# open-speech/HTK

Measured on AMD Instinct MI355X. Metric: herest_gmm_frame_state_loglik_per_sec, higher is better.
Workload: dtype f32 (scores: bf16x3 split operands, fp32 accumulate) + f64 (alpha / beta with fp32-transcendental log-add, accumulators); 1 GPU; HERest EM iteration (pass + accumulator all-reduce + model update), 5000 tied states x 16 mix, D=39, 1250 x 500-frame utterances per GPU (BASELINE config[2]: 10k utterances sharded 8-way); states=5000, mix=16, utts_per_gpu=1250, frames=500, chunks=1, update=HERest -m 3 -v 0.01, on the device

## Files before the change

### htk_amd/build.py

```python
from __future__ import annotations

import os
import subprocess
import sys

HERE = os.path.dirname(os.path.abspath(__file__))
OBJ = os.path.join(HERE, "_obj")
LIB = os.path.join(HERE, "libhtk_amd.so")
HIP_SRCS = ["csrc/model.hip", "csrc/gmm_exact.hip", "csrc/gmm_full.hip", "csrc/gmm_mfma.hip", "csrc/gmm_bf16.hip", "csrc/gmm_f16.hip", "csrc/fb_kernels.hip", "csrc/fb_wave.hip", "csrc/fb_state.hip", "csrc/fb_lr.hip", "csrc/fb.hip", "csrc/viterbi.hip", "csrc/decode.hip", "csrc/decode_n.hip", "csrc/decode_ord.hip", "csrc/decode_set.hip", "csrc/mfcc.hip", "csrc/cepsnorm.hip", "csrc/inputxform.hip", "csrc/update.hip", "csrc/comm.hip", "csrc/treeclust.hip", "csrc/datacluster.hip", "csrc/treesynth.hip", "csrc/hinit.hip", "csrc/hrest.hip", "csrc/results.hip", "csrc/latrescore.hip"]
C_SRCS = ["host/prep.c", "host/update.c", "host/fbank.c", "host/accio.c", "host/parmfile.c", "host/cepsnorm.c", "host/mmf.c", "host/labio.c", "host/net.c", "host/lattice.c", "host/slfout.c", "host/treeclust.c", "host/treesynth.c", "host/hinit.c", "host/hrest.c", "host/unit_train.c", "host/results.c", "host/latrescore.c", "host/htktext.c"]
HEADERS = ["csrc/fb_lr_lean.inc", "csrc/internal.h", "csrc/kernels.h", "csrc/hipcheck.h", "csrc/devbuf.h", "csrc/ladd.h", "csrc/wavegrp.h", "csrc/fb_state.h", "csrc/decode.h", "csrc/decode_dev.h", "csrc/decode_ord.h", "csrc/hinit_seg.h", "csrc/gauss_derive.h", "csrc/unit_train.h", "csrc/results.h", "csrc/latrescore.h", "host/mmf_priv.h", "host/htktext.h", "../include/htk_amd.h"]
ARCH = "gfx950"
EXTRA_FLAGS = {"csrc/gmm_mfma.hip": ["-fno-honor-nans"], "csrc/gmm_bf16.hip": ["-fno-honor-nans"], "csrc/gmm_f16.hip": ["-fno-honor-nans"],
               "csrc/fb_kernels.hip": ["-Wno-pass-failed"]}


def _newer(target, deps):
    if not os.path.exists(target):
        return True
    t = os.path.getmtime(target)
    return any(os.path.getmtime(d) > t for d in deps if os.path.exists(d))


def build(force: bool = False, verbose: bool = False) -> str:
    os.makedirs(OBJ, exist_ok=True)
    hdrs = [os.path.join(HERE, h) for h in HEADERS]
    objs = []
    procs = []
    for src in HIP_SRCS + C_SRCS:
        p = os.path.join(HERE, src)
        if not os.path.exists(p):
            continue
        o = os.path.join(OBJ, os.path.basename(src) + ".o")
        objs.append(o)
        if force or _newer(o, [p] + hdrs):
            if src.endswith(".hip"):
                cmd = ["hipcc", "--offload-arch=" + ARCH, "-O3", "-ffp-contract=off", "-fPIC", "-std=c++17",
                       "-Wall", "-Wno-unused-function"] + EXTRA_FLAGS.get(src, []) + ["-c", p, "-o", o]
            else:
                cmd = ["gcc", "-O2", "-std=gnu11", "-ffp-contract=off", "-fPIC", "-Wall", "-c", p, "-o", o]
            if verbose:
                print(" ".join(cmd))
            procs.append((cmd, subprocess.Popen(cmd)))
    for cmd, pr in procs:
        if pr.wait() != 0:
            raise RuntimeError("build failed: " + " ".join(cmd))
    if force or procs or _newer(LIB, objs):
        cmd = ["hipcc", "--offload-arch=" + ARCH, "-shared", "-fPIC", "-o", LIB] + objs + ["-lm", "-ldl"]
        if verbose:
            print(" ".join(cmd))
        subprocess.check_call(cmd)
    build_tools(verbose)
    return LIB


TOOLS = ["herest", "hvite"]


def build_tools(verbose: bool = False) -> None:
    root = os.path.dirname(HERE)
    bindir = os.path.join(root, "tools", "bin")
    os.makedirs(bindir, exist_ok=True)
    for t in TOOLS:
        src = os.path.join(root, "tools", t + ".c")
        if not os.path.exists(src):
            continue
        exe = os.path.join(bindir, t)
        if not _newer(exe, [src, os.path.join(root, "tools", "cli_common.h"), os.path.join(root, "include", "htk_amd.h"), LIB]):
            continue
        cmd = ["gcc", "-O2", "-std=gnu11", "-Wall", "-I" + os.path.join(root, "include"), "-I" + os.path.join(root, "tools"), src, "-o", exe,
               "-L" + HERE, "-lhtk_amd", "-Wl,-rpath,$ORIGIN/../../htk_amd", "-lm"]
        if verbose:
            print(" ".join(cmd))
        subprocess.check_call(cmd)


if __name__ == "__main__":
    print(build(force="--force" in sys.argv, verbose=True))
```

### htk_amd/csrc/fb.hip

```cpp
#include <hip/hip_runtime.h>
#include <cstdio>
#include <cstdlib>
#include <cstring>
#include <cmath>
#include <algorithm>
#include <vector>
#include <thread>
#include <mutex>
#include <condition_variable>
#include <functional>
#include "internal.h"
#include "hipcheck.h"
#include "kernels.h"
#include "devbuf.h"

static constexpr char fbOwner[] = "fb";
typedef DevBufT<fbOwner> DevBuf;

struct PrepPool {
   std::vector<std::thread> th;
   std::mutex mu;
   std::condition_variable cvGo, cvDone;
   std::function<void(int)> job;
   int generation = 0, pending = 0, nJobs = 0;
   bool quit = false;
   void start(int n)
   {
      for (int k = 0; k < n; k++)
         th.emplace_back([this, k]() {
            int seen = 0;
            for (;;) {
               std::function<void(int)> f;
               {
                  std::unique_lock<std::mutex> lk(mu);
                  cvGo.wait(lk, [&] { return quit || generation != seen; });
                  if (quit) return;
                  seen = generation;
                  if (k + 1 >= nJobs) { if (--pending == 0) cvDone.notify_one(); continue; }
                  f = job;
               }
               f(k + 1);
               std::unique_lock<std::mutex> lk(mu);
               if (--pending == 0) cvDone.notify_one();
            }
         });
   }
   void run(int n, const std::function<void(int)> &f)
   {
      if (n <= 1 || th.empty()) { for (int k = 0; k < n; k++) f(k); return; }
      {
         std::unique_lock<std::mutex> lk(mu);
         job = f; nJobs = n; pending = (int)th.size(); generation++;
      }
      cvGo.notify_all();
      f(0);
      std::unique_lock<std::mutex> lk(mu);
      cvDone.wait(lk, [&] { return pending == 0; });
   }
   ~PrepPool()
   {
      { std::unique_lock<std::mutex> lk(mu); quit = true; }
      cvGo.notify_all();
      for (auto &t : th) t.join();
   }
};


template <typename T> struct Tab : std::vector<T> { const T *dev = nullptr; };

enum TabGroup { TG_MODEL, TG_CELL, TG_SLOT, TG_SLOT_PAIR, TG_SLOT_STREAM, TG_THREAD, TG_TASK, TG_TASK_WIDE, TG_BATCH, TG_COUNT };

#define FB_BATCH_TABLES(X) \
   X(UttDesc, utt, TG_BATCH) \
   X(int, mN, TG_MODEL) X(int, mTp, TG_MODEL) X(int, mCell0, TG_MODEL) X(int, mSlot0, TG_MODEL) X(int, mDms, TG_MODEL) X(int, mHmm, TG_MODEL) X(int, mTrans, TG_MODEL) \
   X(int, slotState, TG_SLOT) \
   X(short, cQ, TG_CELL) X(short, thrCell, TG_THREAD) X(short, cI, TG_CELL) \
   X(short, taperLo, TG_BATCH) X(short, taperHi, TG_BATCH)       \
   X(ScoreTask, tasks, TG_TASK) X(ScoreTask, tasksW, TG_TASK_WIDE)       \
   X(size_t, gamOff, TG_BATCH) X(int, gamChunkUtt, TG_BATCH) \
   X(int, uttList, TG_BATCH)            \
   X(short, sQ, TG_SLOT) \
   X(int, slotStateU, TG_SLOT_STREAM)   \
   X(int, nextSame, TG_BATCH)           \
   X(int, qBeamNP, TG_BATCH)            \
   X(int, slotRange, TG_SLOT_PAIR)      \
   X(int, wqStart, TG_BATCH)

struct BatchTables {
#define X(T, name, group) Tab<T> name;
   FB_BATCH_TABLES(X)
#undef X
   template <class O, class F> void for_each(O &o, F &&f)
   {
#define X(T, name, group) f(name, o.name, group);
      FB_BATCH_TABLES(X)
#undef X
   }
   template <class F> void for_each(F &&f) { for_each(*this, [&](auto &v, auto &, int g) { f(v, g); }); }
};

struct PrepChunk : BatchTables {
   std::vector<int> evLo, evHi;
   size_t outp = 0, beta = 0, gam = 0;
   long long frameStates = 0;
   int nCellsMax = 1, QMax = 1, TMax = 1, nThrMax = 64, rc = HTKAMD_OK;
   char err[256] = "";
   void reset()
   {
      for_each([](auto &v, int) { v.clear(); });
      outp = beta = gam = 0; frameStates = 0; nCellsMax = QMax = TMax = 1; nThrMax = 64; rc = HTKAMD_OK; err[0] = 0;
   }
};

struct UttClasses {
   static constexpr int N = 13;
   struct Range { int first, n; };
   static int index(int family, int W) { return W == 0 ? 4 : (family ? 4 * family + 1 : 0) + (W == 1 ? 0 : W == 2 ? 1 : W == 4 ? 2 : 3); }
   void set(const std::vector<int> (&cls)[N], std::vector<int> &list)
   {
      list.clear();
      for (int c = 0; c < N; c++) { list.insert(list.end(), cls[c].begin(), cls[c].end()); off[c + 1] = (int)list.size(); }
   }
   Range of(int family, int W) const { const int c = index(family, W); return {off[c], off[c + 1] - off[c]}; }
   Range general() const { return of(FB_LANE_PER_MODEL, 0); } int nGeneral() const { return general().n; }
   int nLr() const { return off[N] - of(FB_LEFT_TO_RIGHT, 1).first; }
   bool anyOffLr() const { return of(FB_LEFT_TO_RIGHT, 1).first > 0; }
private:
   int off[N + 1] = {};
};

struct ResLayout {
   size_t nUtt;
   size_t status() const { return sizeof(double) * nUtt; }
   size_t counter() const { return (sizeof(double) + sizeof(int)) * nUtt; }
   size_t flag() const { return counter() + sizeof(int); } size_t bytes() const { return counter() + 2 * sizeof(int); }
};

enum { UTT_NO_TEE = 1, UTT_ALL_LR = 2 };

struct htkamd_fb : BatchTables {
   htkamd_model *m = nullptr;
   int nUtt = 0;
   int debug = 0;
   int forceGeneral = 0;
   int noStatePath = 0;
   int noLrPath = 0;
   int topoVersion = 0;
   std::vector<unsigned char> uttFlags;
   UttClasses cls;
   size_t gamTotal = 0, betaWTotal = 0, alphaWTotal = 0;
   int totalFrames = 0, nCellsMax = 1, QMax = 1, TMax = 1, blockDim = 64;
   long long frameStates = 0;
   const float *dX = nullptr;
   DevBuf d_arena;
   DevBuf d_qLo, d_qHi, d_aLo, d_aHi, d_outp, d_beta, d_gam, d_alpha, d_pr;
   DevBuf d_betaW;
   DevBuf d_tmE, d_tmMaxP;
   DevBuf d_outpU;
   DevBuf d_alphaW, d_qBeam, d_aBeam, d_trPart, d_hits, d_hitCtl;
   DevBuf d_sink;
   DevBuf d_stCnt, d_stBucket;
   DevBuf d_laneRec;
   bool mixStateLast = false;
   bool mixDeferred = false;
   FbArgs *faMix = nullptr;
   const int *qBeamLast = nullptr;
   DevBuf d_transOff, d_trOccOff, d_counter;
   DevBuf d_rec, d_recSorted, d_recCtl;
   int recCapForce = 0;
   PrepPool *pool = nullptr; std::vector<PrepChunk> *chunks = nullptr;
   void *h_arena = nullptr; size_t h_arenaCap = 0;
   void *h_res = nullptr; size_t h_resCap = 0;
   hipEvent_t evRes = nullptr; bool resPending = false;
   bool f16Pass = false;
   hipEvent_t ev[6] = {}, evK[2] = {}, evCopy = nullptr;
   hipStream_t resStream = nullptr;
   bool timed = false, copyPending = false, scored = false;
   int evMode = 0, evModeLast = 0;
   ResLayout res() const { return {(size_t)nUtt}; }
};

static bool compat_revisit(const htkamd_model *m) { return (m->compat & HTKAMD_COMPAT_STREAM_REVISIT) && m->NSt > 1 && m->NSt != 3 && !m->tiedMix; }

extern "C" int htkamd_fb_create(htkamd_model *m, htkamd_fb **out)
{
   if (!m || !out) { htkamd_set_error("fb_create: NULL argument"); return HTKAMD_EINVAL; }
   if (m->fullc) { htkamd_set_error("fb_create: forward-backward on FULLC models is not supported yet (its mixture statistics are diagonal)"); return HTKAMD_EMODEL; }
   if (m->maxM > 4096) { htkamd_set_error("fb_create: %d mixture components per state not supported", m->maxM); return HTKAMD_EMODEL; }
   htkamd_fb *fb = new htkamd_fb();
   fb->m = m;
   auto fail = [&](const char *what, hipError_t e) { htkamd_set_error("fb_create: %s: %s", what, hipGetErrorString(e)); htkamd_fb_destroy(fb); return HTKAMD_EHIP; };
   hipError_t e;
   for (hipEvent_t *v : {&fb->ev[0], &fb->ev[1], &fb->ev[2], &fb->ev[3], &fb->ev[4], &fb->ev[5], &fb->evK[0], &fb->evK[1]})
      if ((e = hipEventCreate(v)) != hipSuccess) return fail("hipEventCreate", e);
   if ((e = hipEventCreateWithFlags(&fb->evCopy, hipEventDisableTiming)) != hipSuccess) return fail("hipEventCreate", e);
   if ((e = hipStreamCreateWithFlags(&fb->resStream, hipStreamNonBlocking)) != hipSuccess) return fail("hipStreamCreate", e);
   int rc;
   if ((rc = fb->d_counter.reserve(64)) || (rc = fb->d_transOff.reserve(sizeof(int) * (m->nT + 1))) || (rc = fb->d_trOccOff.reserve(sizeof(int) * (m->nT + 1)))) { htkamd_fb_destroy(fb); return rc; }
   if ((e = hipMemcpy(fb->d_transOff.p, m->h_transOff, sizeof(int) * (m->nT + 1), hipMemcpyHostToDevice)) != hipSuccess ||
       (e = hipMemcpy(fb->d_trOccOff.p, m->h_trOccOff, sizeof(int) * (m->nT + 1), hipMemcpyHostToDevice)) != hipSuccess) return fail("hipMemcpy", e);
   *out = fb;
   return HTKAMD_OK;
}

extern "C" void htkamd_fb_destroy(htkamd_fb *fb)
{
   if (!fb) return;
   if (fb->h_arena) (void)hipHostFree(fb->h_arena);
   if (fb->h_res) (void)hipHostFree(fb->h_res);
   delete fb->pool; delete fb->chunks; delete fb->faMix;
   for (hipEvent_t v : fb->ev) if (v) (void)hipEventDestroy(v);
   for (hipEvent_t v : {fb->evCopy, fb->evRes, fb->evK[0], fb->evK[1]}) if (v) (void)hipEventDestroy(v);
   if (fb->resStream) (void)hipStreamDestroy(fb->resStream);
   delete fb;
}

extern "C" int htkamd_fb_set_debug(htkamd_fb *fb, int on)
{
   if (!fb) { htkamd_set_error("fb_set_debug: NULL"); return HTKAMD_EINVAL; }
   fb->debug = on & 1;
   fb->forceGeneral = (on & 2) ? 1 : 0;
   fb->noStatePath = (on & 4) ? 1 : 0;
   fb->recCapForce = (on & 8) ? 128 : ((on & 16) ? -1 : 0);
   fb->noLrPath = (on & 32) ? 1 : 0;
   return HTKAMD_OK;
}

static int prep_utterance(htkamd_fb *fb, const htkamd_batch_desc *b, int u, PrepChunk &C)
{
   const htkamd_model *m = fb->m;
   std::vector<int> &evLo = C.evLo, &evHi = C.evHi;
      UttDesc &d = fb->utt[u];
      const int T = b->frameOff[u + 1] - b->frameOff[u], Q = b->labOff[u + 1] - b->labOff[u];
      const int *labs = b->labs + b->labOff[u];
      d.T = T; d.Q = Q; d.frame0 = b->frameOff[u];
      d.q0 = (int)C.mN.size(); d.cell0 = (int)C.cQ.size(); d.slot0 = (int)C.slotState.size();
      d.status = HTKAMD_UTT_OK; d.nEval = 0;
      d.outp0 = C.outp; d.beta0 = C.beta; d.gam0 = C.gam;
      unsigned char &flags = fb->uttFlags[u];
      flags = UTT_NO_TEE | UTT_ALL_LR;
      if (T <= 0 || Q <= 0) {
         for (int t = 0; t < T; t++) { fb->taperLo[d.frame0 + t] = 0; fb->taperHi[d.frame0 + t] = 0; fb->qBeamNP[d.frame0 + t] = 1; }
         d.status = HTKAMD_UTT_SKIPPED; d.nCells = d.nSlots = 0; d.thr0 = (int)C.thrCell.size(); d.nThr = 0; return HTKAMD_OK;
      }
      int nCells = 0, nSlots = 0, qt = 0, prevDm = 1;
      for (int q = 1; q <= Q; q++) {
         const int h = labs[q - 1];
         if (h < 0 || h >= m->H) { snprintf(C.err, sizeof(C.err), "fb_prepare: utterance %d label %d: HMM index %d out of range", u, q, h); return HTKAMD_EINVAL; }
         const int ti = m->h_hmmTrans[h], N = m->h_transN[ti], dm = m->h_minDur[ti];
         C.mN.push_back(N); C.mTp.push_back(m->h_transOff[ti]); C.mCell0.push_back(nCells); C.mSlot0.push_back(nSlots);
         C.mDms.push_back(dm); C.mHmm.push_back(h); C.mTrans.push_back(ti);
         for (int i = 1; i <= N; i++) { C.cQ.push_back((short)q); C.cI.push_back((short)i); }
         for (int j = 2; j < N; j++) { C.slotState.push_back(m->h_hmmState[m->h_hmmStateOff[h] + (j - 2) * m->NSt]); C.sQ.push_back((short)q); C.slotRange.push_back(0); C.slotRange.push_back(-1); }
         nCells += N; nSlots += N - 2; qt += dm;
         if (dm == 0) flags &= ~UTT_NO_TEE;
         if (m->h_transLR[ti] != 1) flags &= ~UTT_ALL_LR;
         if (q > 1 && dm == 0 && prevDm == 0) d.status = HTKAMD_UTT_ETEE;
         prevDm = dm;
      }
      if (C.mDms[d.q0] == 0 || C.mDms[d.q0 + Q - 1] == 0) d.status = HTKAMD_UTT_ETEE;
      if (d.status == HTKAMD_UTT_OK && qt > T) d.status = HTKAMD_UTT_SKIPPED;
      d.nCells = nCells; d.nSlots = nSlots;
      if (m->NSt > 1) for (int ks = 0; ks < m->NSt; ks++) for (int k = 0; k < nSlots; k++) C.slotStateU.push_back(C.slotState[d.slot0 + k] + ks);
      {
         d.thr0 = (int)C.thrCell.size();
         for (int role = 0; role < 3; role++) {
            for (int q = 1; q <= Q; q++) {
               const int c0 = C.mCell0[d.q0 + q - 1], N = C.mN[d.q0 + q - 1];
               if (role == 0) C.thrCell.push_back((short)c0);
               else if (role == 2) C.thrCell.push_back((short)(c0 + N - 1));
               else for (int i = 2; i < N; i++) C.thrCell.push_back((short)(c0 + i - 1));
            }
            while ((C.thrCell.size() - d.thr0) % 64) C.thrCell.push_back((short)-1);
         }
         d.nThr = (int)C.thrCell.size() - d.thr0;
      }
      const bool waveOk = fb->m->maxN <= 5 && !fb->forceGeneral && !compat_revisit(fb->m) && Q <= 512;
      if (!waveOk) {
         if (Q > 32000 || d.nThr > 1024) {
            snprintf(C.err, sizeof(C.err), "fb_prepare: utterance %d has %d models / %d model states; the device path handles chains of up to 512 models of "
                     "up to 5 states, or up to 1024 model states per utterance", u, Q, nCells);
            return HTKAMD_EINVAL;
         }
         if (d.nThr > C.nThrMax) C.nThrMax = d.nThr;
         if (nCells > C.nCellsMax) C.nCellsMax = nCells;
         if (Q > C.QMax) C.QMax = Q;
      }
      if (T > C.TMax) C.TMax = T;
      C.outp += (size_t)T * nSlots; C.beta += (size_t)T * nCells; C.gam += (size_t)T * nSlots;
      if (d.status != HTKAMD_UTT_OK) {
         for (int t = 0; t < T; t++) { fb->taperLo[d.frame0 + t] = 0; fb->taperHi[d.frame0 + t] = 0; fb->qBeamNP[d.frame0 + t] = 1; }
         return HTKAMD_OK;
      }
      short *lo = fb->taperLo.data() + d.frame0 - 1, *hi = fb->taperHi.data() + d.frame0 - 1;
      const int *dms = C.mDms.data() + d.q0 - 1;
      {
         int q = 1, dq = dms[q], i = 0;
         for (int t = 1; t <= T; t++) {
            while (i == dq) { i = 0; if (q < Q) { q++; dq = dms[q]; } else dq = -1; }
            hi[t] = (short)q; i++;
         }
         q = Q; dq = dms[q]; i = 0;
         for (int t = T; t >= 1; t--) {
            while (i == dq) { i = 0; if (q > 1) { q--; dq = dms[q]; } else dq = -1; }
            lo[t] = (short)q; i++;
         }
      }
      evLo.assign(T + 2, 0); evHi.assign(T + 2, 0);
      {
         const long long before = C.frameStates;
         int qHiN = Q, qLoN = lo[T];
         int *npw = fb->qBeamNP.data() + d.frame0 - 1;
         npw[T] = qLoN | (qHiN << 16);
         const int *msl = C.mSlot0.data() + d.q0 - 1;
         auto slotsIn = [&](int a, int z) { return (z < Q ? msl[z + 1] : nSlots) - msl[a]; };
         evLo[T] = qLoN > 1 ? qLoN - 1 : 1; evHi[T] = Q;
// ... 213 lines not shown
         fb->h_arena = nullptr; fb->h_arenaCap = 0;
         const size_t want = total + total / 4;
         HIPCHECK(hipHostMalloc(&fb->h_arena, want, hipHostMallocDefault));
         fb->h_arenaCap = want;
      }
      if (fb->copyPending) { HIPCHECK(hipEventSynchronize(fb->evCopy)); fb->copyPending = false; }
      if ((rc = fb->d_arena.reserve(total))) return rc;
      {
         struct Piece { char *dst; const char *src; size_t n; };
         std::vector<Piece> pieces;
         const size_t cut = (size_t)256 << 10;
         const size_t *at = off.data();
         fb->for_each([&](auto &v, int) {
            const size_t bytes = sizeof(v[0]) * v.size();
            for (size_t o = 0; o < bytes; o += cut)
               pieces.push_back({(char *)fb->h_arena + *at + o, (const char *)v.data() + o, bytes - o < cut ? bytes - o : cut});
            v.dev = (decltype(v.dev))((char *)fb->d_arena.p + *at++);
         });
         const int nP = (int)pieces.size(), nT = nW < 8 ? nW : 8;
         fb->pool->run(nT, [&](int k) { for (int i = k; i < nP; i += nT) memcpy(pieces[i].dst, pieces[i].src, pieces[i].n); });
      }
      HIPCHECK(hipMemcpyAsync(fb->d_arena.p, fb->h_arena, total, hipMemcpyHostToDevice, s));
      HIPCHECK(hipEventRecord(fb->evCopy, s));
      fb->copyPending = true;
   }
   const bool wavePathPrep = fb->cls.nGeneral() == 0;
   const size_t nf = fb->totalFrames ? fb->totalFrames : 1;
   if ((rc = fb->d_qLo.reserve(sizeof(short) * nf)) || (rc = fb->d_qHi.reserve(sizeof(short) * nf)) ||
       (rc = fb->d_aLo.reserve(sizeof(short) * nf)) || (rc = fb->d_aHi.reserve(sizeof(short) * nf)) ||
       (rc = fb->d_outp.reserve(sizeof(float) * (outp + 16))) || (rc = fb->d_beta.reserve(sizeof(double) * ((beta && !wavePathPrep) ? beta : 1))) ||
       (rc = fb->d_gam.reserve(sizeof(double) * ((gam && fb->cls.anyOffLr()) ? gam : 1))) || (rc = fb->d_pr.reserve(ResLayout{(size_t)(U ? U : 1)}.bytes())) ||
       (fb->m->NSt > 1 && (rc = fb->d_outpU.reserve(sizeof(float) * (outp * fb->m->NSt + 16)))) ||
       (fb->m->tiedMix && ((rc = fb->d_tmE.reserve(sizeof(float) * (nf * fb->m->tmPool + 16))) || (rc = fb->d_tmMaxP.reserve(sizeof(float) * (nf * fb->m->NSt + 16))))))
      return rc;
   if (fb->debug && (rc = fb->d_alpha.reserve(sizeof(double) * (beta ? beta : 1)))) return rc;
   guard.ok = true;
   return HTKAMD_OK;
}

extern "C" long long htkamd_fb_frame_states(const htkamd_fb *fb) { return fb ? fb->frameStates : 0; }

extern "C" int htkamd_fb_score_work(const htkamd_fb *fb, long long out[3])
{
   if (!fb || !out) { htkamd_set_error("fb_score_work: NULL argument"); return HTKAMD_EINVAL; }
   long long skip = 0, all = 0;
   const bool ranges = fb->m->NSt == 1 && fb->slotRange.size() == 2 * fb->slotState.size();
   for (const ScoreTask &tk : fb->tasksW) {
      const int nPairs = (tk.nSlots + 1) >> 1;
      for (int w = 0; w < B16_TASK_FRAMES / 32; w++) {
         if (32 * w >= tk.nFrames) break;
         all += nPairs;
         if (!ranges) { skip += nPairs; continue; }
         const int r0 = tk.frame0 + 32 * w, r1 = r0 + 31;
         for (int j = 0; j < nPairs; j++) {
            const int k0 = tk.slot0 + 2 * j, k1 = (2 * j + 1 < tk.nSlots) ? k0 + 1 : k0;
            const int lo = std::min(fb->slotRange[2 * k0], fb->slotRange[2 * k1]), hi = std::max(fb->slotRange[2 * k0 + 1], fb->slotRange[2 * k1 + 1]);
            if (lo <= r1 && hi >= r0) skip++;
         }
      }
   }
   out[0] = skip; out[1] = all; out[2] = (fb->frameStates + 63) / 64;
   return HTKAMD_OK;
}

extern "C" int htkamd_fb_prepared_current(const htkamd_fb *fb) { return fb && fb->topoVersion == fb->m->topoVersion; }

static ScoreArgs fb_score_args(htkamd_fb *fb, const htkamd_fb_config *cfg)
{
   const htkamd_model *m = fb->m;
   ScoreArgs sa = htkamd_score_args(m);
   sa.NSt = 1; sa.streamWt = nullptr;
   const bool wideTasks = (cfg->scoreMode & (HTKAMD_SCORE_F16 | HTKAMD_SCORE_BF16 | HTKAMD_SCORE_MFMA)) != 0;
   const Tab<ScoreTask> &tasks = wideTasks ? fb->tasksW : fb->tasks;
   sa.tasks = tasks.dev; sa.nTasks = (int)tasks.size(); sa.X = fb->dX;
   sa.slotState = fb->slotState.dev; sa.out = (float *)fb->d_outp.p;
   if (m->NSt > 1) { sa.slotState = fb->slotStateU.dev; sa.out = (float *)fb->d_outpU.p; }
   sa.taskCounter = (int *)fb->d_counter.p;
   if (wideTasks && m->NSt == 1 && fb->wqStart.size() == 9) { sa.qStart = fb->wqStart.dev; sa.qCounters = (int *)fb->d_counter.p + 8; }
   if ((cfg->scoreMode & HTKAMD_SCORE_BF16) && !(cfg->scoreMode & HTKAMD_SCORE_F16) && m->NSt == 1 && !getenv("HTKAMD_NO_TAPER_SKIP")) sa.slotRange = fb->slotRange.dev;
   fb->f16Pass = (cfg->scoreMode & HTKAMD_SCORE_F16) != 0 && !m->tiedMix && sa.nTasks > 0;
   if (fb->f16Pass) {
      sa.taskCounter = (int *)((char *)fb->d_pr.p + fb->res().counter());
      sa.rangeFlag = (int *)((char *)fb->d_pr.p + fb->res().flag());
   }
   return sa;
}

static FbArgs fb_args(const htkamd_fb *fb, const htkamd_fb_config *cfg, const htkamd_accs *accs)
{
   const htkamd_model *m = fb->m;
   FbArgs fa;
   memset(&fa, 0, sizeof(fa));
   fa.utt = fb->utt.dev; fa.nUtt = fb->nUtt;
   fa.mN = fb->mN.dev; fa.mTp = fb->mTp.dev; fa.mCell0 = fb->mCell0.dev; fa.mSlot0 = fb->mSlot0.dev; fa.mDms = fb->mDms.dev; fa.mHmm = fb->mHmm.dev; fa.mTrans = fb->mTrans.dev;
   fa.sQ = fb->sQ.dev; fa.thrCell = fb->thrCell.dev; fa.cQ = fb->cQ.dev; fa.cI = fb->cI.dev; fa.slotState = fb->slotState.dev;
   fa.taperLo = fb->taperLo.dev; fa.taperHi = fb->taperHi.dev;
   fa.qLo = (short *)fb->d_qLo.p; fa.qHi = (short *)fb->d_qHi.p; fa.aLo = (short *)fb->d_aLo.p; fa.aHi = (short *)fb->d_aHi.p;
   fa.X = fb->dX; fa.transP = m->d_transP; fa.outp = (float *)fb->d_outp.p;
   fa.beta = (double *)fb->d_beta.p; fa.gam = (double *)fb->d_gam.p; fa.alphaDbg = fb->debug ? (double *)fb->d_alpha.p : nullptr;
   fa.pr = (double *)fb->d_pr.p; fa.status = (int *)((char *)fb->d_pr.p + fb->res().status());
   fa.stateCompOff = m->d_stateCompOff; fa.compGauss = m->d_compGauss;
   fa.NSt = m->NSt; fa.outpU = (const float *)fb->d_outpU.p; fa.dimStream = m->d_dimStream;
   fa.compatRevisit = compat_revisit(m) && !fb->nextSame.empty(); fa.nextSame = fb->nextSame.dev;
   fa.transOff = (const int *)fb->d_transOff.p; fa.trOccOff = (const int *)fb->d_trOccOff.p;
   fa.compLogWt = m->d_compLogWt; fa.gparam = m->d_gparam; fa.mean = m->d_mean; fa.laddTab = m->d_laddTab;
   fa.PS = m->PS; fa.D = m->D; fa.maxN = m->maxN; fa.maxM = m->maxM;
   fa.nCellsMax = fb->nCellsMax; fa.QMax = fb->QMax; fa.TMax = fb->TMax;
   fa.acc = accs->d_vec; fa.lay = accs->lay;
   fa.pruneInit = cfg->pruneInit; fa.pruneInc = cfg->pruneInc; fa.pruneLim = cfg->pruneLim;
   fa.minLogExp = m->minLogExp; fa.minFrwdP = cfg->minFrwdP; fa.uFlags = cfg->uFlags;
   fa.gamTotal = fb->gamTotal; fa.gamOffByUtt = fb->gamOff.dev; fa.gamChunkUtt = fb->gamChunkUtt.dev;
   return fa;
}

struct LdsSizes { size_t beta, alpha; };
static LdsSizes fb_lds_sizes(const FbArgs &fa)
{
   const size_t nc = fa.nCellsMax, qm = fa.QMax + 3, mn = fa.maxN, tm = (size_t)fa.TMax + 3;
   auto r8 = [](size_t x) { return (x + 7) & ~(size_t)7; };
   const size_t ldsTab = r8((size_t)LADD_NK * (LADD_DEG + 1) * 8);
   return {2 * r8(nc * 8) + r8(qm * 8) + r8(nc * mn * 4) + 4 * r8(qm * 4) + r8(32) + ldsTab,
           2 * r8(nc * 8) + r8(3 * nc * 8) + r8(qm * 8) + r8(nc * (mn + 1) * 8) + ldsTab + r8(3 * nc * 4) + 2 * r8(nc * mn * 4) + 4 * r8(qm * 4) + 2 * r8(tm * 2)};
}

static const int clsW[4] = {1, 2, 4, 8};

static int fb_reserve_lr(htkamd_fb *fb, const htkamd_fb_config *cfg, FbArgs &fa, bool fastLadd, hipStream_t s)
{
   const htkamd_model *m = fb->m;
   int rc;
   size_t rows = 0;
   for (int W : clsW) rows += (size_t)fb->cls.of(FB_LEFT_TO_RIGHT, W).n * htkamd_stats_lr_chunks(fb->TMax) * W;
   const size_t nfr = fb->totalFrames ? fb->totalFrames : 1;
   if ((rc = fb->d_laneRec.reserve(sizeof(LaneRec) * (fb->slotState.size() + 1))) || (rc = fb->d_sink.reserve(256))) return rc;
   fa.laneRec = (LaneRec *)fb->d_laneRec.p; fa.sink = (double *)fb->d_sink.p;
   if ((rc = fb->d_alphaW.reserve(sizeof(double) * (fb->alphaWTotal + 64))) || (rc = fb->d_qBeam.reserve(sizeof(int) * (nfr + 2))) ||
       (rc = fb->d_aBeam.reserve(sizeof(int) * (nfr + 2))) || (rc = fb->d_trPart.reserve(sizeof(double) * htkamd_stats_lr_row_doubles() * (rows + 256))) ||
       (rc = fb->d_hits.reserve(sizeof(MixHit) * (rows * htkamd_stats_lr_region_cap() + 64))) || (rc = fb->d_hitCtl.reserve(sizeof(int) * (rows + 1))))
      return rc;
   fa.alphaW = (double *)fb->d_alphaW.p; fa.qBeam = (int *)fb->d_qBeam.p; fa.aBeam = (int *)fb->d_aBeam.p; fa.trPart = (double *)fb->d_trPart.p;
   fa.hits = (MixHit *)fb->d_hits.p; fa.hitCtl = (int *)fb->d_hitCtl.p; fa.nHitRegions = (int)rows; fa.hitRegionCap = htkamd_stats_lr_region_cap();
   fa.hitSlots = (m->NSt > 1 || m->tiedMix) ? 1 : 0;
   fa.qBeamNP = fb->qBeamNP.dev;
   if (htkamd_beta_lr_is_lean(fa, fastLadd)) fa.qBeam = const_cast<int *>(fb->qBeamNP.dev);
   fb->qBeamLast = fa.qBeam;
   fb->mixStateLast = false;
   fa.fastMath = fastLadd ? 1 : 0;
   if (fb->recCapForce == 0 && !fa.hitSlots && m->maxM <= 16 && (m->D == 39 || m->D == 26 || m->D == 13) &&
       (cfg->uFlags & (HTKAMD_UPMEANS | HTKAMD_UPVARS | HTKAMD_UPMIXES))) {
      size_t cap = 64;
      while (cap < 65536 && cap * (size_t)m->S < (size_t)16 * fb->totalFrames) cap <<= 1;
      while (cap > 64 && cap * (size_t)m->S * sizeof(HitS) > ((size_t)1 << 30)) cap >>= 1;
      { const char *e = getenv("HTKAMD_ST_CAP"); if (e && atoi(e) > 0) cap = (size_t)atoi(e); }
      if ((rc = fb->d_stCnt.reserve(sizeof(int) * (3 * (size_t)m->S + 4))) || (rc = fb->d_stBucket.reserve(sizeof(HitS) * cap * (size_t)m->S))) return rc;
      fb->mixStateLast = true;
      fa.stCnt = (int *)fb->d_stCnt.p; fa.nTiedStates = m->S; fa.stBucket = (HitS *)fb->d_stBucket.p; fa.stCap = (int)cap;
      HIPCHECK(hipMemsetAsync(fa.stCnt, 0, sizeof(int) * (3 * (size_t)m->S + 4), s));
   }
   return HTKAMD_OK;
}

struct FamilyKernels { int family; int (*beta)(const FbArgs &, int, bool, hipStream_t); int (*alpha)(const FbArgs &, int, bool, hipStream_t); };
static const FamilyKernels familyKernels[] = {{FB_LANE_PER_MODEL, htkamd_launch_beta_w, htkamd_launch_alpha_w},
                                              {FB_LANE_PER_STATE, htkamd_launch_beta_s, htkamd_launch_alpha_s},
                                              {FB_LEFT_TO_RIGHT, htkamd_launch_beta_lr, htkamd_launch_alpha_lr}};

static int fb_recursions(htkamd_fb *fb, const FbArgs &fa, const LdsSizes &lds, bool fastLadd, bool noEv, hipStream_t s)
{
   int rc;
   for (int pass = 0; pass < 2; pass++) {
      FbArgs fc = fa;
      const UttClasses::Range g = fb->cls.general();
      fc.uttList = fb->uttList.dev + g.first; fc.nList = g.n;
      if (g.n > 0 && (rc = pass == 0 ? htkamd_launch_beta(fc, fb->blockDim, lds.beta, s) : htkamd_launch_alpha(fc, fb->blockDim, lds.alpha, s))) return rc;
      for (const FamilyKernels &k : familyKernels)
         for (int c = 3; c >= 0; c--) {
            const UttClasses::Range r = fb->cls.of(k.family, clsW[c]);
            fc.uttList = fb->uttList.dev + r.first; fc.nList = r.n;
            if ((rc = (pass == 0 ? k.beta : k.alpha)(fc, clsW[c], fastLadd, s))) return rc;
         }
      if (!noEv) HIPCHECK(hipEventRecord(fb->ev[2 + pass], s));
   }
   return HTKAMD_OK;
}

static int fb_stats_lr(htkamd_fb *fb, const FbArgs &fa, bool fastLadd, bool noEv, hipStream_t s)
{
   int rc;
   FbArgs fc = fa;
   size_t rowOff = 0;
   for (int c = 3; c >= 0; c--) {
      const UttClasses::Range r = fb->cls.of(FB_LEFT_TO_RIGHT, clsW[c]);
      fc.uttList = fb->uttList.dev + r.first; fc.nList = r.n;
      fc.trPart = fa.trPart ? fa.trPart + rowOff * htkamd_stats_lr_row_doubles() : nullptr;
      fc.hits = fa.hits ? fa.hits + rowOff * htkamd_stats_lr_region_cap() : nullptr; fc.hitCtl = fa.hitCtl ? fa.hitCtl + rowOff : nullptr;
      rowOff += (size_t)fc.nList * htkamd_stats_lr_chunks(fb->TMax) * clsW[c];
      if ((rc = htkamd_launch_stats_lr(fc, clsW[c], fastLadd, s))) return rc;
   }
   if (!noEv) HIPCHECK(hipEventRecord(fb->ev[4], s));
   return HTKAMD_OK;
}

static int fb_mix_stats(htkamd_fb *fb, const htkamd_fb_config *cfg, FbArgs &fa, bool defer, hipStream_t s)
{
   const htkamd_model *m = fb->m;
   const int nLr = fb->cls.nLr();
   int rc;
   if (!(cfg->uFlags & (HTKAMD_UPMEANS | HTKAMD_UPVARS | HTKAMD_UPMIXES))) return HTKAMD_OK;
   if ((cfg->uFlags & (HTKAMD_UPMEANS | HTKAMD_UPVARS)) && fb->recCapForce >= 0) {
      const size_t cap = fb->recCapForce > 0 ? (size_t)fb->recCapForce : std::min<size_t>((size_t)16 * fb->totalFrames + 4096, (size_t)1 << 30);
      if ((rc = fb->d_rec.reserve(sizeof(MixRec) * cap)) || (rc = fb->d_recSorted.reserve(sizeof(MixRec) * cap)) ||
          (rc = fb->d_recCtl.reserve(sizeof(int) * (3 * ((size_t)m->G + 1) + 1 + (size_t)m->G / 2048 + 2))))
         return rc;
      fa.rec = (MixRec *)fb->d_rec.p; fa.recSorted = (MixRec *)fb->d_recSorted.p; fa.recCap = (int)cap; fa.G = m->G; fa.recCtl = (int *)fb->d_recCtl.p;
   }
   if (m->tiedMix || m->NSt > 1) {
      fa.stateCompOff = m->d_stateCompOff; fa.rec = nullptr;
      if (fb->nUtt > nLr && (rc = m->tiedMix ? htkamd_launch_mixstats_tm(fa, s) : htkamd_launch_mixstats_ms(fa, s))) return rc;
      if (nLr > 0 && (rc = htkamd_launch_mixhits_streams(fa, m->tiedMix != 0, s))) return rc;
      return HTKAMD_OK;
   }
   const bool dense = fb->nUtt > nLr && fa.gamTotal > 0, listed = nLr > 0;
   if ((rc = htkamd_launch_mixstats(fa, s, dense, listed, defer))) return rc;
   if (defer && listed && !dense && htkamd_mixstate_applies(fa)) {
      if (!fb->faMix) fb->faMix = new FbArgs();
      *fb->faMix = fa;
      fb->mixDeferred = true;
   }
   return HTKAMD_OK;
}

static int fb_execute_impl(htkamd_fb *fb, const htkamd_fb_config *cfg, htkamd_accs *accs, void *stream, bool defer)
{
   if (!fb || !cfg || !accs) { htkamd_set_error("fb_execute: NULL argument"); return HTKAMD_EINVAL; }
   fb->mixDeferred = false;
   if (accs->m != fb->m) { htkamd_set_error("fb_execute: accumulators belong to a different model"); return HTKAMD_EINVAL; }
   if (fb->nUtt == 0) return HTKAMD_OK;
   const htkamd_model *m = fb->m;
   hipStream_t s = (hipStream_t)stream;
   if (fb->topoVersion != m->topoVersion) {
      htkamd_set_error("fb_execute: the model's minimum durations changed since htkamd_fb_prepare (a re-estimated transition reached or left zero): prepare the batch again");
      return HTKAMD_EINVAL;
   }
   const ScoreArgs sa = fb_score_args(fb, cfg);
   if (cfg->scoreMode & ~(HTKAMD_SCORE_MFMA | HTKAMD_SCORE_FASTLADD | HTKAMD_SCORE_BF16 | HTKAMD_SCORE_F16 | HTKAMD_SCORE_SOUTP | HTKAMD_SCORE_DIAGC)) { htkamd_set_error("fb_execute: unknown score mode %d", cfg->scoreMode); return HTKAMD_EINVAL; }
   const bool fastLadd = (cfg->scoreMode & HTKAMD_SCORE_FASTLADD) != 0;
   FbArgs fa = fb_args(fb, cfg, accs);
   const LdsSizes lds = fb_lds_sizes(fa);

   int rc;
   if (fb->copyPending) HIPCHECK(hipStreamWaitEvent(s, fb->evCopy, 0));
   const bool noEv = fb->evMode == 1;
   HIPCHECK(hipEventRecord(fb->ev[0], s));
   if (m->tiedMix) {
      fa.tmE = (float *)fb->d_tmE.p; fa.tmMaxP = (float *)fb->d_tmMaxP.p; fa.tmPoolOff = m->d_tmPoolOff; fa.tmPool = m->tmPool; fa.totalFrames = fb->totalFrames;
      fa.tmTasks = fb->tasks.dev; fa.tmNTasks = (int)fb->tasks.size(); fa.tmSlotState = sa.slotState; fa.tmOut = sa.out;
      fa.compWeight = m->d_compWeight; fa.var = m->d_var;
      if ((rc = htkamd_launch_tm_score(fa, s))) return rc;
      fb->scored = false;
   } else {
      if ((rc = htkamd_launch_score(cfg->scoreMode, m, sa, s, fb->evK[0], fb->evK[1]))) return rc;
      fb->scored = sa.nTasks > 0;
   }
   if (m->NSt > 1) {
      if ((rc = htkamd_launch_combine_streams(fa, s))) return rc;
      if (m->maxM > 1) fa.stateCompOff = m->d_msCompOff;
   } else if (m->tiedMix) fa.stateCompOff = m->d_msCompOff;
   if (!noEv) HIPCHECK(hipEventRecord(fb->ev[1], s));
   if (fb->cls.nGeneral() > 0 && lds.alpha > 160 * 1024) { htkamd_set_error("fb_execute: %zu bytes of LDS needed (max model size %zu states)", lds.alpha, (size_t)m->maxN); return HTKAMD_EMODEL; }
   if ((rc = fb->d_betaW.reserve(sizeof(double) * (fb->betaWTotal + 8 * 512)))) return rc;
   fa.betaW = (double *)fb->d_betaW.p;
   if (fb->cls.nLr() > 0 && (rc = fb_reserve_lr(fb, cfg, fa, fastLadd, s))) return rc;
   if ((rc = fb_recursions(fb, fa, lds, fastLadd, noEv, s)) || (rc = fb_stats_lr(fb, fa, fastLadd, noEv, s)) || (rc = fb_mix_stats(fb, cfg, fa, defer, s))) return rc;
   HIPCHECK(hipEventRecord(fb->ev[5], s));
   fb->timed = true; fb->evModeLast = noEv ? 1 : 0;
   return HTKAMD_OK;
}

extern "C" int htkamd_fb_execute(htkamd_fb *fb, const htkamd_fb_config *cfg, htkamd_accs *accs, void *stream)
{
   return fb_execute_impl(fb, cfg, accs, stream, false);
}

extern "C" int htkamd_fb_execute_begin(htkamd_fb *fb, const htkamd_fb_config *cfg, htkamd_accs *accs, void *stream, int *deferred)
{
   if (deferred) *deferred = 0;
   const int rc = fb_execute_impl(fb, cfg, accs, stream, true);
   if (rc == HTKAMD_OK && deferred && fb && fb->nUtt > 0) *deferred = fb->mixDeferred ? 1 : 0;
   return rc;
}

extern "C" int htkamd_fb_execute_mix(htkamd_fb *fb, int state0, int state1, void *stream)
{
   if (!fb) { htkamd_set_error("fb_execute_mix: NULL"); return HTKAMD_EINVAL; }
   if (fb->nUtt == 0 || !fb->mixDeferred) return HTKAMD_OK;
   const int rc = htkamd_launch_mixstate_range(*fb->faMix, state0, state1, (hipStream_t)stream);
   if (rc) return rc;
   HIPCHECK(hipEventRecord(fb->ev[5], (hipStream_t)stream));
   return HTKAMD_OK;
}


static int res_staging(htkamd_fb *fb, size_t bytes)
{
   if (bytes > fb->h_resCap) {
      if (fb->h_res) (void)hipHostFree(fb->h_res);
      fb->h_res = nullptr; fb->h_resCap = 0;
      HIPCHECK(hipHostMalloc(&fb->h_res, bytes + bytes / 4, hipHostMallocDefault));
      fb->h_resCap = bytes + bytes / 4;
   }
   return HTKAMD_OK;
}

extern "C" int htkamd_fb_results_begin(htkamd_fb *fb, void *stream)
{
   if (!fb) { htkamd_set_error("fb_results_begin: NULL"); return HTKAMD_EINVAL; }
   if (fb->nUtt == 0) return HTKAMD_OK;
   hipStream_t s = (hipStream_t)stream;
   const size_t bytes = fb->res().bytes();
   int rc = res_staging(fb, bytes);
   if (rc) return rc;
   if (!fb->evRes) HIPCHECK(hipEventCreateWithFlags(&fb->evRes, hipEventDisableTiming));
   HIPCHECK(hipMemcpyAsync(fb->h_res, fb->d_pr.p, bytes, hipMemcpyDeviceToHost, s));
   HIPCHECK(hipEventRecord(fb->evRes, s));
   fb->resPending = true;
   return HTKAMD_OK;
}

extern "C" int htkamd_fb_results(htkamd_fb *fb, double *pr, int *status, void *stream)
{
   if (!fb) { htkamd_set_error("fb_results: NULL"); return HTKAMD_EINVAL; }
   hipStream_t s = (hipStream_t)stream;
   if (fb->nUtt == 0) return HTKAMD_OK;
   const size_t bytes = fb->res().bytes();
   if (fb->resPending) {
      fb->resPending = false;
      HIPCHECK(hipEventSynchronize(fb->evRes));
   } else {
      int rc = res_staging(fb, bytes);
      if (rc) return rc;
      hipStream_t cs = fb->timed ? fb->resStream : s;
      if (fb->timed) HIPCHECK(hipEventSynchronize(fb->ev[5]));
      HIPCHECK(hipMemcpyAsync(fb->h_res, fb->d_pr.p, bytes, hipMemcpyDeviceToHost, cs));
      HIPCHECK(hipStreamSynchronize(cs));
   }
   if (pr) memcpy(pr, fb->h_res, sizeof(double) * (size_t)fb->nUtt);
   if (status) memcpy(status, (const char *)fb->h_res + fb->res().status(), sizeof(int) * (size_t)fb->nUtt);
   if (fb->f16Pass) {
      int flag;
      memcpy(&flag, (const char *)fb->h_res + fb->res().flag(), sizeof(int));
      if (flag) {
         htkamd_set_error("fb_results: the fp16 scoring path met %s%s%s outside its range: nothing of this pass can be used (accumulators included) -- repeat it with HTKAMD_SCORE_BF16",
                          (flag & HTKAMD_F16_EMODEL) ? "a model coefficient" : "", (flag & HTKAMD_F16_EMODEL) && (flag & HTKAMD_F16_EFEAT) ? " and " : "", (flag & HTKAMD_F16_EFEAT) ? "a feature value" : "");
         return HTKAMD_ERANGE;
      }
   }
   return HTKAMD_OK;
}

extern "C" int htkamd_fb_set_event_mode(htkamd_fb *fb, int mode)
{
   if (!fb || mode < 0 || mode > 1) { htkamd_set_error("fb_set_event_mode: bad argument"); return HTKAMD_EINVAL; }
   fb->evMode = mode;
   return HTKAMD_OK;
}

extern "C" int htkamd_fb_kernel_times5(htkamd_fb *fb, double out[5])
{
   if (!fb || !out) { htkamd_set_error("fb_kernel_times: NULL"); return HTKAMD_EINVAL; }
   if (!fb->timed) { htkamd_set_error("fb_kernel_times: nothing executed yet"); return HTKAMD_EINVAL; }
   HIPCHECK(hipEventSynchronize(fb->ev[5]));
   for (int i = 0; i < 5; i++) {
      float ms = 0.f;
      if (i == 0 && fb->scored) HIPCHECK(hipEventElapsedTime(&ms, fb->evK[0], fb->evK[1]));
      else if (fb->evModeLast == 1) { out[i] = -1.0; continue; }
      else HIPCHECK(hipEventElapsedTime(&ms, fb->ev[i], fb->ev[i + 1]));
      out[i] = (double)ms * 1e-3;
   }
   return HTKAMD_OK;
}

extern "C" int htkamd_fb_mix_counts(htkamd_fb *fb, long long out[2])
{
   if (!fb || !out) { htkamd_set_error("fb_mix_counts: NULL"); return HTKAMD_EINVAL; }
   out[0] = out[1] = -1;
   if (!fb->timed || !fb->mixStateLast || !fb->d_stCnt.p) return HTKAMD_OK;
   HIPCHECK(hipEventSynchronize(fb->ev[5]));
   const size_t S = (size_t)fb->m->S;
   std::vector<int> c(2 * S);
   HIPCHECK(hipMemcpy(c.data(), (int *)fb->d_stCnt.p + S + 4, sizeof(int) * 2 * S, hipMemcpyDeviceToHost));
   out[0] = out[1] = 0;
   for (size_t i = 0; i < S; i++) { out[0] += c[2 * i]; out[1] += c[2 * i + 1]; }
   return HTKAMD_OK;
}

extern "C" int htkamd_fb_kernel_times(htkamd_fb *fb, double out[4])
{
   double t[5];
   const int rc = htkamd_fb_kernel_times5(fb, t);
   if (rc) return rc;
   out[0] = t[0]; out[1] = t[1]; out[2] = (t[2] < 0.0 || t[3] < 0.0) ? -1.0 : t[2] + t[3]; out[3] = t[4];
   return HTKAMD_OK;
}

extern "C" int htkamd_fb_get_trellis(htkamd_fb *fb, int u, double *beta, double *alpha, float *outp,
                                     int *qLo, int *qHi, int *aLo, int *aHi, int *pT, int *pQ, int *pMaxN, void *stream)
{
   if (!fb || u < 0 || u >= fb->nUtt) { htkamd_set_error("fb_get_trellis: bad utterance index"); return HTKAMD_EINVAL; }
   hipStream_t s = (hipStream_t)stream;
   HIPCHECK(hipStreamSynchronize(s));
   const UttDesc &d = fb->utt[u];
   const int T = d.T, Q = d.Q, nC = d.nCells, nS = d.nSlots, maxN = fb->m->maxN;
   if (pT) *pT = T; if (pQ) *pQ = Q; if (pMaxN) *pMaxN = maxN;
   if (T <= 0 || Q <= 0) return HTKAMD_OK;
   std::vector<short> lo(T), hi(T), alo(T), ahi(T);
   const std::pair<std::vector<short> *, const DevBuf *> beams[] = {{&lo, &fb->d_qLo}, {&hi, &fb->d_qHi}, {&alo, &fb->d_aLo}, {&ahi, &fb->d_aHi}};
   for (auto &bm : beams) HIPCHECK(hipMemcpy(bm.first->data(), (short *)bm.second->p + d.frame0, sizeof(short) * T, hipMemcpyDeviceToHost));
   if (d.W > 0 && d.family == FB_LEFT_TO_RIGHT && fb->qBeamLast) {
      std::vector<int> qb(T);
      HIPCHECK(hipMemcpy(qb.data(), fb->qBeamLast + d.frame0, sizeof(int) * T, hipMemcpyDeviceToHost));
      for (int t = 0; t < T; t++) { lo[t] = (short)(qb[t] & 0xffff); hi[t] = (short)((qb[t] >> 16) & 0xffff); }
   }
   if (d.W > 0 && d.family == FB_LEFT_TO_RIGHT) {
      std::vector<int> ab(T);
      HIPCHECK(hipMemcpy(ab.data(), (int *)fb->d_aBeam.p + d.frame0, sizeof(int) * T, hipMemcpyDeviceToHost));
      for (int t = 0; t < T; t++) { alo[t] = fb->sQ[d.slot0 + (ab[t] & 0xffff)]; ahi[t] = fb->sQ[d.slot0 + ((ab[t] >> 16) & 0xffff)]; }
   }
   for (int t = 0; t < T; t++) {
      if (qLo) qLo[t] = lo[t]; if (qHi) qHi[t] = hi[t]; if (aLo) aLo[t] = alo[t]; if (aHi) aHi[t] = ahi[t];
   }
   const int *mN = fb->mN.data() + d.q0, *mC = fb->mCell0.data() + d.q0, *mS = fb->mSlot0.data() + d.q0;
   const size_t n = (size_t)T * Q * maxN;
   if (beta) {
      std::vector<double> b((size_t)T * nC);
      if (d.W > 0 && d.family != FB_LANE_PER_MODEL) {
         const bool lr = d.family == FB_LEFT_TO_RIGHT;
         const size_t Lw = (size_t)64 * d.W;
         std::vector<double> bs((size_t)T * (lr ? 1 : 2) * Lw);
         HIPCHECK(hipMemcpy(bs.data(), (double *)fb->d_betaW.p + d.betaW0, sizeof(double) * bs.size(), hipMemcpyDeviceToHost));
         std::vector<float> o(lr ? (size_t)T * nS : 0);
         if (lr) HIPCHECK(hipMemcpy(o.data(), (float *)fb->d_outp.p + d.outp0, sizeof(float) * o.size(), hipMemcpyDeviceToHost));
         const int *mTp = fb->mTp.data() + d.q0;
         auto entry = [&](int t, int q) {
            const int l0 = mS[q - 1];
            if (!lr) return bs[(size_t)T * Lw + (size_t)t * Lw + l0];
            if (q < lo[t] || q > hi[t]) return (double)LZERO;
            const double aa = fb->m->h_transP[mTp[q - 1] + 1], y = bs[(size_t)t * Lw + l0];
            if (!(aa > LSMALL && y > LSMALL)) return (double)LZERO;
            const double v = aa + (double)o[(size_t)l0 * T + t] + y;
            return v < LSMALL ? (double)LZERO : v;
         };
         for (int t = 0; t < T; t++)
            for (int q = 1; q <= Q; q++) {
               const int Nq = mN[q - 1], l0 = mS[q - 1];
               double *cell = &b[(size_t)t * nC + mC[q - 1]];
               cell[0] = entry(t, q);
               for (int i = 2; i < Nq; i++) cell[i - 1] = bs[(size_t)t * Lw + l0 + i - 2];
               double bN = LZERO;
               if (t == T - 1) bN = (q == Q) ? 0.0 : LZERO;
               else if (q < Q && q + 1 >= lo[t + 1] && q + 1 <= hi[t + 1]) bN = entry(t + 1, q + 1);
               cell[Nq - 1] = bN;
            }
      } else if (d.W > 0) {
         const size_t run = (size_t)64 * d.W;
         std::vector<double> bs((size_t)T * 5 * run);
         HIPCHECK(hipMemcpy(bs.data(), (double *)fb->d_betaW.p + d.betaW0, sizeof(double) * bs.size(), hipMemcpyDeviceToHost));
         for (int t = 0; t < T; t++)
            for (int q = 1; q <= Q; q++)
               for (int i = 0; i < mN[q - 1]; i++)
                  b[(size_t)t * nC + mC[q - 1] + i] = bs[((size_t)t * 5 + i) * run + (q - 1)];
      } else
      HIPCHECK(hipMemcpy(b.data(), (double *)fb->d_beta.p + d.beta0, sizeof(double) * b.size(), hipMemcpyDeviceToHost));
      for (size_t k = 0; k < n; k++) beta[k] = NAN;
      for (int t = 0; t < T; t++)
         for (int q = lo[t]; q <= hi[t]; q++)
            for (int i = 0; i < mN[q - 1]; i++)
               beta[((size_t)t * Q + (q - 1)) * maxN + i] = b[(size_t)t * nC + mC[q - 1] + i];
   }
   if (alpha) {
      if (!fb->debug) { htkamd_set_error("fb_get_trellis: alpha is only kept in debug mode (htkamd_fb_set_debug before prepare)"); return HTKAMD_EINVAL; }
      std::vector<double> al((size_t)T * nC);
      HIPCHECK(hipMemcpy(al.data(), (double *)fb->d_alpha.p + d.beta0, sizeof(double) * al.size(), hipMemcpyDeviceToHost));
      for (size_t k = 0; k < n; k++) alpha[k] = NAN;
      for (int t = 0; t < T; t++)
         for (int q = 1; q <= Q; q++)
            for (int i = 0; i < mN[q - 1]; i++)
               alpha[((size_t)t * Q + (q - 1)) * maxN + i] = al[(size_t)t * nC + mC[q - 1] + i];
   }
   if (outp) {
      std::vector<float> o((size_t)T * nS);
      HIPCHECK(hipMemcpy(o.data(), (float *)fb->d_outp.p + d.outp0, sizeof(float) * o.size(), hipMemcpyDeviceToHost));
      for (size_t k = 0; k < n; k++) outp[k] = NAN;
      for (int t = 0; t < T; t++)
         for (int q = 1; q <= Q; q++)
            for (int j = 2; j < mN[q - 1]; j++)
               outp[((size_t)t * Q + (q - 1)) * maxN + (j - 1)] = o[(size_t)(mS[q - 1] + j - 2) * T + t];
   }
   return HTKAMD_OK;
}

int htkamd_fb_device_results(htkamd_fb *fb, htkamd_fb_dev *out)
{
   if (!fb || !out || fb->nUtt <= 0 || !fb->d_pr.p) { htkamd_set_error("fb_device_results: no pass to read"); return HTKAMD_EINVAL; }
   out->pr = (const double *)fb->d_pr.p; out->status = (const int *)((const char *)fb->d_pr.p + fb->res().status());
   return HTKAMD_OK;
}
```

### htk_amd/csrc/fb_kernels.hip

```cpp
#include <hip/hip_runtime.h>
#include <cstring>
#include <cstdlib>
#include "internal.h"
#include "hipcheck.h"
#include "kernels.h"
#include "ladd.h"

#define ladd(x, y, mle) ladd_tab((x), (y), (mle), ltab)

#define EXPFLOOR (-100.0)

struct CellMeta {
   int q, i, N, mc0, ms0;
};

struct LdsCarve {
   char *p;
   __device__ explicit LdsCarve(void *base) : p((char *)base) {}
   template <typename T> __device__ T *take(size_t n)
   {
      T *r = (T *)p;
      p += ((n * sizeof(T) + 7) & ~(size_t)7);
      return r;
   }
// ... 533 lines not shown
            }
            recUsed += np;
         }
      }
   }
   if (pass) {
      if (upMu && !stored) atomicAdd(a.acc + a.lay.muOcc + g, Lr);
      if (upVa && !stored) atomicAdd(a.acc + a.lay.vaOcc + g, Lr);
      if (upWt) atomicAdd(a.acc + a.lay.wt + c0 + m, Lr);
   }
   unsigned long long pm = __ballot(pass && !stored);
   while (pm) {
      const int ml = __ffsll((long long)pm) - 1;
      pm &= pm - 1;
      const double L = __shfl(Lr, ml);
      const int gg = __shfl(g, ml);
      const unsigned long long xp = (unsigned long long)xrow;
      const float *xr = (const float *)(((unsigned long long)__shfl((int)(xp >> 32), ml) << 32) | (unsigned int)__shfl((int)(xp & 0xffffffffu), ml));
      const float *mean = a.mean + (size_t)gg * D;
      for (int k = lane; k < D; k += 64) {
         const float z = xr[k] - mean[k];
         if (upMu && upVa) {
            const float zl = (float)((double)z * L);
            atomicAdd(a.acc + a.lay.mu + (size_t)gg * D + k, (double)zl);
            atomicAdd(a.acc + a.lay.va + (size_t)gg * D + k, (double)(z * zl));
         } else if (upMu) {
            atomicAdd(a.acc + a.lay.mu + (size_t)gg * D + k, (double)z * L);
         } else if (upVa) {
            atomicAdd(a.acc + a.lay.va + (size_t)gg * D + k, (double)(z * z) * L);
         }
      }
   }
}

template <int DT, int GS>
__device__ __forceinline__ void mix_hit(const FbArgs &a, const bool ok, const int st, const int frameRow, const double seed, int &recBase, int &recUsed)
{
   const int lane = threadIdx.x & 63, sub = lane % GS;
   const int D = DT > 0 ? DT : a.D;
   const double minF = (double)a.minFrwdP;
   const int s = ok ? st : 0;
   const int c0 = a.stateCompOff[s], M = ok ? a.stateCompOff[s + 1] - c0 : 0;
   const float *xrow = a.X + (size_t)(ok ? frameRow : 0) * D;
   int Mmax = M;
#pragma unroll
   for (int o = 32; o > 0; o >>= 1) { const int w = __shfl_xor(Mmax, o); Mmax = w > Mmax ? w : Mmax; }
   for (int mb = 0; mb < Mmax; mb += GS) {
      const int m = mb + sub;
      bool pass = false;
      double Lr = 0.0;
      int g = 0;
      if (m < M) {
         g = a.compGauss[c0 + m];
         if (M == 1 || a.maxM == 1) { pass = true; Lr = exp(seed); }
         else {
            const float wt = a.compLogWt[c0 + m];
            if (wt > (float)LMINMIX) {
               const float *P = a.gparam + (size_t)g * a.PS;
               float sum = P[2 * D];
               if (DT > 0) {
                  const float4 *P4 = (const float4 *)P;
                  constexpr int NQ = (DT + 1) / 2;
#pragma unroll 1
                  for (int q0 = 0; q0 < NQ; q0 += 4) {
                     float4 pv[4]; float xv[8];
#pragma unroll
                     for (int i = 0; i < 4; i++) if (q0 + i < NQ) pv[i] = P4[q0 + i];
#pragma unroll
                     for (int i = 0; i < 8; i++) if (2 * q0 + i < DT) xv[i] = xrow[2 * q0 + i];
#pragma unroll
                     for (int i = 0; i < 8; i++)
                        if (2 * q0 + i < DT) {
                           const float mu = (i & 1) ? pv[i >> 1].z : pv[i >> 1].x, iv = (i & 1) ? pv[i >> 1].w : pv[i >> 1].y;
                           const float xmm = xv[i] - mu;
                           sum += xmm * xmm * iv;
                        }
                  }
               } else {
                  for (int i = 0; i < D; i++) {
                     const float xmm = xrow[i] - P[2 * i];
                     sum += xmm * xmm * P[2 * i + 1];
                  }
               }
               const float prob = -0.5f * sum;
               const double x = (seed + (double)wt) + (double)prob;
               if (-x < minF) { pass = true; Lr = exp(x); }
            }
         }
      }
      mix_post<GS>(a, s, c0, m, g, pass, Lr, frameRow, xrow, recBase, recUsed);
   }
}

template <int DT, int GS>
__global__ __launch_bounds__(256, 4) void k_mixstats(FbArgs a)
{
   constexpr int HPS = 64 / GS;
   __shared__ unsigned short hitIdx[4][512];
   __shared__ double hitSeed[4][512];
   const int lane = threadIdx.x & 63;
   const int grp = lane / GS;
   const size_t nWaves = ((size_t)gridDim.x * blockDim.x) >> 6;
   const size_t waveId = ((size_t)blockIdx.x * blockDim.x + threadIdx.x) >> 6;
   int recBase = -1, recUsed = 0;
   for (size_t base0 = waveId * 512; base0 < a.gamTotal; base0 += nWaves * 512) {
    double vv[8];
#pragma unroll
    for (int r = 0; r < 8; r++) {
       const size_t idx = base0 + (size_t)r * 64 + lane;
       vv[r] = (idx < a.gamTotal) ? a.gam[idx] : LZERO;
    }
    const int cu = a.gamChunkUtt[base0 >> 9];
    volatile unsigned short *hIdx = hitIdx[threadIdx.x >> 6];
    volatile double *hSeed = hitSeed[threadIdx.x >> 6];
    int count = 0;
#pragma unroll
    for (int r = 0; r < 8; r++) {
       const double v = vv[r];
       const unsigned long long hm = __ballot(v > LSMALL);
       if (v > LSMALL) {
          const int pos = count + __popcll(hm & ((1ull << lane) - 1));
          hIdx[pos] = (unsigned short)(r * 64 + lane); hSeed[pos] = v;
       }
       count += __popcll(hm);
    }
    for (int i0 = 0; i0 < count; i0 += HPS) {
       const int src = (i0 + grp < count) ? i0 + grp : -1;
       const bool have = src >= 0;
       const size_t hidx = base0 + (have ? hIdx[src] : 0);
       const double seed = have ? hSeed[src] : LZERO;
       int u = cu;
       while (u + 1 < a.nUtt && a.gamOffByUtt[u + 1] <= hidx) u++;
       const UttDesc *up = a.utt + u;
       const size_t udGam0 = up->gam0;
       const int udSlots = up->nSlots, udSlot0 = up->slot0, udFrame0 = up->frame0;
       const bool ok = have && a.status[u] == HTKAMD_UTT_OK && up->family != FB_LEFT_TO_RIGHT;
       const size_t rel = hidx - udGam0;
       const int nSl = udSlots > 0 ? udSlots : 1;
       const int t0 = (int)(rel / nSl), slot = (int)(rel % nSl);
       mix_hit<DT, GS>(a, ok, ok ? a.slotState[udSlot0 + slot] : 0, udFrame0 + (ok ? t0 : 0), seed, recBase, recUsed);
    }
   }
   if (recBase >= 0 && recUsed + lane < 64) a.rec[recBase + recUsed + lane].g = -1;
}

__device__ __forceinline__ double uniform_f64(double v)
{
   const unsigned long long b = __builtin_bit_cast(unsigned long long, v);
   const unsigned int lo = __builtin_amdgcn_readfirstlane((unsigned int)b), hi = __builtin_amdgcn_readfirstlane((unsigned int)(b >> 32));
   return __builtin_bit_cast(double, ((unsigned long long)hi << 32) | lo);
}

template <int DT, int GS>
__global__ __launch_bounds__(256, 3) void k_mixhits(FbArgs a)
{
   constexpr int HPS = 64 / GS;
   __shared__ int hitSt[4][64], hitFrame[4][64];
   __shared__ double hitSeed[4][64];
   __shared__ unsigned long long hitKey[4][64];
   const int lane = threadIdx.x & 63, wv = threadIdx.x >> 6;
   const int grp = lane / GS, sub = lane % GS;
   const int nWaves = (int)(((size_t)gridDim.x * blockDim.x) >> 6);
   const int waveId = (int)(((size_t)blockIdx.x * blockDim.x + threadIdx.x) >> 6);
   if (a.stCnt && a.stBucket && !a.hitSlots && a.stCnt[a.nTiedStates] == 0) return;
   int recBase = -1, recUsed = 0;
   volatile int *hSt = hitSt[wv], *hFr = hitFrame[wv];
   volatile double *hSeed = hitSeed[wv];
   volatile unsigned long long *hKey = hitKey[wv];
   for (int b = waveId; b < a.nHitRegions; b += nWaves) {
      const int cnt = a.hitCtl[b];
      const MixHit *reg = a.hits + (size_t)b * a.hitRegionCap;
      for (int c0r = 0; c0r < cnt; c0r += 64) {
         const int n = (cnt - c0r < 64) ? cnt - c0r : 64;
         if constexpr (DT > 0) {
            MixHit h; h.st = 0; h.frame = 0; h.seed = LZERO;
            if (lane < n) h = reg[c0r + lane];
            const unsigned long long key = ((unsigned long long)(unsigned int)h.st << 32) | (unsigned int)h.frame;
            hKey[lane] = (lane < n) ? key : ~0ull;
            int rank = 0;
            for (int jx = 0; jx < n; jx++) { const unsigned long long kj = hKey[jx]; rank += (kj < key || (kj == key && jx < lane)) ? 1 : 0; }
            if (lane < n) { hSt[rank] = h.st; hFr[rank] = h.frame; hSeed[rank] = h.seed; }
            const int per = (n + HPS - 1) / HPS;
            const int i0g = grp * per, i1g = (i0g + per < n) ? i0g + per : n;
            constexpr int NQ = (DT + 1) / 2;
            float4 pm[NQ];
            float gcst = 0.0f, wt = 0.0f;
            int stPrev = -1, c0 = 0, M = 0, g = 0;
            const double minF = uniform_f64((double)a.minFrwdP);
            for (int it = 0; it < per; it++) {
               const int idx = i0g + it;
               const bool have = idx < i1g;
               const int st = have ? hSt[idx] : 0, frameRow = have ? hFr[idx] : 0;
               const double seed = have ? hSeed[idx] : LZERO;
               if (have && st != stPrev) {
                  stPrev = st;
                  c0 = a.stateCompOff[st]; M = a.stateCompOff[st + 1] - c0;
                  if (sub < M) {
                     g = a.compGauss[c0 + sub];
                     wt = a.compLogWt[c0 + sub];
                     const float4 *P4 = (const float4 *)(a.gparam + (size_t)g * a.PS);
#pragma unroll
                     for (int q = 0; q < NQ; q++) pm[q] = P4[q];
                     gcst = a.gparam[(size_t)g * a.PS + 2 * DT];
                  }
               }
               const float *xrow = a.X + (size_t)frameRow * DT;
               bool pass = false;
               double Lr = 0.0;
               if (have && sub < M) {
                  if (M == 1 || a.maxM == 1) { pass = true; Lr = exp(seed); }
                  else if (wt > (float)LMINMIX) {
                     float sum = gcst;
#pragma unroll
                     for (int q0 = 0; q0 < NQ; q0 += 4) {
                        float xv[8];
#pragma unroll
                        for (int i = 0; i < 8; i++) if (2 * q0 + i < DT) xv[i] = xrow[2 * q0 + i];
#pragma unroll
                        for (int i = 0; i < 8; i++)
                           if (2 * q0 + i < DT) {
                              const float4 pv = pm[q0 + (i >> 1)];
                              const float mu = (i & 1) ? pv.z : pv.x, iv = (i & 1) ? pv.w : pv.y;
                              const float xmm = xv[i] - mu;
                              sum += xmm * xmm * iv;
                           }
                     }
                     const float prob = -0.5f * sum;
                     const double x = (seed + (double)wt) + (double)prob;
                     if (-x < minF) { pass = true; Lr = exp(x); }
                  }
               }
               mix_post<GS>(a, st, c0, sub, g, pass, Lr, frameRow, xrow, recBase, recUsed);
            }
         } else {
            if (lane < n) { const MixHit h = reg[c0r + lane]; hSt[lane] = h.st; hFr[lane] = h.frame; hSeed[lane] = h.seed; }
            for (int i0 = 0; i0 < n; i0 += HPS) {
               const int src = (i0 + grp < n) ? i0 + grp : -1;
               const bool have = src >= 0;
               mix_hit<DT, GS>(a, have, have ? hSt[src] : 0, have ? hFr[src] : 0, have ? hSeed[src] : LZERO, recBase, recUsed);
            }
         }
      }
   }
   if (recBase >= 0 && recUsed + lane < 64) a.rec[recBase + recUsed + lane].g = -1;
}

#define REC_TILE 2048
__global__ __launch_bounds__(256) void k_rec_tilesum(int *ctl, int G, int *tileSum)
{
   __shared__ int part[4];
   if (ctl[0] == 0) return;
   const int *cnt = ctl + 1;
   int sum = 0;
   for (int i = blockIdx.x * REC_TILE + threadIdx.x; i < (blockIdx.x + 1) * REC_TILE && i < G; i += 256) sum += cnt[i];
#pragma unroll
   for (int o = 32; o > 0; o >>= 1) sum += __shfl_xor(sum, o);
   if ((threadIdx.x & 63) == 0) part[threadIdx.x >> 6] = sum;
   __syncthreads();
   if (threadIdx.x == 0) tileSum[blockIdx.x] = part[0] + part[1] + part[2] + part[3];
}
__global__ __launch_bounds__(256) void k_rec_tilescan(int *ctl, int G, const int *tileSum)
{
   __shared__ int wsum[4];
   __shared__ int offSh;
   if (ctl[0] == 0) return;
   const int *cnt = ctl + 1;
   int *start = ctl + 1 + (G + 1);
   const int tid = threadIdx.x, lane = tid & 63, wv = tid >> 6;
   int off = 0;
   for (int b = tid; b < (int)blockIdx.x; b += 256) off += tileSum[b];
#pragma unroll
   for (int o = 32; o > 0; o >>= 1) off += __shfl_xor(off, o);
   if (lane == 0) wsum[wv] = off;
   __syncthreads();
   if (tid == 0) offSh = wsum[0] + wsum[1] + wsum[2] + wsum[3];
   __syncthreads();
   off = offSh;
   __syncthreads();
   const int i0 = blockIdx.x * REC_TILE + tid * 8;
   int v[8], mine = 0;
#pragma unroll
   for (int k = 0; k < 8; k++) { v[k] = (i0 + k < G) ? cnt[i0 + k] : 0; mine += v[k]; }
   int inc = mine;
#pragma unroll
   for (int o = 1; o < 64; o <<= 1) { const int w = __shfl_up(inc, o); if (lane >= o) inc += w; }
   if (lane == 63) wsum[wv] = inc;
   __syncthreads();
   int run = off + inc - mine;
   for (int w = 0; w < wv; w++) run += wsum[w];
#pragma unroll
   for (int k = 0; k < 8; k++) { if (i0 + k < G) start[i0 + k] = run; run += v[k]; }
   if (i0 <= G - 1 && G - 1 < i0 + 8) start[G] = run;
}

__global__ __launch_bounds__(256) void k_rec_scatter(FbArgs a)
{
   const int G = a.G;
   if (a.recCtl[0] == 0) return;
   const int *start = a.recCtl + 1 + (G + 1);
   int *cur = a.recCtl + 1 + 2 * (G + 1);
   const int n = (a.recCtl[0] >= 0 && a.recCtl[0] < a.recCap) ? a.recCtl[0] : (a.recCap & ~63);
   for (int i = blockIdx.x * blockDim.x + threadIdx.x; i < n; i += gridDim.x * blockDim.x) {
      const MixRec r = a.rec[i];
      if (r.g < 0) continue;
      a.recSorted[start[r.g] + atomicAdd(cur + r.g, 1)] = r;
   }
}

__global__ __launch_bounds__(256) void k_rec_reduce(FbArgs a)
{
   const int G = a.G, D = a.D, lane = threadIdx.x & 63;
   if (a.recCtl[0] == 0) return;
   const int *start = a.recCtl + 1 + (G + 1);
   const bool upMu = a.uFlags & HTKAMD_UPMEANS, upVa = a.uFlags & HTKAMD_UPVARS;
   const int nWaves = (gridDim.x * blockDim.x) >> 6;
   for (int g = (blockIdx.x * blockDim.x + threadIdx.x) >> 6; g < G; g += nWaves) {
      const int r0 = start[g], r1 = start[g + 1];
      if (r0 == r1) continue;
      for (int k0 = 0; k0 < D; k0 += 64) {
         const int k = k0 + lane;
         const float mean = (k < D) ? a.mean[(size_t)g * D + k] : 0.0f;
         double sMu = 0.0, sVa = 0.0, sL = 0.0;
         for (int rb = r0; rb < r1; rb += 64) {
            const int nb = (r1 - rb < 64) ? r1 - rb : 64;
            MixRec mine; mine.frame = 0; mine.L = 0.0;
            if (lane < nb) mine = a.recSorted[rb + lane];
            sL += mine.L;
            for (int i = 0; i < nb; i += 4) {
               float xv[4]; double Lv[4];
#pragma unroll
               for (int e = 0; e < 4; e++) {
                  const int ii = (i + e < nb) ? i + e : nb - 1;
                  const int fr = __shfl(mine.frame, ii);
                  Lv[e] = (i + e < nb) ? __shfl(mine.L, ii) : 0.0;
                  xv[e] = (k < D) ? a.X[(size_t)fr * D + k] : 0.0f;
               }
#pragma unroll
               for (int e = 0; e < 4; e++) {
                  if (i + e >= nb) break;
                  const float z = xv[e] - mean;
                  const double L = Lv[e];
                  if (upMu && upVa) {
                     const float zl = (float)((double)z * L);
                     sMu += (double)zl; sVa += (double)(z * zl);
                  } else if (upMu) sMu += (double)z * L;
                  else if (upVa) sVa += (double)(z * z) * L;
               }
            }
         }
         if (k < D) {
            if (upMu && sMu != 0.0) atomicAdd(a.acc + a.lay.mu + (size_t)g * D + k, sMu);
            if (upVa && sVa != 0.0) atomicAdd(a.acc + a.lay.va + (size_t)g * D + k, sVa);
         }
         if (k0 == 0) {
#pragma unroll
            for (int o = 32; o > 0; o >>= 1) sL += __shfl_xor(sL, o);
            if (lane == 0) {
               if (upMu) atomicAdd(a.acc + a.lay.muOcc + g, sL);
               if (upVa) atomicAdd(a.acc + a.lay.vaOcc + g, sL);
            }
         }
      }
   }
}

#define MS_EU 8
template <int DT, int MODE>
__global__ __launch_bounds__(64, MS_EU) void k_mixstate(FbArgs a)
{
#define MS_CHUNK 32
#define MS_CAP 128
#define MS_PARTS 4
   constexpr int GS = 16, HPS = 64 / GS, NQ = (DT + 1) / 2, XS = (DT + 3) & ~3;
   constexpr int CH = MS_CHUNK;
   __shared__ float xs[CH * XS];
   __shared__ double Lt[CH][GS];
   __shared__ double hSeed[CH];
   const int st = a.stBase + blockIdx.x, lane = threadIdx.x, grp = lane / GS, sub = lane % GS;
   const int nst = a.stCnt[st] < a.stCap ? a.stCnt[st] : a.stCap;
   const int part = blockIdx.y;
   const int r0 = part * MS_CAP, r1 = (part == (int)gridDim.y - 1 || r0 + MS_CAP > nst) ? nst : r0 + MS_CAP;
   if (r0 >= nst) return;
   const HitS *bucket = a.stBucket + (size_t)st * a.stCap;
   const int c0 = a.stateCompOff[st], M = a.stateCompOff[st + 1] - c0;
   const bool single = (M == 1 || a.maxM == 1);
   constexpr bool upMu = (MODE & 1) != 0, upVa = (MODE & 2) != 0;
   const bool upWt = a.uFlags & HTKAMD_UPMIXES;
   __shared__ float4 pl[NQ][GS];
   int g = 0;
   float wt = 0.0f, gcst = 0.0f;
   if (sub < M) {
      g = a.compGauss[c0 + sub];
      wt = a.compLogWt[c0 + sub];
      gcst = a.gparam[(size_t)g * a.PS + 2 * DT];
      if (grp == 0) {
         const float4 *P4 = (const float4 *)(a.gparam + (size_t)g * a.PS);
#pragma unroll
         for (int q = 0; q < NQ; q++) { const float4 pv = P4[q]; pl[q][sub] = make_float4(pv.x, pv.z, pv.y, pv.w); }
// ... 17 lines not shown
      if (lane < n) { const HitS h = bucket[base + lane]; hfr = h.frame; hSeed[lane] = h.seed; }
      for (int r = 0; r < n; r++) {
         const int fr = __builtin_amdgcn_readlane(hfr, r);
         if (lane < DT)
            __builtin_amdgcn_global_load_lds((const __attribute__((address_space(1))) void *)(a.X + (size_t)fr * DT + lane),
                                             (__attribute__((address_space(3))) void *)(xs + r * XS), 4, 0, 0);
      }
      asm volatile("s_waitcnt vmcnt(0)" ::: "memory");
      __syncthreads();
      for (int it = 0; it * HPS < n; it++) {
         const int h = it * HPS + grp;
         const bool have = h < n;
         bool pass = false;
         double Lr = 0.0;
         if (have && sub < M) {
            const double seed = hSeed[h];
            if (single) { pass = true; Lr = exp(seed); }
            else if (wt > (float)LMINMIX) {
               typedef float v2f __attribute__((ext_vector_type(2)));
               const v2f *xr = (const v2f *)(xs + h * XS);
               float sum = gcst;
#pragma unroll
               for (int q = 0; q < NQ; q++) {
                  const float4 pv = pl[q][sub];
                  const v2f xv = xr[q];
                  v2f mu; mu[0] = pv.x; mu[1] = pv.y;
                  v2f iv; iv[0] = pv.z; iv[1] = pv.w;
                  const v2f xmm = xv - mu;
                  const v2f tt = xmm * xmm * iv;
                  sum += tt[0];
                  if (2 * q + 1 < DT) sum += tt[1];
               }
               const float prob = -0.5f * sum;
               const double x = (seed + (double)wt) + (double)prob;
               if (-x < minF) { pass = true; Lr = a.fastMath ? (double)__builtin_amdgcn_exp2f((float)x * 1.44269504088896341f) : exp(x); }
            }
         }
         if (have) Lt[h][sub] = pass ? Lr : 0.0;
         wtAcc += pass ? Lr : 0.0;
         nTriples += pass ? 1 : 0;
      }
      __syncthreads();
      if (upMu || upVa) {
         unsigned long long bmAll[GS];
#pragma unroll
         for (int m4 = 0; m4 < GS; m4 += 4) {
            double Lq[4];
#pragma unroll
            for (int i = 0; i < 4; i++) Lq[i] = (lane < n) ? Lt[lane][m4 + i] : 0.0;
#pragma unroll
            for (int i = 0; i < 4; i++) bmAll[m4 + i] = __ballot(Lq[i] != 0.0);
         }
#pragma unroll
         for (int m = 0; m < GS; m++) {
            if (m < M) {
               unsigned long long bm = bmAll[m];
               double mu = sMu[m], va = sVa[m];
               const float mean = meanR[m];
               while (bm) {
                  double Lv[4]; float xv[4];
#pragma unroll
                  for (int i = 0; i < 4; i++) {
                     const bool live = bm != 0;
                     const int h = live ? (int)__builtin_ctzll(bm) : 0;
                     bm &= bm - 1;
                     Lv[i] = live ? Lt[h][m] : 0.0;
                     xv[i] = xs[h * XS + (lane < DT ? lane : 0)];
                  }
#pragma unroll
                  for (int i = 0; i < 4; i++) {
                     const double L = Lv[i];
                     const float z = xv[i] - mean;
                     if constexpr (upMu && upVa) { const float zl = (float)((double)z * L); mu += (double)zl; va += (double)(z * zl); }
                     else if constexpr (upMu) mu += (double)z * L;
                     else va += (double)(z * z) * L;
                  }
               }
               sMu[m] = mu; sVa[m] = va;
            }
         }
      }
   }
#pragma unroll
   for (int m = 0; m < GS; m++) {
      if (m < M && lane < DT) {
         const int gm = a.compGauss[c0 + m];
         if (upMu && sMu[m] != 0.0) atomicAdd(a.acc + a.lay.mu + (size_t)gm * DT + lane, sMu[m]);
         if (upVa && sVa[m] != 0.0) atomicAdd(a.acc + a.lay.va + (size_t)gm * DT + lane, sVa[m]);
      }
   }
   double w = wtAcc;
   w += __shfl_xor(w, 16); w += __shfl_xor(w, 32);
   if (grp == 0 && sub < M && w != 0.0) {
      if (upWt) atomicAdd(a.acc + a.lay.wt + c0 + sub, w);
      if (upMu) atomicAdd(a.acc + a.lay.muOcc + g, w);
      if (upVa) atomicAdd(a.acc + a.lay.vaOcc + g, w);
   }
#pragma unroll
   for (int o = 32; o > 0; o >>= 1) nTriples += __shfl_xor(nTriples, o);
   if (lane == 0) { if (part == 0) a.stCnt[a.nTiedStates + 4 + 2 * st] = nst; atomicAdd(a.stCnt + a.nTiedStates + 5 + 2 * st, nTriples); }
   double so = (sub < M) ? w : 0.0;
#pragma unroll
   for (int o = GS / 2; o > 0; o >>= 1) so += __shfl_xor(so, o);
   if (lane == 0 && so != 0.0) atomicAdd(a.acc + a.lay.wtOcc + st, so);
}

bool htkamd_mixstate_applies(const FbArgs &a) { return a.stCnt && a.stBucket && !a.hitSlots && a.maxM <= 16 && (a.D == 39 || a.D == 26 || a.D == 13); }
int htkamd_launch_mixstate_range(const FbArgs &a_in, int st0, int st1, hipStream_t s)
{
   if (st0 < 0 || st1 > a_in.nTiedStates || st0 > st1) { htkamd_set_error("mixture statistics: state range [%d, %d) outside the set's %d", st0, st1, a_in.nTiedStates); return HTKAMD_EINVAL; }
   if (st0 == st1) return HTKAMD_OK;
   FbArgs a = a_in;
   a.stBase = st0;
   const int S = st1 - st0;
   const int mode = ((a.uFlags & HTKAMD_UPMEANS) ? 1 : 0) | ((a.uFlags & HTKAMD_UPVARS) ? 2 : 0);
#define MS_LAUNCH(DT_) \
   do { \
      if (mode == 3) hipLaunchKernelGGL((k_mixstate<DT_, 3>), dim3(S, MS_PARTS), dim3(64), 0, s, a); \
      else if (mode == 1) hipLaunchKernelGGL((k_mixstate<DT_, 1>), dim3(S, MS_PARTS), dim3(64), 0, s, a); \
      else if (mode == 2) hipLaunchKernelGGL((k_mixstate<DT_, 2>), dim3(S, MS_PARTS), dim3(64), 0, s, a); \
      else hipLaunchKernelGGL((k_mixstate<DT_, 0>), dim3(S, MS_PARTS), dim3(64), 0, s, a); \
   } while (0)
   if (a.D == 39) MS_LAUNCH(39); else if (a.D == 26) MS_LAUNCH(26); else MS_LAUNCH(13);
#undef MS_LAUNCH
   HIPCHECK(hipGetLastError());
   return HTKAMD_OK;
}

static int set_lds_limit(const void *fn, size_t lds)
{
   if (lds > 64 * 1024)
      HIPCHECK(hipFuncSetAttribute(fn, hipFuncAttributeMaxDynamicSharedMemorySize, (int)lds));
   return HTKAMD_OK;
}

int htkamd_launch_beta(const FbArgs &a, int blockDim, size_t lds, hipStream_t s)
{
   int rc = set_lds_limit((const void *)k_beta, lds);
   if (rc) return rc;
   hipLaunchKernelGGL(k_beta, dim3(a.nList), dim3(blockDim), lds, s, a);
   HIPCHECK(hipGetLastError());
   return HTKAMD_OK;
}

int htkamd_launch_alpha(const FbArgs &a, int blockDim, size_t lds, hipStream_t s)
{
   int rc = set_lds_limit((const void *)k_alpha, lds);
   if (rc) return rc;
   hipLaunchKernelGGL(k_alpha, dim3(a.nList), dim3(blockDim), lds, s, a);
   HIPCHECK(hipGetLastError());
   return HTKAMD_OK;
}

int htkamd_launch_mixstats(const FbArgs &a_in, hipStream_t s, bool dense, bool listed, bool deferState)
{
   if (!dense && !listed) return HTKAMD_OK;
   FbArgs a = a_in;
   dense = dense && a.gamTotal > 0;
   const bool stateOnly = listed && !dense && htkamd_mixstate_applies(a);
   if (stateOnly) a.rec = nullptr;
   if (a.rec) HIPCHECK(hipMemsetAsync(a.recCtl, 0, sizeof(int) * (3 * ((size_t)a.G + 1) + 1), s));
#define MIX_LAUNCH(K, GS) \
   switch (a.D) { \
   case 39: hipLaunchKernelGGL((K<39, GS>), grid, block, 0, s, a); break; \
   case 26: hipLaunchKernelGGL((K<26, GS>), grid, block, 0, s, a); break; \
   case 13: hipLaunchKernelGGL((K<13, GS>), grid, block, 0, s, a); break; \
   default: hipLaunchKernelGGL((K<0, GS>), grid, block, 0, s, a); break; \
   }
#define MIX_LAUNCH_GS(K) \
   if (a.maxM <= 16) { MIX_LAUNCH(K, 16) } else if (a.maxM <= 32) { MIX_LAUNCH(K, 32) } else { MIX_LAUNCH(K, 64) }
   if (dense) {
      size_t waves = (a.gamTotal + 511) / 512;
      size_t blocks = (waves + 3) / 4;
      if (blocks > 8192) blocks = 8192;
      const dim3 grid((unsigned)blocks), block(256);
      MIX_LAUNCH_GS(k_mixstats)
   }
   if (listed) {
      const dim3 grid(stateOnly ? 512 : 4096), block(256);
      if (stateOnly) {
         MIX_LAUNCH_GS(k_mixhits)
         HIPCHECK(hipGetLastError());
         if (!deferState) { const int rc = htkamd_launch_mixstate_range(a_in, 0, a_in.nTiedStates, s); if (rc) return rc; }
      } else {
         if (htkamd_mixstate_applies(a)) { const int rc = htkamd_launch_mixstate_range(a, 0, a.nTiedStates, s); if (rc) return rc; }
         MIX_LAUNCH_GS(k_mixhits)
      }
   }
#undef MIX_LAUNCH_GS
#undef MIX_LAUNCH
   HIPCHECK(hipGetLastError());
   if (a.rec) {
      const int nTile = (a.G + REC_TILE - 1) / REC_TILE;
      hipLaunchKernelGGL(k_rec_tilesum, dim3(nTile), dim3(256), 0, s, a.recCtl, a.G, a.recCtl + 1 + 3 * (a.G + 1));
      hipLaunchKernelGGL(k_rec_tilescan, dim3(nTile), dim3(256), 0, s, a.recCtl, a.G, a.recCtl + 1 + 3 * (a.G + 1));
      hipLaunchKernelGGL(k_rec_scatter, dim3(2048), dim3(256), 0, s, a);
      const int gb = (a.G + 3) / 4;
      hipLaunchKernelGGL(k_rec_reduce, dim3(gb < 16384 ? gb : 16384), dim3(256), 0, s, a);
      HIPCHECK(hipGetLastError());
   }
   return HTKAMD_OK;
}

__global__ __launch_bounds__(256) void k_combine_streams(FbArgs a)
{
   const UttDesc *up = a.utt + blockIdx.x;
   const size_t n = (size_t)up->T * up->nSlots;
   const float *src = a.outpU + up->outp0 * a.NSt;
   float *dst = a.outp + up->outp0;
   for (size_t i = (size_t)blockIdx.y * blockDim.x + threadIdx.x; i < n; i += (size_t)gridDim.y * blockDim.x) {
      float sum = 0.0f;
      for (int k = 0; k < a.NSt; k++) sum += src[(size_t)k * n + i];
      dst[i] = sum;
   }
}

int htkamd_launch_combine_streams(const FbArgs &a, hipStream_t s)
{
   if (a.nUtt <= 0) return HTKAMD_OK;
   hipLaunchKernelGGL(k_combine_streams, dim3((unsigned)a.nUtt, 16), dim3(256), 0, s, a);
   HIPCHECK(hipGetLastError());
   return HTKAMD_OK;
}

__device__ void ms_pair(const FbArgs &a, const UttDesc *up, const int t0, const int slot, const double seed, const int lane)
{
   const int D = a.D, NSt = a.NSt;
   const double minF = (double)a.minFrwdP;
   const bool upMu = a.uFlags & HTKAMD_UPMEANS, upVa = a.uFlags & HTKAMD_UPVARS, upWt = a.uFlags & HTKAMD_UPMIXES;
   const int nSl = up->nSlots, T = up->T;
   const int e0 = a.slotState[up->slot0 + slot];
   const float *xrow = a.X + (size_t)(up->frame0 + t0) * D;
   const float oS = a.outp[up->outp0 + (size_t)slot * T + t0];
   for (int ks = 0; ks < NSt; ks++) {
      const int e = e0 + ks, c0 = a.stateCompOff[e], M = a.stateCompOff[e + 1] - c0;
      const float oK = a.outpU[up->outp0 * NSt + ((size_t)ks * nSl + slot) * T + t0];
      float sumS = oS;
      if (a.compatRevisit) {
         sumS = 0.0f;
         for (int k2 = 0; k2 < NSt; k2++) sumS += a.outpU[up->outp0 * NSt + ((size_t)k2 * nSl + slot) * T + t0];
      }
      const float others = sumS - oK;
      for (int mb = 0; mb < M; mb += 64) {
         const int m = mb + lane;
         bool pass = false;
         double Lr = 0.0;
         int g = 0;
         if (m < M) {
            const float wt = a.compLogWt[c0 + m];
            g = a.compGauss[c0 + m];
            if (wt > (float)LMINMIX) {
               double x;
               if (M == 1) x = (a.maxM == 1) ? seed : seed + (double)oS;
               else {
                  const float *P = a.gparam + (size_t)g * a.PS;
                  float sum = P[2 * D];
                  for (int k = 0; k < D; k++) {
                     const float xmm = xrow[k] - P[2 * k];
                     sum += xmm * xmm * P[2 * k + 1];
                  }
                  const float prob = -0.5f * sum;
                  x = seed + (double)wt;
                  x += (double)prob;
                  x += (double)others;
               }
               if (-x < minF) { pass = true; Lr = exp(x); }
            }
         }
         double sumLr = pass ? Lr : 0.0;
#pragma unroll
         for (int o = 32; o > 0; o >>= 1) sumLr += __shfl_xor(sumLr, o);
         if (lane == 0 && sumLr != 0.0) atomicAdd(a.acc + a.lay.wtOcc + e, sumLr);
         if (pass) {
            if (upMu) atomicAdd(a.acc + a.lay.muOcc + g, Lr);
            if (upVa) atomicAdd(a.acc + a.lay.vaOcc + g, Lr);
            if (upWt) atomicAdd(a.acc + a.lay.wt + c0 + m, Lr);
         }
         unsigned long long pm = __ballot(pass);
         while (pm) {
            const int ml = __ffsll((long long)pm) - 1;
            pm &= pm - 1;
            const double L = __shfl(Lr, ml);
            const int gg = __shfl(g, ml);
            const float *mean = a.mean + (size_t)gg * D;
            for (int k = lane; k < D; k += 64) {
               if (a.dimStream[k] != ks) continue;
               const float z = xrow[k] - mean[k];
               if (upMu && upVa) {
                  const float zl = (float)((double)z * L);
                  atomicAdd(a.acc + a.lay.mu + (size_t)gg * D + k, (double)zl);
                  atomicAdd(a.acc + a.lay.va + (size_t)gg * D + k, (double)(z * zl));
               } else if (upMu) atomicAdd(a.acc + a.lay.mu + (size_t)gg * D + k, (double)z * L);
               else if (upVa) atomicAdd(a.acc + a.lay.va + (size_t)gg * D + k, (double)(z * z) * L);
            }
         }
      }
   }
}

__global__ __launch_bounds__(256) void k_mixstats_ms(FbArgs a)
{
   __shared__ unsigned short hitIdx[4][512];
   __shared__ double hitSeed[4][512];
   const int lane = threadIdx.x & 63;
   const size_t nWaves = ((size_t)gridDim.x * blockDim.x) >> 6;
   const size_t waveId = ((size_t)blockIdx.x * blockDim.x + threadIdx.x) >> 6;
   for (size_t base0 = waveId * 512; base0 < a.gamTotal; base0 += nWaves * 512) {
      volatile unsigned short *hIdx = hitIdx[threadIdx.x >> 6];
      volatile double *hSeed = hitSeed[threadIdx.x >> 6];
      int count = 0;
      for (int r = 0; r < 8; r++) {
         const size_t idx = base0 + (size_t)r * 64 + lane;
         const double v = (idx < a.gamTotal) ? a.gam[idx] : LZERO;
         const unsigned long long hm = __ballot(v > LSMALL);
         if (v > LSMALL) {
            const int pos = count + __popcll(hm & ((1ull << lane) - 1));
            hIdx[pos] = (unsigned short)(r * 64 + lane); hSeed[pos] = v;
         }
         count += __popcll(hm);
      }
      int u = a.gamChunkUtt[base0 >> 9];
      for (int i = 0; i < count; i++) {
         const size_t hidx = base0 + hIdx[i];
         const double seed = hSeed[i];
         while (u + 1 < a.nUtt && a.gamOffByUtt[u + 1] <= hidx) u++;
         const UttDesc *up = a.utt + u;
         if (a.status[u] != HTKAMD_UTT_OK || up->family == FB_LEFT_TO_RIGHT) continue;
         const int nSl_ = up->nSlots;
         const size_t rel = hidx - up->gam0;
         ms_pair(a, up, (int)(rel / nSl_), (int)(rel % nSl_), seed, lane);
      }
   }
}
// ... 248 lines not shown
```

### htk_amd/csrc/fb_lr.hip

```cpp
#include <hip/hip_runtime.h>
#include <type_traits>
#include "internal.h"
#include "hipcheck.h"
#include "kernels.h"
#include "ladd.h"
#include "wavegrp.h"
#include "fb_state.h"

typedef const __attribute__((address_space(4))) int cint_lr;

#define ALPHA_S(t) (a.alphaW[ud.alphaW0 + (size_t)((t) - 1) * L + gl])
#define ALPHA_E(t, q_) (a.alphaW[ud.alphaW0 + (size_t)T * L + (size_t)((t) - 1) * ud.QP + ((q_) - 1)])

struct LrRegs {
   int q, j, N, mi;
   bool first, last;
   float aSelf, aNext, aPrev;
   float aEntry, aExit;
   float aExitPrev, aEntryNext;
};

__device__ __forceinline__ void load_lr(LrRegs &s, const FbArgs &a, const UttDesc &ud, int gl, bool valid)
{
   s.q = 0; s.j = 2; s.N = 3; s.mi = 0; s.first = false; s.last = false;
// ... 258 lines not shown
   const int myFirst = gl - (j - 2);
   int prevFirst = myFirst;
   if (valid && s.first && q > 1) prevFirst = flOf[q - 1];
#define ladd(x, y) ladd_sel<false>((x), (y), mle, ltab)

   double aJ = LZERO, aE = LZERO, aEnext = LZERO;
   double yPrev = LZERO;
   double xpre = LZERO;
   double bT = LZERO, bT1 = LZERO, bT2 = LZERO;
   float oT = 0.f, oT1 = 0.f;
   int w1 = qBeam[1], w2 = (T >= 2) ? qBeam[2] : 1, w3 = 1;
   int wq1 = w1, wq2 = w2, wSame = -1;
   int hi0 = 0, lo1 = w1 & 0xffff, hi1 = w1 >> 16, lo2 = w2 & 0xffff, hi2 = (T >= 2) ? (w2 >> 16) : 0;
   double *pS = &ALPHA_S(1);
   double *pE = (valid && s.first) ? &ALPHA_E(1, q) : nullptr;
   {
      bT = BETA_S(1);
      if (T >= 2) bT1 = BETA_S(2);
   }
   st.load_all(0); st.park(0);
   if (T > 4) st.load_all(1);
   oT = st.get_all(0); if (T >= 2) oT1 = st.get_all(1);
   int err = 0;
   double mmpA = LZERO;
   int fLo0 = 0, fLo1 = flOf[lo1], fHi1 = flOf[hi1 > 0 ? hi1 : 1], fE0 = 0;
   MaskW<W> mLo = MaskW<W>::range(0, L - 1), mE = MaskW<W>::range(0, -1);
   int mLoOf = 0, mEOf = 0, lo1Of = lo1, hi1Of = hi1, e0Of = -1;
   double eT = LZERO, eT1 = LZERO;
   if (valid && s.first) { eT = entry_beta<false>(s.aEntry, (double)oT, bT); if (T >= 2) eT1 = entry_beta<false>(s.aEntry, (double)oT1, bT1); }

   auto step = [&](const int t, auto first_, auto inner_) -> bool {
      constexpr bool FIRST = decltype(first_)::value, INNER = decltype(inner_)::value;
      const bool has2 = INNER || t + 2 <= T, isLast = !INNER && t == T;
      if (has2) {
         w3 = qBeam[t + 2];
         bT2 = BETA_S(t + 2);
      }
      const int par = t & 1;
      const bool inB = valid && q >= lo1 && q <= hi1;
      bool in;
      int sl = 0, el = 0;
      if constexpr (FIRST) {
         const int eq = hi1;
         double a1 = 0.0;
         for (int k = 2; k <= q && k <= eq; k++) a1 += (double)(float)LZERO;
         in = valid && q <= eq;
         if (in) {
            aE = a1;
            const double aa = s.aEntry;
            xpre = aE + aa;
            aJ = (aa > LSMALL) ? xpre + (double)oT : LZERO;
         }
         sl = 0; el = fHi1;
         xalpha[par][SPAD + gl] = in ? aJ : LZERO;
         xsum[par][SPAD + gl] = inB ? aJ + bT : LZERO;
         xsync<W>();
         yPrev = xalpha[par][SPAD + gl - 1];
      } else {
         const unsigned long long bal = __ballot(valid && s.first && (pr - mmpA > minF));
         if constexpr (W > 1) { if (lane == 0) bslot[par][wv] = bal; }
         const double a1 = (q == 1) ? LZERO : aEnext;
         double x = s.first ? (((double)s.aEntry > LSMALL) ? (double)s.aEntry + a1 : LZERO) : LZERO;
         if (!s.first && (double)s.aPrev > LSMALL && yPrev > LSMALL) x = ladd(x, yPrev + (double)s.aPrev);
         if ((double)s.aSelf > LSMALL && aJ > LSMALL) x = ladd(x, aJ + (double)s.aSelf);
         const double aJn = x + (double)oT;
         xalpha[par][SPAD + gl] = aJn;
         xsum[par][SPAD + gl] = inB ? aJn + bT : LZERO;
         xsync<W>();
         MaskW<W> kept;
         if constexpr (W == 1) kept.w[0] = firsts.w[0] & ~bal;
         else {
#pragma unroll
            for (int k = 0; k < W; k++) kept.w[k] = firsts.w[k] & ~bslot[par][k];
         }
         const int slane = (kept & mLo).lowest();
         if (slane < 0 || slane > fHi1) { err = 1; return false; }
         sl = (slane < fLo1) ? fLo1 : slane;
         const int elane = (kept & mE).highest();
         if (elane < 0 || elane < sl) { err = 1; return false; }
         el = (elane > fHi1) ? fHi1 : elane;
         in = valid && myFirst >= sl && myFirst <= el;
         aJ = in ? aJn : LZERO; aE = in ? a1 : LZERO; xpre = x;
         const bool inPrev = prevFirst >= sl && prevFirst <= el;
         const double yp = xalpha[par][SPAD + gl - 1];
         yPrev = inPrev ? yp : LZERO;
      }
      if (gl == 0) gaBeam[t] = sl | (el << 16);
      *pS = xpre; pS += L;
      if (valid && s.first) { *pE = aE; pE += ud.QP; }
      const double aXp = ((double)s.aExitPrev > LSMALL && yPrev > LSMALL) ? from_zero(yPrev + (double)s.aExitPrev) : LZERO;
      if (a.alphaDbg && valid) {
         double *ad = a.alphaDbg + ud.beta0 + (size_t)(t - 1) * nC + mc0;
         ad[j - 1] = aJ;
         if (s.first) ad[0] = aE;
         if (s.last) {
            const double aa = s.aExit;
            ad[N - 1] = (aa > LSMALL && (t == 1 || aJ > LSMALL)) ? ladd(LZERO, aJ + aa) : LZERO;
         }
      }
      {
         double mm = aE + eT;
         const double *xs = xsum[par] + SPAD + gl;
#pragma unroll
         for (int k = 0; k < 3; k++) { const double v = xs[k]; mm = (2 + k <= N - 1 && v > mm) ? v : mm; }
         mm = (inB && in) ? mm : LZERO;
         const double bNp = (!isLast && q >= lo2 && q <= hi2) ? eT1 : LZERO;
         const double prevExit = (q > 1 && q - 1 >= lo1 && q - 1 <= hi1) ? aXp + bNp : LZERO;
         mmpA = (prevExit > mm) ? prevExit : mm;
      }
      aEnext = aXp;
      bT = bT1; bT1 = bT2;
      oT = oT1;
      if (has2) {
         const int f = t + 1;
         if ((f & 3) == 0) { st.park(f >> 2); if (4 * ((f >> 2) + 1) < T) st.load_all((f >> 2) + 1); }
         oT1 = st.get_all(f);
      }
      eT = eT1;
      if (has2) eT1 = entry_beta<false>(s.aEntry, (double)oT1, bT1);
      if (!INNER || w3 != wSame) {
         hi0 = hi1; lo1 = lo2; hi1 = hi2; lo2 = w3 & 0xffff; hi2 = has2 ? (w3 >> 16) : 0;
         fLo0 = fLo1;
         if (lo1 != lo1Of) { fLo1 = flOf[lo1]; lo1Of = lo1; }
         if (hi1 != hi1Of) { fHi1 = flOf[hi1 > 0 ? hi1 : 1]; hi1Of = hi1; }
         { const int e0 = ((hi0 < Q) ? hi0 + 1 : hi0) + 1; if (e0 != e0Of) { fE0 = flOf[e0]; e0Of = e0; } }
         if (fLo0 != mLoOf) { mLo = MaskW<W>::range(fLo0, L - 1); mLoOf = fLo0; }
         if (fE0 != mEOf) { mE = MaskW<W>::range(0, fE0 - 1); mEOf = fE0; }
         wSame = (has2 && wq1 == wq2 && wq2 == w3) ? w3 : -1;
         wq1 = wq2; wq2 = w3;
      }
      return true;
   };
   if (T >= 1 && step(1, std::true_type{}, std::false_type{})) {
      int t = 2;
      for (; t + 2 <= T; t++) if (!step(t, std::false_type{}, std::true_type{})) { t = T + 1; break; }
      for (; t <= T; t++) if (!step(t, std::false_type{}, std::false_type{})) break;
   }

   if (err) {
      if (gl == 0) { a.status[u] = HTKAMD_UTT_EALPHA; atomicAdd(a.acc + a.lay.nUttSkipped, 1.0); }
      return;
   }
   if (valid && s.first) atomicAdd(a.acc + a.lay.nEgs + cHmm, 1.0);
   if (gl == 0) {
      atomicAdd(a.acc + a.lay.totalPr, pr);
      atomicAdd(a.acc + a.lay.totalT, (double)T);
      atomicAdd(a.acc + a.lay.nUttDone, 1.0);
      atomicAdd(a.acc + a.lay.nEval, (double)ud.nEval);
   }
#undef ladd
}

#define STATS_FC 32
#define TR_ROW 16
#define EXP_TERM(acc, x) do { if constexpr (FAST) acc += exp_fast(x); else if ((x) > EXPFLOOR) acc += exp_tab((x), etab); } while (0)

__global__ __launch_bounds__(256) void k_trans_reduce(FbArgs a, int nRows)
{
   __shared__ double sh[256][TR_ROW + 1];
   __shared__ int mixed;
   const int tid = threadIdx.x, r = blockIdx.x * 256 + tid;
   if (tid == 0) mixed = 0;
   const double *row = a.trPart + (size_t)r * TR_ROW;
   int ti = -1;
   if (r < nRows) ti = (int)row[TR_ROW - 1];
#pragma unroll
   for (int k = 0; k < 11; k++) sh[tid][k] = (ti >= 0) ? row[k] : 0.0;
   __syncthreads();
   __shared__ int tiBlock;
   if (tid == 0) tiBlock = -1;
   __syncthreads();
   if (ti >= 0) atomicMax(&tiBlock, ti);
   __syncthreads();
   const int tb = tiBlock;
   if (ti >= 0 && ti != tb) mixed = 1;
   __syncthreads();
   auto add_row = [&](int t_, const double *v) {
      const int N0 = a.trOccOff[t_ + 1] - a.trOccOff[t_];
      double *tr = a.acc + a.lay.tr + a.transOff[t_];
      double *oc = a.acc + a.lay.trOcc + a.trOccOff[t_];
      for (int i = 2; i <= 4 && i <= N0 - 1; i++) {
         if (v[i - 2] != 0.0) atomicAdd(tr + (size_t)(i - 1) * N0 + (i - 1), v[i - 2]);
         if (v[3 + i - 2] != 0.0) atomicAdd(tr + (size_t)(i - 1) * N0 + i, v[3 + i - 2]);
         if (v[7 + i - 2] != 0.0) atomicAdd(oc + (i - 1), v[7 + i - 2]);
      }
      if (v[6] != 0.0) atomicAdd(tr + 1, v[6]);
      if (v[10] != 0.0) atomicAdd(oc, v[10]);
   };
   if (tb < 0) return;
   if (mixed) {
      if (ti >= 0) add_row(ti, sh[tid]);
      return;
   }
   const int k = tid & 15, part = tid >> 4;
   double v = 0.0;
   if (k < 11) for (int rr = part; rr < 256; rr += 16) v += sh[rr][k];
   __syncthreads();
   sh[part][k] = v;
   __syncthreads();
   if (tid < 11) {
      double tot = 0.0;
      for (int p = 0; p < 16; p++) tot += sh[p][tid];
      sh[16][tid] = tot;
   }
   __syncthreads();
   if (tid == 0) add_row(tb, sh[16]);
}

#include "fb_lr_lean.inc"

template <bool FAST> static void launch_beta_lr(const FbArgs &a, int W, hipStream_t s)
{
   if (W == 1) hipLaunchKernelGGL((k_beta_lr<1, FAST>), dim3(a.nList), dim3(64), 0, s, a);
   else if (W == 2) hipLaunchKernelGGL((k_beta_lr<2, FAST>), dim3(a.nList), dim3(128), 0, s, a);
   else if (W == 4) hipLaunchKernelGGL((k_beta_lr<4, FAST>), dim3(a.nList), dim3(256), 0, s, a);
   else hipLaunchKernelGGL((k_beta_lr<8, FAST>), dim3(a.nList), dim3(512), 0, s, a);
}
static void launch_alpha_lr(const FbArgs &a, int W, hipStream_t s)
{
   if (W == 1) hipLaunchKernelGGL((k_alpha_lr<1>), dim3(a.nList), dim3(64), 0, s, a);
   else if (W == 2) hipLaunchKernelGGL((k_alpha_lr<2>), dim3(a.nList), dim3(128), 0, s, a);
   else if (W == 4) hipLaunchKernelGGL((k_alpha_lr<4>), dim3(a.nList), dim3(256), 0, s, a);
   else hipLaunchKernelGGL((k_alpha_lr<8>), dim3(a.nList), dim3(512), 0, s, a);
}
template <bool DBG> static void launch_alpha_f(const FbArgs &a, int W, hipStream_t s)
{
   if (W == 1) hipLaunchKernelGGL((k_alpha_f<1, DBG>), dim3(a.nList), dim3(64), 0, s, a);
   else if (W == 2) hipLaunchKernelGGL(k_alpha_f2<DBG>, dim3(a.nList), dim3(64), 0, s, a);
   else if (W == 4) hipLaunchKernelGGL((k_alpha_f<4, DBG>), dim3(a.nList), dim3(256), 0, s, a);
   else hipLaunchKernelGGL((k_alpha_f<8, DBG>), dim3(a.nList), dim3(512), 0, s, a);
}
template <bool FAST> static void launch_stats_sp(const FbArgs &a, int W, int nChunks, hipStream_t s)
{
   if (W == 1) hipLaunchKernelGGL((k_stats_sp<1, FAST>), dim3(a.nList, nChunks), dim3(64), 0, s, a);
   else if (W == 2) hipLaunchKernelGGL((k_stats_sp<2, FAST>), dim3(a.nList, nChunks), dim3(128), 0, s, a);
   else if (W == 4) hipLaunchKernelGGL((k_stats_sp<4, FAST>), dim3(a.nList, nChunks), dim3(256), 0, s, a);
   else hipLaunchKernelGGL((k_stats_sp<8, FAST>), dim3(a.nList, nChunks), dim3(512), 0, s, a);
}

int htkamd_stats_lr_chunks(int TMax) { return (TMax + STATS_FC - 1) / STATS_FC; }
int htkamd_stats_lr_region_cap(void) { return STATS_FC * 64; }
size_t htkamd_stats_lr_row_doubles(void) { return TR_ROW; }

bool htkamd_beta_lr_is_lean(const FbArgs &a, bool fast) { return fast && a.qBeamNP && !(a.pruneInit < HTKAMD_NOPRUNE); }

int htkamd_launch_beta_lr(const FbArgs &a, int W, bool fast, hipStream_t s)
{
   if (a.nList <= 0) return HTKAMD_OK;
   if (htkamd_beta_lr_is_lean(a, fast)) {
      const dim3 grid(a.nList);
      if (W == 2) hipLaunchKernelGGL(k_beta_np2, grid, dim3(64), 0, s, a);
      else if (W == 1) hipLaunchKernelGGL((k_beta_np<1>), grid, dim3(64), 0, s, a);
      else if (W == 4) hipLaunchKernelGGL((k_beta_np<4>), grid, dim3(256), 0, s, a);
      else hipLaunchKernelGGL((k_beta_np<8>), grid, dim3(512), 0, s, a);
      HIPCHECK(hipGetLastError());
      return HTKAMD_OK;
   }
   if (fast) launch_beta_lr<true>(a, W, s); else launch_beta_lr<false>(a, W, s);
   HIPCHECK(hipGetLastError());
   return HTKAMD_OK;
}

int htkamd_launch_alpha_lr(const FbArgs &a, int W, bool fast, hipStream_t s)
{
   if (a.nList <= 0) return HTKAMD_OK;
   if (!fast) launch_alpha_lr(a, W, s);
   else if (a.alphaDbg) launch_alpha_f<true>(a, W, s);
   else launch_alpha_f<false>(a, W, s);
   HIPCHECK(hipGetLastError());
   return HTKAMD_OK;
}

int htkamd_launch_stats_lr(const FbArgs &a, int W, bool fast, hipStream_t s)
{
   if (a.nList <= 0) return HTKAMD_OK;
   const int nChunks = htkamd_stats_lr_chunks(a.TMax);
   if (fast) launch_stats_sp<true>(a, W, nChunks, s); else launch_stats_sp<false>(a, W, nChunks, s);
   const int nRows = a.nList * nChunks * W;
   hipLaunchKernelGGL(k_trans_reduce, dim3((nRows + 255) / 256), dim3(256), 0, s, a, nRows);
   HIPCHECK(hipGetLastError());
   return HTKAMD_OK;
}
```

### htk_amd/csrc/gmm_bf16.hip

```cpp
#include <hip/hip_runtime.h>
#include <hip/hip_ext.h>
#include "internal.h"
#include "hipcheck.h"
#include "kernels.h"

typedef float f4 __attribute__((ext_vector_type(4)));
typedef float f4u __attribute__((ext_vector_type(4), aligned(4)));
typedef __bf16 bf8 __attribute__((ext_vector_type(8)));
typedef unsigned int u4 __attribute__((ext_vector_type(4)));
typedef const __attribute__((address_space(4))) int cint;

#define EXP2(x) __builtin_amdgcn_exp2f(x)
#define LOG2(x) __builtin_amdgcn_logf(x)
#define B16_COL_TILES 2

__device__ __forceinline__ float rows_max_b(float v)
{
   auto a = __builtin_amdgcn_permlane16_swap(__float_as_uint(v), __float_as_uint(v), false, false);
   v = fmaxf(__uint_as_float(a[0]), __uint_as_float(a[1]));
   auto b = __builtin_amdgcn_permlane32_swap(__float_as_uint(v), __float_as_uint(v), false, false);
   return fmaxf(__uint_as_float(b[0]), __uint_as_float(b[1]));
}
__device__ __forceinline__ float rows_sum_b(float v)
{
// ... 311 lines not shown
            } else {
            const int c = ks >> 1, i0 = 8 * (ks & 1) + 4 * khL;
#pragma unroll
            for (int i = 0; i < 4; i++) {
               int dim = dpc * c + i0 + i;
               const bool pad = i0 + i >= dpc || dim >= D;
               if (pad) dim = D - 1;
               float v = row[dim];
               if (pad) v = 0.0f;
               float v2 = v * v;
               if ((ks & 1) && khL == 1 && i == 3) v2 = 1.0f;
               split3(v2, p[0][2 * i], p[1][2 * i], p[2][2 * i]);
               split3(v, p[0][2 * i + 1], p[1][2 * i + 1], p[2][2 * i + 1]);
            }
            }
#pragma unroll
            for (int s = 0; s < 3; s++) {
               u4 w;
               w[0] = p[s][0] | ((unsigned int)p[s][1] << 16); w[1] = p[s][2] | ((unsigned int)p[s][3] << 16);
               w[2] = p[s][4] | ((unsigned int)p[s][5] << 16); w[3] = p[s][6] | ((unsigned int)p[s][7] << 16);
               zb[ks][s] = __builtin_bit_cast(bf8, w);
            }
            __builtin_amdgcn_sched_barrier(0);
         }
      }

      int buf = 0;
      float *oPrev = a.out + tk.outBase + (size_t)(tk.outSlot0 + kh) * tk.ldo + fw + fcol;
      const size_t oStep = 2 * (size_t)tk.ldo;
      oPrev -= oStep;
      float *oQ = oPrev;
      float yP[16];
#pragma unroll
      for (int r = 0; r < 16; r++) yP[r] = 0.0f;
      float resQ = 0.0f;
      bool haveQ = false;
      bool prevAct = false;
      auto lse_full = [&]() {
         float m8[8], m4[4];
#pragma unroll
         for (int r = 0; r < 8; r++) m8[r] = fmaxf(yP[r], yP[r + 8]);
#pragma unroll
         for (int r = 0; r < 4; r++) m4[r] = fmaxf(m8[r], m8[r + 4]);
         const float mx = fmaxf(fmaxf(m4[0], m4[1]), fmaxf(m4[2], m4[3]));
         float e[16];
#pragma unroll
         for (int r = 0; r < 16; r++) e[r] = EXP2(yP[r] - mx);
#pragma unroll
         for (int r = 0; r < 8; r++) e[r] += e[r + 8];
#pragma unroll
         for (int r = 0; r < 4; r++) e[r] += e[r + 4];
         const float sm = (e[0] + e[1]) + (e[2] + e[3]);
         return (mx + LOG2(sm)) * 0.69314718055994531f;
      };
      int rLoV = 0x7fffffff, rHiV = -1;
      if (a.slotRange && lane < tk.nSlots) { const int2 rr = ((const int2 *)a.slotRange)[tk.slot0 + lane]; rLoV = rr.x; rHiV = rr.y; }
      const int wRow0 = tk.frame0 + fw, wRow1 = wRow0 + 31;
      for (int j = 0; j < nPairs; j++) {
         const bool more = j + 1 < nPairs;
         bool actJ = active;
         if (a.slotRange) {
            const int lo0 = __builtin_amdgcn_readlane(rLoV, (2 * j) & 63), lo1 = __builtin_amdgcn_readlane(rLoV, (2 * j + 1) & 63);
            const int hi0 = __builtin_amdgcn_readlane(rHiV, (2 * j) & 63), hi1 = __builtin_amdgcn_readlane(rHiV, (2 * j + 1) & 63);
            actJ = active && (lo0 < lo1 ? lo0 : lo1) <= wRow1 && (hi0 > hi1 ? hi0 : hi1) >= wRow0;
         }
         if (haveQ) { if (fw + fcol < tk.nFrames) *oQ = resQ; haveQ = false; }
         if (more) stage_pair(j + 1, buf ^ 1);
         if (!actJ) {
            if (prevAct) { resQ = lse_full(); oQ = oPrev; haveQ = true; }
         } else {
            typedef float v2f __attribute__((ext_vector_type(2)));
            float m6[6], m2[2], mx = 0.0f, sm = 0.0f, lg = 0.0f, resP = 0.0f;
            v2f nmx = {0.0f, 0.0f}, eA = {0.0f, 0.0f}, sA = {0.0f, 0.0f}, sB = {0.0f, 0.0f}, E01 = {0.0f, 0.0f}, E23 = {0.0f, 0.0f};
            auto exp_pair = [&](int i) { const v2f d = (v2f){yP[2 * i], yP[2 * i + 1]} + nmx; return (v2f){EXP2(d.x), EXP2(d.y)}; };
            auto lse_slice = [&](int sl) {
               if (sl == 0) { for (int r = 0; r < 3; r++) m6[r] = fmaxf(fmaxf(yP[3 * r], yP[3 * r + 1]), yP[3 * r + 2]); }
               else if (sl == 1) { for (int r = 3; r < 5; r++) m6[r] = fmaxf(fmaxf(yP[3 * r], yP[3 * r + 1]), yP[3 * r + 2]); m6[5] = yP[15]; }
               else if (sl == 2) { m2[0] = fmaxf(fmaxf(m6[0], m6[1]), m6[2]); m2[1] = fmaxf(fmaxf(m6[3], m6[4]), m6[5]); }
               else if (sl == 3) { mx = fmaxf(m2[0], m2[1]); nmx = (v2f){-mx, -mx}; }
               else if (sl == 4) eA = exp_pair(0);
               else if (sl == 5) sA = eA + exp_pair(4);
               else if (sl == 6) eA = exp_pair(2);
               else if (sl == 7) { sB = eA + exp_pair(6); E01 = sA + sB; }
               else if (sl == 8) eA = exp_pair(1);
               else if (sl == 9) sA = eA + exp_pair(5);
               else if (sl == 10) eA = exp_pair(3);
               else if (sl == 11) { sB = eA + exp_pair(7); E23 = sA + sB; }
               else if (sl < 15) { }
               else if (sl == 15) { sm = (E01.x + E01.y) + (E23.x + E23.y); }
               else if (sl == 16) { lg = LOG2(sm); }
               else { resP = (mx + lg) * 0.69314718055994531f; }
            };
            f16v Cx, Cc;
#pragma unroll
            for (int r = 0; r < 16; r++) { Cx[r] = 0.0f; Cc[r] = 0.0f; }
            auto cx_start = [&]() {
               if constexpr (DENSE) {
#pragma unroll
                  for (int b = 0; b < 4; b++) {
                     const f4 c0 = __builtin_bit_cast(f4, wbuf[buf][KS * 192 + 8 + kh * 4 + b]);
#pragma unroll
                     for (int r = 0; r < 4; r++) Cx[4 * b + r] = c0[r];
                  }
               }
            };
            bf8 wa[KS][3];
#pragma unroll
            for (int s = 0; s < 3; s++) wa[0][s] = __builtin_bit_cast(bf8, wbuf[buf][(0 * 3 + s) * 64 + lane]);
            __builtin_amdgcn_s_setprio(B16_PRIO_LEVEL);
#pragma unroll
            for (int ks = 0; ks < KS; ks++) {
               if (ks + 1 < KS) {
#pragma unroll
                  for (int s = 0; s < 3; s++) wa[ks + 1][s] = __builtin_bit_cast(bf8, wbuf[buf][((ks + 1) * 3 + s) * 64 + lane]);
               }
               Cc = __builtin_amdgcn_mfma_f32_32x32x16_bf16(wa[ks][1], zb[ks][1], Cc, 0, 0, 0);
               if (3 * ks + 0 < 18) lse_slice(3 * ks + 0);
               Cc = __builtin_amdgcn_mfma_f32_32x32x16_bf16(wa[ks][0], zb[ks][2], Cc, 0, 0, 0);
               if (ks == 0) cx_start();
               Cc = __builtin_amdgcn_mfma_f32_32x32x16_bf16(wa[ks][2], zb[ks][0], Cc, 0, 0, 0);
               if (3 * ks + 1 < 18) lse_slice(3 * ks + 1);
               Cc = __builtin_amdgcn_mfma_f32_32x32x16_bf16(wa[ks][0], zb[ks][1], Cc, 0, 0, 0);
               Cc = __builtin_amdgcn_mfma_f32_32x32x16_bf16(wa[ks][1], zb[ks][0], Cc, 0, 0, 0);
               if (3 * ks + 2 < 18) lse_slice(3 * ks + 2);
               Cx = __builtin_amdgcn_mfma_f32_32x32x16_bf16(wa[ks][0], zb[ks][0], Cx, 0, 0, 0);
            }
            for (int sl = 3 * KS; sl < 18; sl++) lse_slice(sl);
            asm volatile("" : "+v"(resP));
            resQ = resP; oQ = oPrev; haveQ = prevAct;
#pragma unroll
            for (int b = 0; b < 4; b++) {
               const f4 ci = __builtin_bit_cast(f4, wbuf[buf][KS * 192 + kh * 4 + b]);
#pragma unroll
               for (int r = 0; r < 4; r++) yP[4 * b + r] = (Cx[4 * b + r] + Cc[4 * b + r]) + ci[r];
            }
         }
         prevAct = actJ; oPrev += oStep;
         asm volatile("s_waitcnt vmcnt(0)" ::: "memory");
         __syncthreads();
         buf ^= 1;
      }
      if (haveQ) { if (fw + fcol < tk.nFrames) *oQ = resQ; }
      if (prevAct) {
         const float res = lse_full();
         if (fw + fcol < tk.nFrames && 2 * (nPairs - 1) + kh < tk.nSlots) *oPrev = res;
      }
   }
}

int htkamd_launch_score_bf16(const htkamd_model *m, const ScoreArgs &a, hipStream_t stream, hipEvent_t evStart, hipEvent_t evStop)
{
   if (a.nTasks <= 0) return HTKAMD_OK;
   { const int rc = htkamd_model_table_current(m, HTKAMD_SCORE_BF16, stream); if (rc) return rc; }
   if (a.qCounters == a.taskCounter + 8) HIPCHECK(hipMemsetAsync(a.taskCounter, 0, 16 * sizeof(int), stream));
   else {
      HIPCHECK(hipMemsetAsync(a.taskCounter, 0, sizeof(int), stream));
      if (a.qCounters) HIPCHECK(hipMemsetAsync(a.qCounters, 0, 8 * sizeof(int), stream));
   }
   if (m->f16Wide && (size_t)m->nTiles * ((size_t)3 * m->bf16NC * 64 * 16 + 64 * 16) >= ((size_t)1 << 32)) {
      htkamd_set_error("score_bf16: a table of %d tiles is beyond the kernel's 32-bit staging offsets", m->nTiles); return HTKAMD_EMODEL;
   }
   if (m->f16Wide) {
      dim3 block(256);
#define W_LAUNCH(KS_) do { const int b_ = a.nTasks < 256 * b16w_eu(KS_) ? a.nTasks : 256 * b16w_eu(KS_); \
                           hipExtLaunchKernelGGL((k_score_bf16w<KS_>), dim3(b_), block, 0, stream, evStart, evStop, 0, a); } while (0)
      if (m->bf16Dense) {
         W_LAUNCH(5); HIPCHECK(hipGetLastError());
         return HTKAMD_OK;
      }
      switch (m->bf16NC) {
      case 3: W_LAUNCH(6); break;
      case 2: W_LAUNCH(4); break;
      case 1: W_LAUNCH(2); break;
      default: htkamd_set_error("score_bf16: no kernel for %d K-chunks", m->bf16NC); return HTKAMD_EMODEL;
      }
#undef W_LAUNCH
      HIPCHECK(hipGetLastError());
      return HTKAMD_OK;
   }
   const int parts = B16_TASK_FRAMES / (16 * B16_COL_TILES * B16_WPB);
   int blocks = a.nTasks * parts;
   if (blocks > 256 * ((B16_COL_TILES > 2 ? 8 : 12) / B16_WPB)) blocks = 256 * ((B16_COL_TILES > 2 ? 8 : 12) / B16_WPB);
   dim3 grid(blocks), block(64 * B16_WPB);
   switch (m->bf16NC) {
   case 3: hipExtLaunchKernelGGL((k_score_bf16<3>), grid, block, 0, stream, evStart, evStop, 0, a); break;
   case 2: hipExtLaunchKernelGGL((k_score_bf16<2>), grid, block, 0, stream, evStart, evStop, 0, a); break;
   case 1: hipExtLaunchKernelGGL((k_score_bf16<1>), grid, block, 0, stream, evStart, evStop, 0, a); break;
   default: htkamd_set_error("score_bf16: no kernel for %d K-chunks", m->bf16NC); return HTKAMD_EMODEL;
   }
   HIPCHECK(hipGetLastError());
   return HTKAMD_OK;
}

struct Bf16TabArgs {
   int D, NC, S;
   const int *stateCompOff, *stateTileOff, *compGauss, *tileState;
   const float *mean, *ivar, *gconst, *compLogWt;
   unsigned short *tab;
};

template <bool WIDE>
__global__ void k_build_bf16tab(Bf16TabArgs a, int nTiles)
{
   const int NC = a.NC, D = a.D;
   const int idx = blockIdx.x * blockDim.x + threadIdx.x;
   if (idx >= nTiles * NC * 64) return;
   const int t = idx / (NC * 64), r = idx - t * (NC * 64), ch = r >> 6, lane = r & 63, rowc = lane & 15, kg = lane >> 4;
   const int s = a.tileState[t], c0 = a.stateCompOff[s], c1 = a.stateCompOff[s + 1];
   const int c = c0 + 16 * (t - a.stateTileOff[s]) + rowc;
   const size_t tileShorts = WIDE ? ((size_t)NC * 2 * 3 * 32 + 4) * 8 : (size_t)3 * NC * 64 * 8 + 64 * 8;
   unsigned short *T = a.tab + (size_t)t * tileShorts;
   const bool live = c < c1 && (c1 - c0 == 1 || a.compLogWt[c] > (float)LMINMIX);
   const double L2E = 1.4426950408889634;
   const float *mu = nullptr, *iv = nullptr;
   if (live) { const int g = a.compGauss[c]; mu = a.mean + (size_t)g * D; iv = a.ivar + (size_t)g * D; }
   const int dpc = (D + NC - 1) / NC, dlo = dpc * ch, dhi = (dlo + dpc < D) ? dlo + dpc : D;
   unsigned short p[3][8];
#pragma unroll
   for (int j = 0; j < 8; j++) {
      const int kk = 8 * kg + j, dim = dlo + (kk >> 1);
      float v = 0.0f;
      if (live && dim < dhi) v = (kk & 1) ? (float)((double)mu[dim] * iv[dim] * L2E) : (float)(-0.5 * (double)iv[dim] * L2E);
      if (live && kk == 30) {
         double q = 0.0;
         for (int i = dlo; i < dhi; i++) q += (double)mu[i] * mu[i] * iv[i];
         v = (float)(-0.5 * q * L2E);
      }
      split3(v, p[0][j], p[1][j], p[2][j]);
   }
#pragma unroll
   for (int pc = 0; pc < 3; pc++) {
      u4 w;
      w[0] = p[pc][0] | ((unsigned int)p[pc][1] << 16); w[1] = p[pc][2] | ((unsigned int)p[pc][3] << 16);
      w[2] = p[pc][4] | ((unsigned int)p[pc][5] << 16); w[3] = p[pc][6] | ((unsigned int)p[pc][7] << 16);
      const size_t word = WIDE ? (size_t)((2 * ch + (kg >> 1)) * 3 + pc) * 32 + (kg & 1) * 16 + rowc : (size_t)(pc * NC + ch) * 64 + lane;
      *(u4 *)(T + word * 8) = w;
   }
   if (ch == 0 && kg == 0) {
      float ci = -1.0e30f;
      if (live) {
         const double k0 = a.gconst[a.compGauss[c]];
         ci = (float)(((c1 - c0 == 1 ? 0.0 : (double)a.compLogWt[c]) - 0.5 * k0) * L2E);
      }
      if (WIDE) ((float *)(T + (size_t)NC * 2 * 3 * 32 * 8))[rowc] = ci;
      else {
         float *ciBase = (float *)(T + (size_t)3 * NC * 64 * 8);
         for (int j = 0; j < 16; j++) ciBase[((rowc >> 2) * 16 + j) * 4 + (rowc & 3)] = ci;
      }
   }
}

#define BT_TILES 4
__global__ __launch_bounds__(256) void k_build_bf16tab_dense_lds(Bf16TabArgs a, int nTiles, int KS)
{
   extern __shared__ float btRows[];
   const int D = a.D;
   const int t0 = blockIdx.x * BT_TILES;
   const int nT = (nTiles - t0 < BT_TILES) ? nTiles - t0 : BT_TILES;
   const int nR = nT * 16;
   float *qc = btRows + (size_t)BT_TILES * 16 * 2 * D;
   int *gOf = (int *)(qc + BT_TILES * 16 * 3);
   int *cOf = gOf + BT_TILES * 16;
   const double L2E = 1.4426950408889634;
   if ((int)threadIdx.x < nR) {
      const int t = t0 + (threadIdx.x >> 4), rowc = threadIdx.x & 15;
      const int s = a.tileState[t], c0 = a.stateCompOff[s], c1 = a.stateCompOff[s + 1];
      const int c = c0 + 16 * (t - a.stateTileOff[s]) + rowc;
      const bool live = c < c1 && (c1 - c0 == 1 || a.compLogWt[c] > (float)LMINMIX);
      gOf[threadIdx.x] = live ? a.compGauss[c] : -1;
      cOf[threadIdx.x] = (c1 - c0 == 1) ? -1 - c : c;
   }
   __syncthreads();
   for (int i = threadIdx.x; i < nR * D; i += blockDim.x) {
      const int r = i / D, d = i - r * D, g = gOf[r];
      float mu = 0.0f, iv = 0.0f;
      if (g >= 0) { mu = a.mean[(size_t)g * D + d]; iv = a.ivar[(size_t)g * D + d]; }
      btRows[(size_t)(2 * r) * D + d] = mu; btRows[(size_t)(2 * r + 1) * D + d] = iv;
   }
   __syncthreads();
   if ((int)threadIdx.x < 3 * nR) {
      const int r = threadIdx.x / 3, h = threadIdx.x - 3 * r;
      const float *mu = btRows + (size_t)(2 * r) * D, *iv = mu + D;
      int lo, hi; dense_const_range(h, D, lo, hi);
      double q = 0.0;
      for (int i = lo; i < hi; i++) q += (double)mu[i] * mu[i] * iv[i];
      qc[threadIdx.x] = (float)(-0.5 * q * L2E);
   }
   __syncthreads();
   const size_t tileShorts = ((size_t)KS * 3 * 32 + 8) * 8;
   for (int w = threadIdx.x; w < nT * KS * 32; w += blockDim.x) {
      const int tl = w / (KS * 32), r = w - tl * (KS * 32), ks = r >> 5, khf = (r >> 4) & 1, rowc = r & 15;
      const int row = tl * 16 + rowc;
      const bool live = gOf[row] >= 0;
      const float *mu = btRows + (size_t)(2 * row) * D, *iv = mu + D;
      unsigned short *T = a.tab + (size_t)(t0 + tl) * tileShorts;
      unsigned short p[3][8];
#pragma unroll
      for (int j = 0; j < 8; j++) {
         int dim, kind;
         dense_slot(16 * ks + 8 * khf + j, D, dim, kind);
         float v = 0.0f;
         if (live && kind == 0) v = (float)(-0.5 * (double)iv[dim] * L2E);
         else if (live && kind == 1) v = (float)((double)mu[dim] * iv[dim] * L2E);
         else if (live && kind >= 2) v = qc[3 * row + (kind - 1)];
         split3(v, p[0][j], p[1][j], p[2][j]);
      }
#pragma unroll
// ... 36 lines not shown
```

### htk_amd/csrc/kernels.h

```cpp
#ifndef HTKAMD_KERNELS_H
#define HTKAMD_KERNELS_H
#include <hip/hip_runtime.h>
#include <vector>
#include "internal.h"

#define SCORE_TILE_FRAMES 128
#define B16_TASK_FRAMES 128
#define SCORE_TASK_SLOTS  16
#define SCORE_TASK_SLOTS_WIDE 64
#define SCORE_TASK_SLOTS_EXACT 8

struct ScoreTask {
   int frame0;
   int nFrames;
   int slot0;
   int nSlots;
   int outSlot0;
   int ldo;
   size_t outBase;
};

struct ScoreArgs {
   const ScoreTask *tasks = nullptr;
   int nTasks = 0;
   const float *X = nullptr;
   const int *slotState = nullptr;
   float *out = nullptr;
   const int *stateCompOff = nullptr, *compGauss = nullptr;
   const float *compLogWt = nullptr, *gparam = nullptr;
   int PS = 0, D = 0;
   double minLogExp = 0.0;
   const double *laddTab = nullptr;
   int *taskCounter = nullptr;
   const float *mfmaTab = nullptr;
   const int *stateTileOff = nullptr;
   const void *bf16Tab = nullptr;
   const void *f16Tab = nullptr;
   const int *f16Ctl = nullptr;
   int *rangeFlag = nullptr;
   const float *var = nullptr;
   int NSt = 1;
   const float *streamWt = nullptr;
   const int *qStart = nullptr;
   int *qCounters = nullptr;
   const int *slotRange = nullptr;
};

static inline ScoreArgs htkamd_score_args(const htkamd_model *m)
{
   ScoreArgs a;
   a.stateCompOff = m->d_stateCompOff; a.compGauss = m->d_compGauss; a.compLogWt = m->d_compLogWt;
   a.gparam = m->d_gparam; a.PS = m->PS; a.D = m->D; a.minLogExp = m->minLogExp; a.laddTab = m->d_laddTab;
   a.mfmaTab = m->d_mfmaTab; a.stateTileOff = m->d_stateTileOff; a.bf16Tab = m->d_bf16Tab; a.var = m->d_var;
   a.NSt = m->NSt; a.streamWt = m->d_streamWt;
   return a;
}

static inline int htkamd_tile_count(int T, int nSlots, int FR, int SL) { return ((T + FR - 1) / FR) * ((nSlots + SL - 1) / SL); }
static inline void htkamd_tile_tasks(ScoreTask *tk, int frame0, int T, int slot0, int nSlots, size_t outBase, int ldo, int FR, int SL)
{
   for (int t0 = 0; t0 < T; t0 += FR)
      for (int k0 = 0; k0 < nSlots; k0 += SL, tk++) {
         tk->frame0 = frame0 + t0; tk->nFrames = (T - t0 < FR) ? T - t0 : FR;
         tk->slot0 = slot0 + k0; tk->nSlots = (nSlots - k0 < SL) ? nSlots - k0 : SL;
         tk->outSlot0 = k0; tk->ldo = ldo; tk->outBase = outBase + (size_t)t0;
      }
}
static inline void htkamd_tile_tasks(std::vector<ScoreTask> &v, int frame0, int T, int slot0, int nSlots, size_t outBase, int ldo, int FR, int SL)
{
   if (T <= 0 || nSlots <= 0) return;
   const size_t n = v.size();
   v.resize(n + (size_t)htkamd_tile_count(T, nSlots, FR, SL));
   htkamd_tile_tasks(v.data() + n, frame0, T, slot0, nSlots, outBase, ldo, FR, SL);
}

int htkamd_launch_score_exact(const htkamd_model *m, const ScoreArgs &a, hipStream_t stream, hipEvent_t evStart = nullptr, hipEvent_t evStop = nullptr, bool soutp = false, bool diagc = false);
int htkamd_launch_score_full(const htkamd_model *m, const ScoreArgs &a, hipStream_t stream, hipEvent_t evStart, hipEvent_t evStop, bool soutp, bool diagc);
int htkamd_launch_score_mfma(const htkamd_model *m, const ScoreArgs &a, hipStream_t stream, hipEvent_t evStart = nullptr, hipEvent_t evStop = nullptr);
int htkamd_launch_score_bf16(const htkamd_model *m, const ScoreArgs &a, hipStream_t stream, hipEvent_t evStart = nullptr, hipEvent_t evStop = nullptr);
int htkamd_launch_score_f16(const htkamd_model *m, const ScoreArgs &a, hipStream_t stream, hipEvent_t evStart = nullptr, hipEvent_t evStop = nullptr);
static inline int htkamd_launch_score(int mode, const htkamd_model *m, const ScoreArgs &a, hipStream_t s, hipEvent_t e0 = nullptr, hipEvent_t e1 = nullptr)
{
   if (m->fullc && (mode & (HTKAMD_SCORE_F16 | HTKAMD_SCORE_BF16 | HTKAMD_SCORE_MFMA))) {
      htkamd_set_error("score: a FULLC model is scored by the exact kernel only (score mode %d asks for a matrix-core one)", mode);
      return HTKAMD_EMODEL;
   }
   if (mode & HTKAMD_SCORE_F16) return htkamd_launch_score_f16(m, a, s, e0, e1);
   if (mode & HTKAMD_SCORE_BF16) return htkamd_launch_score_bf16(m, a, s, e0, e1);
   if (mode & HTKAMD_SCORE_MFMA) return htkamd_launch_score_mfma(m, a, s, e0, e1);
   return htkamd_launch_score_exact(m, a, s, e0, e1, (mode & HTKAMD_SCORE_SOUTP) != 0, (mode & HTKAMD_SCORE_DIAGC) != 0);
}

enum FbFamily {
   FB_LANE_PER_MODEL = 0,
   FB_LANE_PER_STATE = 1,
   FB_LEFT_TO_RIGHT = 2
};
struct UttDesc {
   int T, Q, nCells, nSlots;
   int frame0;
   int q0;
   int cell0;
   int slot0;
   int status;
   int nEval;
   int thr0, nThr;
   size_t outp0;
   size_t beta0;
   size_t gam0;
   size_t betaW0;
   int W, family;
   size_t alphaW0;
   int QP, reserved;
};

struct LaneRec { float aSelf, aOut, aEntry, aEntryNext; short q, j, N, pad; int sidx, cM; };
struct HitS { int frame, pad; double seed; };
struct MixRec { int g, frame; double L; };
struct MixHit { int st, frame; double seed; };

struct FbArgs {
   const UttDesc *utt;
   int nUtt;
   const int *uttList;
   int nList;
   const int *mN, *mTp, *mCell0, *mSlot0, *mDms, *mHmm, *mTrans;
   const short *cQ, *cI;
   const short *thrCell;
   const int *slotState;
   const short *sQ;
   const short *taperLo, *taperHi;
   short *qLo, *qHi, *aLo, *aHi;
   const float *X;
   const float *transP;
   float *outp;
   double *beta, *gam, *alphaDbg;
   double *betaW;
   double *alphaW;
   int *qBeam, *aBeam;
   double *trPart;
   double *pr;
   int *status;
   const int *stateCompOff, *compGauss, *transOff, *trOccOff;
   const float *compLogWt, *gparam, *mean;
   const double *laddTab;
   int PS, D, maxN, maxM;
   int nCellsMax, QMax, TMax;
   double *acc;
   htkamd_accs_layout lay;
   double pruneInit, pruneInc, pruneLim, minLogExp;
   float minFrwdP;
   int uFlags;
   size_t gamTotal;
   const size_t *gamOffByUtt;
   const int *gamChunkUtt;
   MixRec *rec, *recSorted;
   int recCap, G;
   int *recCtl;
   int NSt;
   const float *outpU;
   int compatRevisit;
   const int *nextSame;
   const int *dimStream;
   float *tmE;
   float *tmMaxP;
   const int *tmPoolOff;
   int tmPool, totalFrames;
   const ScoreTask *tmTasks; int tmNTasks; const int *tmSlotState; float *tmOut;
   const float *compWeight, *var;
   int tmCombine;
   const float *streamWt;
   MixHit *hits;
   int hitSlots;
   int *hitCtl;
   int nHitRegions, hitRegionCap;
   LaneRec *laneRec;
   const int *qBeamNP;
   int stBase;
   int *stCnt; int nTiedStates; HitS *stBucket; int stCap;
   int fastMath;
   double *sink;
};

int htkamd_launch_beta(const FbArgs &a, int blockDim, size_t lds, hipStream_t s);
int htkamd_launch_alpha(const FbArgs &a, int blockDim, size_t lds, hipStream_t s);
int htkamd_launch_mixstats(const FbArgs &a, hipStream_t s, bool dense, bool listed, bool deferState = false);
bool htkamd_mixstate_applies(const FbArgs &a);
int htkamd_launch_mixstate_range(const FbArgs &a, int st0, int st1, hipStream_t s);
int htkamd_launch_combine_streams(const FbArgs &a, hipStream_t s);
int htkamd_launch_mixstats_ms(const FbArgs &a, hipStream_t s);
int htkamd_launch_tm_score(const FbArgs &a, hipStream_t s);
int htkamd_launch_mixstats_tm(const FbArgs &a, hipStream_t s);
int htkamd_launch_mixhits_streams(const FbArgs &a, bool tied, hipStream_t s);
int htkamd_tm_score_block(const htkamd_model *m, const ScoreArgs &sa, int nRows, float tmBeam, hipStream_t s);
int htkamd_launch_beta_s(const FbArgs &a, int W, bool fast, hipStream_t s);
int htkamd_launch_alpha_s(const FbArgs &a, int W, bool fast, hipStream_t s);
int htkamd_launch_beta_w(const FbArgs &a, int W, bool fast, hipStream_t s);
int htkamd_launch_beta_lr(const FbArgs &a, int W, bool fast, hipStream_t s);
bool htkamd_beta_lr_is_lean(const FbArgs &a, bool fast);
int htkamd_launch_alpha_lr(const FbArgs &a, int W, bool fast, hipStream_t s);
int htkamd_launch_stats_lr(const FbArgs &a, int W, bool fast, hipStream_t s);
int htkamd_stats_lr_chunks(int TMax);
size_t htkamd_stats_lr_row_doubles(void);
int htkamd_stats_lr_region_cap(void);
int htkamd_launch_alpha_w(const FbArgs &a, int W, bool fast, hipStream_t s);

#endif
```

### htk_amd/csrc/update.hip

```cpp
#include <hip/hip_runtime.h>
#include <cstdlib>
#include <cstring>
#include <cmath>
#include "internal.h"
#include "hipcheck.h"

struct UpdArgs {
   int D, S, C, G, nT, H, PS, maxM;
   const int *stateCompOff, *compGauss, *transN, *transOff, *trOccOff, *hmmTrans, *hmmStateOff, *hmmState;
   float *mean, *var, *gconst, *compWeight, *transP;
   float *ivar, *gparam, *compLogWt;
   const unsigned char *rawLogWt;
   const double *acc;
   htkamd_accs_layout lay;
   int minEgs, uFlags, singleProcess, rowNormalise, hasVarFloor;
   float minVar, mixWeightFloor;
   double logTpi;
   const float *varFloor;
   unsigned char *qualT, *qualS, *qualG, *anyS, *anyG;
   unsigned char *flooredG;
   int *stats;
   int *blkStats;
   float *logVar;
   int tied;
// ... 362 lines not shown
            float iv;
            if (vv > 1E+30f) vv = 1E+30f;
            if (vv < 1E-30f) vv = 1E-30f;
            iv = 1 / vv;
            if (iv > 1E+30f) iv = 1E+30f;
            if (iv < 1E-30f) iv = 1E-30f;
            vv = 1 / iv;
         }
         if (qual && !outside) {
            const float muOcc = (float)dMuOcc;
            if (a.uFlags & HTKAMD_UPVARS) {
               const float occim = (float)dVaOcc;
               if (occim > 0.0f) {
                  const bool shared = (a.uFlags & HTKAMD_UPMEANS) == 0 || muOcc <= 0.0f;
                  const float muDiffk = shared ? 0.0f : (float)dMu / muOcc;
                  float x = (float)dVa / occim - muDiffk * muDiffk;
                  const float fl = a.hasVarFloor ? a.varFloor[k] : a.minVar;
                  if (x < fl) { x = fl; floored = live; }
                  vv = x;
               } else if (k == 0 && live) atomicAdd(blkCnt + 2, 1);
            }
            if ((a.uFlags & HTKAMD_UPMEANS) && muOcc > 0.0f) mm += (float)dMu / muOcc;
         }
         v[j] = vv; mu[j] = mm;
         float cc = vv;
         if (cc > 1E+30f) cc = 1E+30f;
         if (cc < 1E-30f) cc = 1E-30f;
         r[j] = outside ? 0.0f : 1 / cc;
         const float z = ((double)vv <= MINLARG) ? (float)LZERO : (float)log((double)vv);
         if (floored) { nFloored++; flRow[gl] = 1; }
         if (live) {
            lvRows[cl] = z;
            if (!full) { a.var[idx] = vv; a.mean[idx] = mm; a.ivar[idx] = r[j]; }
            *(float2 *)(gpRows + (size_t)gl * PS + 2 * k) = make_float2(mm, r[j]);
         }
      }
      if (full) {
         *(float4 *)(a.var + i0) = make_float4(v[0], v[1], v[2], v[3]);
         *(float4 *)(a.mean + i0) = make_float4(mu[0], mu[1], mu[2], mu[3]);
         *(float4 *)(a.ivar + i0) = make_float4(r[0], r[1], r[2], r[3]);
      }
   }
   {
#pragma unroll
      for (int o = 32; o > 0; o >>= 1) nFloored += __shfl_xor(nFloored, o);
      if (nFloored && (threadIdx.x & 63) == 0) atomicAdd(blkCnt + 0, nFloored);
   }
   __syncthreads();
   const int t = threadIdx.x;
   bool fl = false;
   if (t < nG) {
      const int g = g0 + t;
      fl = flRow[t] != 0;
      if (fl) a.flooredG[g] = 1;
      float gc = a.gconst[g];
      if (a.qualG[g] && (a.uFlags & (HTKAMD_UPMEANS | HTKAMD_UPVARS))) {
         int n = D;
         if (a.dimStream) { n = 0; for (int k = 0; k < D; k++) if (!OUTSIDE(g, k)) n++; }
         float sum = (float)((double)n * a.logTpi);
         const float *lv = lvRows + (size_t)t * D;
         for (int k = 0; k < D; k++) {
            if (OUTSIDE(g, k)) continue;
            sum += lv[k];
         }
         a.gconst[g] = gc = sum;
      }
      gpRows[(size_t)t * PS + 2 * D] = gc;
   }
   if (t < 64) {
      const unsigned long long fb = __ballot(fl);
      if (t == 0) { a.blkStats[3 * blockIdx.x + 0] = blkCnt[0]; a.blkStats[3 * blockIdx.x + 1] = __popcll(fb); a.blkStats[3 * blockIdx.x + 2] = blkCnt[2]; }
   }
   __syncthreads();
   float4 *dst = (float4 *)(a.gparam + (size_t)g0 * PS);
   const float4 *src = (const float4 *)gpRows;
   for (int i = threadIdx.x; i < nG * (PS >> 2); i += blockDim.x) dst[i] = src[i];
}

__global__ __launch_bounds__(128) void k_upd_gconst(UpdArgs a)
{
   extern __shared__ float lvRows[];
   const int g0 = blockIdx.x * blockDim.x, g = g0 + threadIdx.x;
   const int D = a.D;
   if (a.logVar) {
      const int nG = (a.G - g0 < (int)blockDim.x) ? a.G - g0 : (int)blockDim.x;
      const float *src = a.logVar + (size_t)g0 * D;
      for (int i = threadIdx.x; i < nG * D; i += blockDim.x) lvRows[i] = src[i];
      __syncthreads();
   }
   if (g >= a.G) return;
   int flooredCnt = a.flooredG[g] ? 1 : 0;
   {
      const unsigned long long fb = __ballot(flooredCnt != 0);
      if (fb && (threadIdx.x & 63) == (unsigned)(__ffsll((long long)fb) - 1)) atomicAdd(a.stats + 1, __popcll(fb));
   }
   if (a.qualG[g] && (a.uFlags & (HTKAMD_UPMEANS | HTKAMD_UPVARS))) {
      const float *var = a.var + (size_t)g * D;
      int n = D;
      if (a.dimStream) { n = 0; for (int k = 0; k < D; k++) if (!OUTSIDE(g, k)) n++; }
      float sum = (float)((double)n * a.logTpi);
      const float *lv = a.logVar ? lvRows + (size_t)threadIdx.x * D : nullptr;
      for (int k = 0; k < D; k++) {
         if (OUTSIDE(g, k)) continue;
         const float z = lv ? lv[k] : (((double)var[k] <= MINLARG) ? (float)LZERO : (float)log((double)var[k]));
         sum += z;
      }
      a.gconst[g] = sum;
   }
   a.gparam[(size_t)g * a.PS + 2 * D] = a.gconst[g];
}

struct MfmaTabArgs {
   int D, NS, S;
   const int *stateCompOff, *stateTileOff, *compGauss;
   const float *mean, *ivar, *gconst, *compLogWt;
   float *tab;
};

__global__ void k_upd_mfma(MfmaTabArgs a, int nTiles)
{
   const int idx = blockIdx.x * blockDim.x + threadIdx.x;
   if (idx >= nTiles * 16) return;
   const int t = idx >> 4, col = idx & 15;
   int lo = 0, hi = a.S - 1;
   while (lo < hi) { const int mid = (lo + hi + 1) >> 1; if (a.stateTileOff[mid] <= t) lo = mid; else hi = mid - 1; }
   const int s = lo, c0 = a.stateCompOff[s], c1 = a.stateCompOff[s + 1];
   const int c = c0 + 16 * (t - a.stateTileOff[s]) + col;
   const int NS = a.NS, D = a.D;
   float *T = a.tab + (size_t)t * (NS + 8) * 64;
   float *ciRow = T + (size_t)(NS + (col & 3)) * 64 + (col >> 2) * 16, *endRow = ciRow + 4 * 64;
   const bool live = c < c1 && (c1 - c0 == 1 || a.compLogWt[c] > (float)LMINMIX);
   if (!live) {
      for (int j = 0; j < 16; j++) { ciRow[j] = 0.0f; endRow[j] = -1.0e30f; }
      for (int st = 0; st < NS; st++) for (int kq = 0; kq < 4; kq++) T[(size_t)st * 64 + kq * 16 + col] = 0.0f;
      return;
   }
   const int g = a.compGauss[c];
   const float *mu = a.mean + (size_t)g * D, *iv = a.ivar + (size_t)g * D;
   double q = 0.0;
   for (int i = 0; i < D; i++) q += (double)mu[i] * mu[i] * iv[i];
   const double L2E = 1.4426950408889634;
   const float ci = (float)(-0.25 * q * L2E);
   const float ce = (float)(((c1 - c0 == 1 ? 0.0 : (double)a.compLogWt[c]) - 0.5 * (double)a.gconst[g] - 0.25 * q) * L2E);
   for (int j = 0; j < 16; j++) { ciRow[j] = ci; endRow[j] = ce; }
   for (int st = 0; st < NS; st++)
      for (int kq = 0; kq < 4; kq++) {
         const int dim = 2 * st + (kq >> 1);
         float v = 0.0f;
         if (dim < D) v = (kq & 1) ? (float)((double)mu[dim] * iv[dim] * L2E) : (float)(-0.5 * (double)iv[dim] * L2E);
         T[(size_t)st * 64 + kq * 16 + col] = v;
      }
}

__global__ void k_upd_export(const int *stats, int *dst, const int *blkStats, int nBlk)
{
   int c0 = 0, c1 = 0, c2 = 0;
   for (int i = threadIdx.x; i < nBlk; i += 64) { c0 += blkStats[3 * i]; c1 += blkStats[3 * i + 1]; c2 += blkStats[3 * i + 2]; }
#pragma unroll
   for (int o = 32; o > 0; o >>= 1) { c0 += __shfl_xor(c0, o); c1 += __shfl_xor(c1, o); c2 += __shfl_xor(c2, o); }
   if (threadIdx.x < 16) dst[threadIdx.x] = stats[threadIdx.x] + (threadIdx.x == 0 ? c0 : threadIdx.x == 1 ? c1 : threadIdx.x == 5 ? c2 : 0);
}

int htkamd_model_refresh_mfma_device(htkamd_model *m, void *stream)
{
   hipStream_t s = (hipStream_t)stream;
   if (!m->d_mfmaTab) return HTKAMD_OK;
   MfmaTabArgs t;
   t.D = m->D; t.NS = m->mfmaNS; t.S = m->S; t.stateCompOff = m->d_stateCompOff; t.stateTileOff = m->d_stateTileOff; t.compGauss = m->d_compGauss;
   t.mean = m->d_mean; t.ivar = m->d_ivar; t.gconst = m->d_gconst; t.compLogWt = m->d_compLogWt; t.tab = m->d_mfmaTab;
   const int n = m->nTiles * 16;
   hipLaunchKernelGGL(k_upd_mfma, dim3((n + 255) / 256), dim3(256), 0, s, t, m->nTiles);
   HIPCHECK(hipGetLastError());
   return HTKAMD_OK;
}

extern "C" int htkamd_model_update_device_begin(htkamd_model *m, htkamd_accs *accs, const htkamd_update_config *cfg, void *stream)
{
   if (!m || !accs || !cfg) { htkamd_set_error("model_update_device: NULL argument"); return HTKAMD_EINVAL; }
   if (accs->m != m) { htkamd_set_error("model_update_device: accumulators belong to a different model"); return HTKAMD_EINVAL; }
   if (cfg->uFlags & HTKAMD_UPMAP) { htkamd_set_error("model_update_device: MAP re-estimation (HTKAMD_UPMAP) is done by htkamd_model_update"); return HTKAMD_EMODEL; }
   hipStream_t s = (hipStream_t)stream;
   int rc;
   if ((rc = htkamd_model_device_tables(m))) return rc;
   const size_t nFlag = (size_t)m->nT + 2 * (size_t)m->S + 3 * (size_t)m->G;
   const bool tied = m->h_meanLeader != nullptr;
   const size_t nTiedInts = tied ? 2 * (size_t)m->G + (size_t)m->H : 0;
   const size_t nLog = tied ? 0 : (((size_t)m->G * m->D + 3) & ~(size_t)3);
   const size_t headBytes = (((nFlag + 63) & ~(size_t)63) + 16 * sizeof(int) + sizeof(float) * (size_t)m->D + sizeof(int) * nTiedInts + 255) & ~(size_t)255;
   const size_t need = headBytes + sizeof(float) * nLog;
   if (need > m->updScratchCap) {
      if (m->d_updScratch) (void)hipFree(m->d_updScratch);
      m->d_updScratch = nullptr; m->updScratchCap = 0;
      HIPCHECK(hipMalloc(&m->d_updScratch, need));
      m->updScratchCap = need;
   }
   unsigned char *fl = (unsigned char *)m->d_updScratch;
   HIPCHECK(hipMemsetAsync(fl, 0, ((nFlag + 63) & ~(size_t)63) + 16 * sizeof(int), s));
   UpdArgs a;
   memset(&a, 0, sizeof(a));
   a.D = m->D; a.S = m->S; a.C = m->C; a.G = m->G; a.nT = m->nT; a.H = m->H; a.PS = m->PS; a.maxM = m->maxM;
   a.stateCompOff = m->d_stateCompOff; a.compGauss = m->d_compGauss; a.transN = m->d_transN; a.transOff = m->d_transOff;
   a.trOccOff = m->d_trOccOff; a.hmmTrans = m->d_hmmTrans; a.hmmStateOff = m->d_hmmStateOff; a.hmmState = m->d_hmmState;
   a.mean = m->d_mean; a.var = m->d_var; a.gconst = m->d_gconst; a.compWeight = m->d_compWeight; a.transP = m->d_transP;
   a.ivar = m->d_ivar; a.gparam = m->d_gparam; a.compLogWt = m->d_compLogWt; a.rawLogWt = m->d_rawLogWt;
   a.acc = accs->d_vec; a.lay = accs->lay;
   a.dimStream = m->NSt > 1 ? m->d_dimStream : nullptr; a.gaussStream = m->NSt > 1 ? m->d_gaussStream : nullptr;
   a.minEgs = cfg->minEgs; a.uFlags = cfg->uFlags; a.singleProcess = m->tiedMix ? 0 : cfg->singleProcess; a.rowNormalise = cfg->rowNormalise;
   a.minVar = cfg->minVar; a.mixWeightFloor = cfg->mixWeightFloor; a.logTpi = log(HTK_TPI);
   a.qualT = fl; a.qualS = a.qualT + m->nT; a.anyS = a.qualS + m->S; a.qualG = a.anyS + m->S; a.anyG = a.qualG + m->G; a.flooredG = a.anyG + m->G;
   a.stats = (int *)(fl + ((nFlag + 63) & ~(size_t)63));
   a.logVar = tied ? nullptr : (float *)(fl + headBytes);
   a.blkStats = (int *)a.logVar;
   float *dFloor = (float *)(a.stats + 16);
   a.hasVarFloor = cfg->varFloor != nullptr; a.varFloor = dFloor;
   if (cfg->varFloor) HIPCHECK(hipMemcpyAsync(dFloor, cfg->varFloor, sizeof(float) * (size_t)m->D, hipMemcpyHostToDevice, s));
   int *scanPosHost = nullptr;
   if (tied) {
      const int G = m->G;
      a.tied = 1;
      a.meanLeader = m->d_shareTab; a.varLeader = a.meanLeader + G; a.varGroupSize = a.varLeader + G;
      a.muMemOff = a.varGroupSize + G; a.vaMemOff = a.muMemOff + G + 1; a.muMem = a.vaMemOff + G + 1; a.vaMem = a.muMem + m->shareMuMem;
      a.firstMu = (int *)(dFloor + m->D); a.firstVa = a.firstMu + G;
      HIPCHECK(hipMemsetAsync(a.firstMu, 0x7f, sizeof(int) * 2 * (size_t)G, s));
      if (m->h_scanOrder) {
         scanPosHost = (int *)malloc(sizeof(int) * (size_t)m->H);
         for (int k = 0; k < m->H; k++) scanPosHost[m->h_scanOrder[k]] = k;
         HIPCHECK(hipMemcpyAsync(a.firstVa + G, scanPosHost, sizeof(int) * (size_t)m->H, hipMemcpyHostToDevice, s));
         a.scanPos = a.firstVa + G;
      }
   }
   const int B = 128;
   hipLaunchKernelGGL(k_upd_mark, dim3((m->H + B - 1) / B), dim3(B), 0, s, a);
   {
      const int gw = m->maxM <= 4 ? 4 : m->maxM <= 16 ? 16 : m->maxM <= 64 ? 64 : 0;
      const unsigned nb = gw ? (unsigned)(((size_t)m->S * gw + 255) / 256) : 0, nbT = (unsigned)((m->nT + 255) / 256);
      if (gw == 4) hipLaunchKernelGGL(k_upd_state_w<4>, dim3(nb + nbT), dim3(256), 0, s, a, (int)nb);
      else if (gw == 16) hipLaunchKernelGGL(k_upd_state_w<16>, dim3(nb + nbT), dim3(256), 0, s, a, (int)nb);
      else if (gw == 64) hipLaunchKernelGGL(k_upd_state_w<64>, dim3(nb + nbT), dim3(256), 0, s, a, (int)nb);
      else {
         hipLaunchKernelGGL(k_upd_trans, dim3((m->nT + B - 1) / B), dim3(B), 0, s, a);
         hipLaunchKernelGGL(k_upd_state, dim3((m->S + B - 1) / B), dim3(B), 0, s, a);
      }
   }
   if (m->tiedMix) HIPCHECK(hipMemsetAsync(a.qualG, 1, (size_t)m->G, s));
   bool fusedG = false;
   {
      const size_t nEl = (size_t)m->G * m->D;
      const size_t ldsFused = sizeof(float) * (size_t)UPD_GPB * (m->D + m->PS) + sizeof(int) * UPD_GPB;
      if (nEl >= ((size_t)1 << 31)) { htkamd_set_error("model_update_device: %zu mean / variance elements (the element kernel indexes with 32 bits)", nEl); return HTKAMD_EMODEL; }
      if (tied) {
         hipLaunchKernelGGL(k_upd_first, dim3((m->H + B - 1) / B), dim3(B), 0, s, a);
         hipLaunchKernelGGL(k_upd_gauss_elem_tied, dim3((unsigned)((nEl + 255) / 256)), dim3(256), 0, s, a);
      } else if (!m->tiedMix && ldsFused <= 60 * 1024 && (m->PS & 3) == 0 && m->D <= 64) {
         const dim3 gr((unsigned)((m->G + UPD_GPB - 1) / UPD_GPB));
         switch ((UPD_GPB * m->D + 1023) / 1024) {
         case 1: hipLaunchKernelGGL(k_upd_gauss_fused<1>, gr, dim3(256), ldsFused, s, a); break;
         case 2: hipLaunchKernelGGL(k_upd_gauss_fused<2>, gr, dim3(256), ldsFused, s, a); break;
         case 3: hipLaunchKernelGGL(k_upd_gauss_fused<3>, gr, dim3(256), ldsFused, s, a); break;
         default: hipLaunchKernelGGL(k_upd_gauss_fused<4>, gr, dim3(256), ldsFused, s, a); break;
         }
         fusedG = true;
      } else
         hipLaunchKernelGGL(k_upd_gauss_elem, dim3((unsigned)((nEl + 1023) / 1024)), dim3(256), 0, s, a);
   }
   if (!fusedG) {
      UpdArgs ag = a;
      if (sizeof(float) * (size_t)B * m->D > 48 * 1024) ag.logVar = nullptr;
      hipLaunchKernelGGL(k_upd_gconst, dim3((m->G + B - 1) / B), dim3(B), ag.logVar ? sizeof(float) * (size_t)B * m->D : 0, s, ag);
   }
   HIPCHECK(hipGetLastError());
   if ((rc = htkamd_model_params_changed(m, s, 1))) return rc;
   const size_t nTp = (size_t)m->h_transOff[m->nT];
   if (!m->h_updPin) HIPCHECK(hipHostMalloc(&m->h_updPin, sizeof(float) * (nTp + 16), hipHostMallocDefault));
   if (!m->evUpd) { hipEvent_t e; HIPCHECK(hipEventCreateWithFlags(&e, hipEventDisableTiming)); m->evUpd = (void *)e; }
   hipLaunchKernelGGL(k_upd_export, dim3(1), dim3(64), 0, s, a.stats, (int *)(m->d_transP + nTp), a.blkStats, fusedG ? (int)((m->G + UPD_GPB - 1) / UPD_GPB) : 0);
   HIPCHECK(hipMemcpyAsync(m->h_updPin, m->d_transP, sizeof(float) * (nTp + 16), hipMemcpyDeviceToHost, s));
   HIPCHECK(hipEventRecord((hipEvent_t)m->evUpd, s));
   free(scanPosHost);
   m->updPending = 1;
   return HTKAMD_OK;
}

extern "C" int htkamd_model_update_device_end(htkamd_model *m, htkamd_update_stats *stats)
{
   if (!m || !m->updPending) { htkamd_set_error("model_update_device_end: no update in flight"); return HTKAMD_EINVAL; }
   m->updPending = 0;
   HIPCHECK(hipEventSynchronize((hipEvent_t)m->evUpd));
   const size_t nTp = (size_t)m->h_transOff[m->nT];
   int hst[16];
   memcpy(m->h_transP, m->h_updPin, sizeof(float) * nTp);
   memcpy(hst, (const float *)m->h_updPin + nTp, sizeof(hst));
   htkamd_model_refresh_topology(m);
   if (stats) {
      stats->nFloorVar = hst[0]; stats->nFloorVarMix = hst[1]; stats->nSkippedHmm = hst[2];
      stats->nNoTransOut = hst[3]; stats->nNoMixUse = hst[4]; stats->nNoVarUse = hst[5]; stats->nWeightAboveOne = hst[6];
   }
   if (hst[6] > 0) { htkamd_set_error("model_update_device: %d mixture weights above 1.001 (HERest: HError 2393)", hst[6]); return HTKAMD_EMODEL; }
   return HTKAMD_OK;
}

extern "C" int htkamd_model_update_device(htkamd_model *m, htkamd_accs *accs, const htkamd_update_config *cfg, htkamd_update_stats *stats, void *stream)
{
   const int rc = htkamd_model_update_device_begin(m, accs, cfg, stream);
   return rc ? rc : htkamd_model_update_device_end(m, stats);
}
```

Baseline: 28.79 billion frame-state log-lik/s.

## Fuse pass tail kernels, memsets and result copies into one launch

Merges the transition-reduce kernels, the mixture-hit kernel, the zeroing of the next pass's state counters and task counters, and the result export into a single tail kernel. The state-count buffer is double-buffered so the next pass needs no memset, and the result and update exports write straight to pinned host memory from kernels instead of issuing D2H memcpys. This removes several small launches, memsets and copies per iteration. In exchange it adds zero-copy host writes over PCIe and extra state tracking for buffer parity and cleanliness.

Result: faster. 29.70 billion frame-state log-lik/s, median of 6 (+3.2%).

```diff
diff --git a/htk_amd/build.py b/htk_amd/build.py
--- a/htk_amd/build.py
+++ b/htk_amd/build.py
@@ -9,7 +9,7 @@
 LIB = os.path.join(HERE, "libhtk_amd.so")
 HIP_SRCS = ["csrc/model.hip", "csrc/gmm_exact.hip", "csrc/gmm_full.hip", "csrc/gmm_mfma.hip", "csrc/gmm_bf16.hip", "csrc/gmm_f16.hip", "csrc/fb_kernels.hip", "csrc/fb_wave.hip", "csrc/fb_state.hip", "csrc/fb_lr.hip", "csrc/fb.hip", "csrc/viterbi.hip", "csrc/decode.hip", "csrc/decode_n.hip", "csrc/decode_ord.hip", "csrc/decode_set.hip", "csrc/mfcc.hip", "csrc/cepsnorm.hip", "csrc/inputxform.hip", "csrc/update.hip", "csrc/comm.hip", "csrc/treeclust.hip", "csrc/datacluster.hip", "csrc/treesynth.hip", "csrc/hinit.hip", "csrc/hrest.hip", "csrc/results.hip", "csrc/latrescore.hip"]
 C_SRCS = ["host/prep.c", "host/update.c", "host/fbank.c", "host/accio.c", "host/parmfile.c", "host/cepsnorm.c", "host/mmf.c", "host/labio.c", "host/net.c", "host/lattice.c", "host/slfout.c", "host/treeclust.c", "host/treesynth.c", "host/hinit.c", "host/hrest.c", "host/unit_train.c", "host/results.c", "host/latrescore.c", "host/htktext.c"]
-HEADERS = ["csrc/fb_lr_lean.inc", "csrc/internal.h", "csrc/kernels.h", "csrc/hipcheck.h", "csrc/devbuf.h", "csrc/ladd.h", "csrc/wavegrp.h", "csrc/fb_state.h", "csrc/decode.h", "csrc/decode_dev.h", "csrc/decode_ord.h", "csrc/hinit_seg.h", "csrc/gauss_derive.h", "csrc/unit_train.h", "csrc/results.h", "csrc/latrescore.h", "host/mmf_priv.h", "host/htktext.h", "../include/htk_amd.h"]
+HEADERS = ["csrc/fb_lr_lean.inc", "csrc/fb_trans_reduce.inc", "csrc/internal.h", "csrc/kernels.h", "csrc/hipcheck.h", "csrc/devbuf.h", "csrc/ladd.h", "csrc/wavegrp.h", "csrc/fb_state.h", "csrc/decode.h", "csrc/decode_dev.h", "csrc/decode_ord.h", "csrc/hinit_seg.h", "csrc/gauss_derive.h", "csrc/unit_train.h", "csrc/results.h", "csrc/latrescore.h", "host/mmf_priv.h", "host/htktext.h", "../include/htk_amd.h"]
 ARCH = "gfx950"
 EXTRA_FLAGS = {"csrc/gmm_mfma.hip": ["-fno-honor-nans"], "csrc/gmm_bf16.hip": ["-fno-honor-nans"], "csrc/gmm_f16.hip": ["-fno-honor-nans"],
                "csrc/fb_kernels.hip": ["-Wno-pass-failed"]}
diff --git a/htk_amd/csrc/fb.hip b/htk_amd/csrc/fb.hip
--- a/htk_amd/csrc/fb.hip
+++ b/htk_amd/csrc/fb.hip
@@ -162,6 +162,9 @@
    DevBuf d_stCnt, d_stBucket;
    DevBuf d_laneRec;
    bool mixStateLast = false;
+   bool stClean = false; int stPar = 0; const int *stCntLast = nullptr;
+   bool ctrClean = false;
+   bool resExported = false;
    bool mixDeferred = false;
    FbArgs *faMix = nullptr;
    const int *qBeamLast = nullptr;
@@ -681,10 +684,17 @@
       while (cap < 65536 && cap * (size_t)m->S < (size_t)16 * fb->totalFrames) cap <<= 1;
       while (cap > 64 && cap * (size_t)m->S * sizeof(HitS) > ((size_t)1 << 30)) cap >>= 1;
       { const char *e = getenv("HTKAMD_ST_CAP"); if (e && atoi(e) > 0) cap = (size_t)atoi(e); }
-      if ((rc = fb->d_stCnt.reserve(sizeof(int) * (3 * (size_t)m->S + 4))) || (rc = fb->d_stBucket.reserve(sizeof(HitS) * cap * (size_t)m->S))) return rc;
+      const size_t nCnt = 3 * (size_t)m->S + 4;
+      const void *was = fb->d_stCnt.p;
+      if ((rc = fb->d_stCnt.reserve(sizeof(int) * 2 * nCnt)) || (rc = fb->d_stBucket.reserve(sizeof(HitS) * cap * (size_t)m->S))) return rc;
+      if (!fb->stClean || fb->d_stCnt.p != was) {
+         HIPCHECK(hipMemsetAsync(fb->d_stCnt.p, 0, sizeof(int) * 2 * nCnt, s));
+         fb->stPar = 0;
+      }
+      fb->stClean = false;
       fb->mixStateLast = true;
-      fa.stCnt = (int *)fb->d_stCnt.p; fa.nTiedStates = m->S; fa.stBucket = (HitS *)fb->d_stBucket.p; fa.stCap = (int)cap;
-      HIPCHECK(hipMemsetAsync(fa.stCnt, 0, sizeof(int) * (3 * (size_t)m->S + 4), s));
+      fa.stCnt = (int *)fb->d_stCnt.p + fb->stPar * nCnt; fa.nTiedStates = m->S; fa.stBucket = (HitS *)fb->d_stBucket.p; fa.stCap = (int)cap;
+      fb->stCntLast = fa.stCnt;
    }
    return HTKAMD_OK;
 }
@@ -713,29 +723,37 @@
    return HTKAMD_OK;
 }
 
-static int fb_stats_lr(htkamd_fb *fb, const FbArgs &fa, bool fastLadd, bool noEv, hipStream_t s)
+static int fb_stats_lr(htkamd_fb *fb, const FbArgs &fa, bool fastLadd, bool noEv, hipStream_t s, TailArgs *tail)
 {
    int rc;
    FbArgs fc = fa;
    size_t rowOff = 0;
+   if (tail) { tail->nSeg = 0; tail->segBlk0[0] = 0; }
    for (int c = 3; c >= 0; c--) {
       const UttClasses::Range r = fb->cls.of(FB_LEFT_TO_RIGHT, clsW[c]);
       fc.uttList = fb->uttList.dev + r.first; fc.nList = r.n;
       fc.trPart = fa.trPart ? fa.trPart + rowOff * htkamd_stats_lr_row_doubles() : nullptr;
       fc.hits = fa.hits ? fa.hits + rowOff * htkamd_stats_lr_region_cap() : nullptr; fc.hitCtl = fa.hitCtl ? fa.hitCtl + rowOff : nullptr;
-      rowOff += (size_t)fc.nList * htkamd_stats_lr_chunks(fb->TMax) * clsW[c];
-      if ((rc = htkamd_launch_stats_lr(fc, clsW[c], fastLadd, s))) return rc;
+      const size_t nRows = (size_t)fc.nList * htkamd_stats_lr_chunks(fb->TMax) * clsW[c];
+      if (tail && nRows > 0) {
+         const int i = tail->nSeg++;
+         tail->segRow0[i] = (int)rowOff; tail->segRows[i] = (int)nRows; tail->segBlk0[i + 1] = tail->segBlk0[i] + (int)((nRows + 255) / 256);
+      }
+      rowOff += nRows;
+      if ((rc = htkamd_launch_stats_lr(fc, clsW[c], fastLadd, s, tail == nullptr))) return rc;
    }
    if (!noEv) HIPCHECK(hipEventRecord(fb->ev[4], s));
    return HTKAMD_OK;
 }
 
-static int fb_mix_stats(htkamd_fb *fb, const htkamd_fb_config *cfg, FbArgs &fa, bool defer, hipStream_t s)
+static int fb_mix_stats(htkamd_fb *fb, const htkamd_fb_config *cfg, FbArgs &fa, bool defer, hipStream_t s, const TailArgs *tail)
 {
    const htkamd_model *m = fb->m;
    const int nLr = fb->cls.nLr();
    int rc;
-   if (!(cfg->uFlags & (HTKAMD_UPMEANS | HTKAMD_UPVARS | HTKAMD_UPMIXES))) return HTKAMD_OK;
+   const bool anyMix = (cfg->uFlags & (HTKAMD_UPMEANS | HTKAMD_UPVARS | HTKAMD_UPMIXES)) != 0;
+   if (tail && (!anyMix || m->tiedMix || m->NSt > 1)) { htkamd_set_error("fb_execute: a tail launch without the state-bucketed statistics"); return HTKAMD_EINVAL; }
+   if (!anyMix) return HTKAMD_OK;
    if ((cfg->uFlags & (HTKAMD_UPMEANS | HTKAMD_UPVARS)) && fb->recCapForce >= 0) {
       const size_t cap = fb->recCapForce > 0 ? (size_t)fb->recCapForce : std::min<size_t>((size_t)16 * fb->totalFrames + 4096, (size_t)1 << 30);
       if ((rc = fb->d_rec.reserve(sizeof(MixRec) * cap)) || (rc = fb->d_recSorted.reserve(sizeof(MixRec) * cap)) ||
@@ -750,11 +768,22 @@
       return HTKAMD_OK;
    }
    const bool dense = fb->nUtt > nLr && fa.gamTotal > 0, listed = nLr > 0;
-   if ((rc = htkamd_launch_mixstats(fa, s, dense, listed, defer))) return rc;
+   if ((rc = htkamd_launch_mixstats(fa, s, dense, listed, defer, tail))) return rc;
    if (defer && listed && !dense && htkamd_mixstate_applies(fa)) {
       if (!fb->faMix) fb->faMix = new FbArgs();
       *fb->faMix = fa;
       fb->mixDeferred = true;
+   }
+   return HTKAMD_OK;
+}
+
+static int res_staging(htkamd_fb *fb, size_t bytes)
+{
+   if (bytes > fb->h_resCap) {
+      if (fb->h_res) (void)hipHostFree(fb->h_res);
+      fb->h_res = nullptr; fb->h_resCap = 0;
+      HIPCHECK(hipHostMalloc(&fb->h_res, bytes + bytes / 4, hipHostMallocDefault));
+      fb->h_resCap = bytes + bytes / 4;
    }
    return HTKAMD_OK;
 }
@@ -771,13 +800,15 @@
       htkamd_set_error("fb_execute: the model's minimum durations changed since htkamd_fb_prepare (a re-estimated transition reached or left zero): prepare the batch again");
       return HTKAMD_EINVAL;
    }
-   const ScoreArgs sa = fb_score_args(fb, cfg);
+   ScoreArgs sa = fb_score_args(fb, cfg);
    if (cfg->scoreMode & ~(HTKAMD_SCORE_MFMA | HTKAMD_SCORE_FASTLADD | HTKAMD_SCORE_BF16 | HTKAMD_SCORE_F16 | HTKAMD_SCORE_SOUTP | HTKAMD_SCORE_DIAGC)) { htkamd_set_error("fb_execute: unknown score mode %d", cfg->scoreMode); return HTKAMD_EINVAL; }
    const bool fastLadd = (cfg->scoreMode & HTKAMD_SCORE_FASTLADD) != 0;
    FbArgs fa = fb_args(fb, cfg, accs);
    const LdsSizes lds = fb_lds_sizes(fa);
 
    int rc;
+   sa.countersZero = fb->ctrClean && sa.taskCounter == (int *)fb->d_counter.p;
+   fb->ctrClean = false; fb->resExported = false;
    if (fb->copyPending) HIPCHECK(hipStreamWaitEvent(s, fb->evCopy, 0));
    const bool noEv = fb->evMode == 1;
    HIPCHECK(hipEventRecord(fb->ev[0], s));
@@ -800,7 +831,24 @@
    if ((rc = fb->d_betaW.reserve(sizeof(double) * (fb->betaWTotal + 8 * 512)))) return rc;
    fa.betaW = (double *)fb->d_betaW.p;
    if (fb->cls.nLr() > 0 && (rc = fb_reserve_lr(fb, cfg, fa, fastLadd, s))) return rc;
-   if ((rc = fb_recursions(fb, fa, lds, fastLadd, noEv, s)) || (rc = fb_stats_lr(fb, fa, fastLadd, noEv, s)) || (rc = fb_mix_stats(fb, cfg, fa, defer, s))) return rc;
+   const bool tailFused = fb->cls.nLr() > 0 && fb->mixStateLast && !(fb->nUtt > fb->cls.nLr() && fa.gamTotal > 0);
+   TailArgs tail;
+   memset(&tail, 0, sizeof(tail));
+   if (tailFused) {
+      const size_t nCnt = 3 * (size_t)m->S + 4;
+      tail.zero[0] = (int *)fb->d_stCnt.p + (fb->stPar ^ 1) * nCnt; tail.nZero[0] = (int)nCnt;
+      tail.zero[1] = (int *)fb->d_counter.p; tail.nZero[1] = 16;
+      if (!fb->resPending) {
+         if ((rc = res_staging(fb, fb->res().bytes()))) return rc;
+         void *dv = nullptr;
+         HIPCHECK(hipHostGetDevicePointer(&dv, fb->h_res, 0));
+         tail.resSrc = (const int *)fb->d_pr.p; tail.resDst = (int *)dv; tail.resBytes = (int)fb->res().bytes();
+      }
+      tail.nHouse = 1 + (int)((nCnt + 4095) / 4096);
+   }
+   if ((rc = fb_recursions(fb, fa, lds, fastLadd, noEv, s)) || (rc = fb_stats_lr(fb, fa, fastLadd, noEv, s, tailFused ? &tail : nullptr)) ||
+       (rc = fb_mix_stats(fb, cfg, fa, defer, s, tailFused ? &tail : nullptr))) return rc;
+   if (tailFused) { fb->stClean = true; fb->stPar ^= 1; fb->ctrClean = true; fb->resExported = tail.resDst != nullptr; }
    HIPCHECK(hipEventRecord(fb->ev[5], s));
    fb->timed = true; fb->evModeLast = noEv ? 1 : 0;
    return HTKAMD_OK;
@@ -829,17 +877,6 @@
    return HTKAMD_OK;
 }
 
-
-static int res_staging(htkamd_fb *fb, size_t bytes)
-{
-   if (bytes > fb->h_resCap) {
-      if (fb->h_res) (void)hipHostFree(fb->h_res);
-      fb->h_res = nullptr; fb->h_resCap = 0;
-      HIPCHECK(hipHostMalloc(&fb->h_res, bytes + bytes / 4, hipHostMallocDefault));
-      fb->h_resCap = bytes + bytes / 4;
-   }
-   return HTKAMD_OK;
-}
 
 extern "C" int htkamd_fb_results_begin(htkamd_fb *fb, void *stream)
 {
@@ -850,7 +887,7 @@
    int rc = res_staging(fb, bytes);
    if (rc) return rc;
    if (!fb->evRes) HIPCHECK(hipEventCreateWithFlags(&fb->evRes, hipEventDisableTiming));
-   HIPCHECK(hipMemcpyAsync(fb->h_res, fb->d_pr.p, bytes, hipMemcpyDeviceToHost, s));
+   if (!fb->resExported) HIPCHECK(hipMemcpyAsync(fb->h_res, fb->d_pr.p, bytes, hipMemcpyDeviceToHost, s));
    HIPCHECK(hipEventRecord(fb->evRes, s));
    fb->resPending = true;
    return HTKAMD_OK;
@@ -913,11 +950,11 @@
 {
    if (!fb || !out) { htkamd_set_error("fb_mix_counts: NULL"); return HTKAMD_EINVAL; }
    out[0] = out[1] = -1;
-   if (!fb->timed || !fb->mixStateLast || !fb->d_stCnt.p) return HTKAMD_OK;
+   if (!fb->timed || !fb->mixStateLast || !fb->stCntLast) return HTKAMD_OK;
    HIPCHECK(hipEventSynchronize(fb->ev[5]));
    const size_t S = (size_t)fb->m->S;
    std::vector<int> c(2 * S);
-   HIPCHECK(hipMemcpy(c.data(), (int *)fb->d_stCnt.p + S + 4, sizeof(int) * 2 * S, hipMemcpyDeviceToHost));
+   HIPCHECK(hipMemcpy(c.data(), fb->stCntLast + S + 4, sizeof(int) * 2 * S, hipMemcpyDeviceToHost));
    out[0] = out[1] = 0;
    for (size_t i = 0; i < S; i++) { out[0] += c[2 * i]; out[1] += c[2 * i + 1]; }
    return HTKAMD_OK;
diff --git a/htk_amd/csrc/fb_kernels.hip b/htk_amd/csrc/fb_kernels.hip
--- a/htk_amd/csrc/fb_kernels.hip
+++ b/htk_amd/csrc/fb_kernels.hip
@@ -709,7 +709,7 @@
 }
 
 template <int DT, int GS>
-__global__ __launch_bounds__(256, 3) void k_mixhits(FbArgs a)
+__device__ __forceinline__ void mixhits_block(const FbArgs &a, int blk, int nBlk)
 {
    constexpr int HPS = 64 / GS;
    __shared__ int hitSt[4][64], hitFrame[4][64];
@@ -717,8 +717,8 @@
    __shared__ unsigned long long hitKey[4][64];
    const int lane = threadIdx.x & 63, wv = threadIdx.x >> 6;
    const int grp = lane / GS, sub = lane % GS;
-   const int nWaves = (int)(((size_t)gridDim.x * blockDim.x) >> 6);
-   const int waveId = (int)(((size_t)blockIdx.x * blockDim.x + threadIdx.x) >> 6);
+   const int nWaves = (int)(((size_t)nBlk * blockDim.x) >> 6);
+   const int waveId = (int)(((size_t)blk * blockDim.x + threadIdx.x) >> 6);
    if (a.stCnt && a.stBucket && !a.hitSlots && a.stCnt[a.nTiedStates] == 0) return;
    int recBase = -1, recUsed = 0;
    volatile int *hSt = hitSt[wv], *hFr = hitFrame[wv];
@@ -801,6 +801,33 @@
    }
    if (recBase >= 0 && recUsed + lane < 64) a.rec[recBase + recUsed + lane].g = -1;
 }
+template <int DT, int GS>
+__global__ __launch_bounds__(256, 3) void k_mixhits(FbArgs a) { mixhits_block<DT, GS>(a, (int)blockIdx.x, (int)gridDim.x); }
+
+#include "fb_trans_reduce.inc"
+template <int DT, int GS>
+__global__ __launch_bounds__(256, 3) void k_pass_tail(FbArgs a, TailArgs t)
+{
+   const int b = (int)blockIdx.x, nTr = t.segBlk0[t.nSeg];
+   if (b < nTr) {
+      int i = 0;
+      while (i + 1 < t.nSeg && b >= t.segBlk0[i + 1]) i++;
+      trans_reduce_block(a, a.trPart + (size_t)t.segRow0[i] * TR_ROW, t.segRows[i], b - t.segBlk0[i]);
+      return;
+   }
+   if (b < nTr + t.nHouse) {
+      const int tid = (b - nTr) * 256 + (int)threadIdx.x, nThr = t.nHouse * 256;
+#pragma unroll
+      for (int k = 0; k < 2; k++)
+         if (t.zero[k]) for (int i = tid; i < t.nZero[k]; i += nThr) t.zero[k][i] = 0;
+      if (t.resDst) {
+         for (int i = tid; i < t.resBytes / 4; i += nThr) t.resDst[i] = t.resSrc[i];
+         __threadfence_system();
+      }
+      return;
+   }
+   mixhits_block<DT, GS>(a, b - nTr - t.nHouse, t.nList);
+}
 
 #define REC_TILE 2048
 __global__ __launch_bounds__(256) void k_rec_tilesum(int *ctl, int G, int *tileSum)
@@ -1124,12 +1151,13 @@
    return HTKAMD_OK;
 }
 
-int htkamd_launch_mixstats(const FbArgs &a_in, hipStream_t s, bool dense, bool listed, bool deferState)
-{
-   if (!dense && !listed) return HTKAMD_OK;
+int htkamd_launch_mixstats(const FbArgs &a_in, hipStream_t s, bool dense, bool listed, bool deferState, const TailArgs *tail)
+{
+   if (!dense && !listed) { if (tail) { htkamd_set_error("mixture statistics: a tail launch without a list"); return HTKAMD_EINVAL; } return HTKAMD_OK; }
    FbArgs a = a_in;
    dense = dense && a.gamTotal > 0;
    const bool stateOnly = listed && !dense && htkamd_mixstate_applies(a);
+   if (tail && !stateOnly) { htkamd_set_error("mixture statistics: a tail launch outside the state-bucketed path"); return HTKAMD_EINVAL; }
    if (stateOnly) a.rec = nullptr;
    if (a.rec) HIPCHECK(hipMemsetAsync(a.recCtl, 0, sizeof(int) * (3 * ((size_t)a.G + 1) + 1), s));
 #define MIX_LAUNCH(K, GS) \
@@ -1150,7 +1178,16 @@
    }
    if (listed) {
       const dim3 grid(stateOnly ? 512 : 4096), block(256);
-      if (stateOnly) {
+      if (stateOnly && tail) {
+         TailArgs t = *tail;
+         t.nList = (int)grid.x;
+         const dim3 gridT((unsigned)(t.segBlk0[t.nSeg] + t.nHouse + t.nList));
+         if (a.D == 39) hipLaunchKernelGGL((k_pass_tail<39, 16>), gridT, block, 0, s, a, t);
+         else if (a.D == 26) hipLaunchKernelGGL((k_pass_tail<26, 16>), gridT, block, 0, s, a, t);
+         else hipLaunchKernelGGL((k_pass_tail<13, 16>), gridT, block, 0, s, a, t);
+         HIPCHECK(hipGetLastError());
+         if (!deferState) { const int rc = htkamd_launch_mixstate_range(a_in, 0, a_in.nTiedStates, s); if (rc) return rc; }
+      } else if (stateOnly) {
          MIX_LAUNCH_GS(k_mixhits)
          HIPCHECK(hipGetLastError());
          if (!deferState) { const int rc = htkamd_launch_mixstate_range(a_in, 0, a_in.nTiedStates, s); if (rc) return rc; }
diff --git a/htk_amd/csrc/fb_lr.hip b/htk_amd/csrc/fb_lr.hip
--- a/htk_amd/csrc/fb_lr.hip
+++ b/htk_amd/csrc/fb_lr.hip
@@ -434,60 +434,10 @@
 }
 
 #define STATS_FC 32
-#define TR_ROW 16
 #define EXP_TERM(acc, x) do { if constexpr (FAST) acc += exp_fast(x); else if ((x) > EXPFLOOR) acc += exp_tab((x), etab); } while (0)
 
-__global__ __launch_bounds__(256) void k_trans_reduce(FbArgs a, int nRows)
-{
-   __shared__ double sh[256][TR_ROW + 1];
-   __shared__ int mixed;
-   const int tid = threadIdx.x, r = blockIdx.x * 256 + tid;
-   if (tid == 0) mixed = 0;
-   const double *row = a.trPart + (size_t)r * TR_ROW;
-   int ti = -1;
-   if (r < nRows) ti = (int)row[TR_ROW - 1];
-#pragma unroll
-   for (int k = 0; k < 11; k++) sh[tid][k] = (ti >= 0) ? row[k] : 0.0;
-   __syncthreads();
-   __shared__ int tiBlock;
-   if (tid == 0) tiBlock = -1;
-   __syncthreads();
-   if (ti >= 0) atomicMax(&tiBlock, ti);
-   __syncthreads();
-   const int tb = tiBlock;
-   if (ti >= 0 && ti != tb) mixed = 1;
-   __syncthreads();
-   auto add_row = [&](int t_, const double *v) {
-      const int N0 = a.trOccOff[t_ + 1] - a.trOccOff[t_];
-      double *tr = a.acc + a.lay.tr + a.transOff[t_];
-      double *oc = a.acc + a.lay.trOcc + a.trOccOff[t_];
-      for (int i = 2; i <= 4 && i <= N0 - 1; i++) {
-         if (v[i - 2] != 0.0) atomicAdd(tr + (size_t)(i - 1) * N0 + (i - 1), v[i - 2]);
-         if (v[3 + i - 2] != 0.0) atomicAdd(tr + (size_t)(i - 1) * N0 + i, v[3 + i - 2]);
-         if (v[7 + i - 2] != 0.0) atomicAdd(oc + (i - 1), v[7 + i - 2]);
-      }
-      if (v[6] != 0.0) atomicAdd(tr + 1, v[6]);
-      if (v[10] != 0.0) atomicAdd(oc, v[10]);
-   };
-   if (tb < 0) return;
-   if (mixed) {
-      if (ti >= 0) add_row(ti, sh[tid]);
-      return;
-   }
-   const int k = tid & 15, part = tid >> 4;
-   double v = 0.0;
-   if (k < 11) for (int rr = part; rr < 256; rr += 16) v += sh[rr][k];
-   __syncthreads();
-   sh[part][k] = v;
-   __syncthreads();
-   if (tid < 11) {
-      double tot = 0.0;
-      for (int p = 0; p < 16; p++) tot += sh[p][tid];
-      sh[16][tid] = tot;
-   }
-   __syncthreads();
-   if (tid == 0) add_row(tb, sh[16]);
-}
+#include "fb_trans_reduce.inc"
+__global__ __launch_bounds__(256) void k_trans_reduce(FbArgs a, int nRows) { trans_reduce_block(a, a.trPart, nRows, (int)blockIdx.x); }
 
 #include "fb_lr_lean.inc"
 
@@ -553,13 +503,13 @@
    return HTKAMD_OK;
 }
 
-int htkamd_launch_stats_lr(const FbArgs &a, int W, bool fast, hipStream_t s)
+int htkamd_launch_stats_lr(const FbArgs &a, int W, bool fast, hipStream_t s, bool reduce)
 {
    if (a.nList <= 0) return HTKAMD_OK;
    const int nChunks = htkamd_stats_lr_chunks(a.TMax);
    if (fast) launch_stats_sp<true>(a, W, nChunks, s); else launch_stats_sp<false>(a, W, nChunks, s);
    const int nRows = a.nList * nChunks * W;
-   hipLaunchKernelGGL(k_trans_reduce, dim3((nRows + 255) / 256), dim3(256), 0, s, a, nRows);
+   if (reduce) hipLaunchKernelGGL(k_trans_reduce, dim3((nRows + 255) / 256), dim3(256), 0, s, a, nRows);
    HIPCHECK(hipGetLastError());
    return HTKAMD_OK;
 }
diff --git a/htk_amd/csrc/fb_trans_reduce.inc b/htk_amd/csrc/fb_trans_reduce.inc
--- /dev/null
+++ b/htk_amd/csrc/fb_trans_reduce.inc
@@ -0,0 +1,55 @@
+#ifndef TR_ROW
+#define TR_ROW 16
+#endif
+
+static __device__ __forceinline__ void trans_reduce_block(const FbArgs &a, const double *trPart, int nRows, int blk)
+{
+   __shared__ double sh[256][TR_ROW + 1];
+   __shared__ int mixed;
+   const int tid = threadIdx.x, r = blk * 256 + tid;
+   if (tid == 0) mixed = 0;
+   const double *row = trPart + (size_t)r * TR_ROW;
+   int ti = -1;
+   if (r < nRows) ti = (int)row[TR_ROW - 1];
+#pragma unroll
+   for (int k = 0; k < 11; k++) sh[tid][k] = (ti >= 0) ? row[k] : 0.0;
+   __syncthreads();
+   __shared__ int tiBlock;
+   if (tid == 0) tiBlock = -1;
+   __syncthreads();
+   if (ti >= 0) atomicMax(&tiBlock, ti);
+   __syncthreads();
+   const int tb = tiBlock;
+   if (ti >= 0 && ti != tb) mixed = 1;
+   __syncthreads();
+   auto add_row = [&](int t_, const double *v) {
+      const int N0 = a.trOccOff[t_ + 1] - a.trOccOff[t_];
+      double *tr = a.acc + a.lay.tr + a.transOff[t_];
+      double *oc = a.acc + a.lay.trOcc + a.trOccOff[t_];
+      for (int i = 2; i <= 4 && i <= N0 - 1; i++) {
+         if (v[i - 2] != 0.0) atomicAdd(tr + (size_t)(i - 1) * N0 + (i - 1), v[i - 2]);
+         if (v[3 + i - 2] != 0.0) atomicAdd(tr + (size_t)(i - 1) * N0 + i, v[3 + i - 2]);
+         if (v[7 + i - 2] != 0.0) atomicAdd(oc + (i - 1), v[7 + i - 2]);
+      }
+      if (v[6] != 0.0) atomicAdd(tr + 1, v[6]);
+      if (v[10] != 0.0) atomicAdd(oc, v[10]);
+   };
+   if (tb < 0) return;
+   if (mixed) {
+      if (ti >= 0) add_row(ti, sh[tid]);
+      return;
+   }
+   const int k = tid & 15, part = tid >> 4;
+   double v = 0.0;
+   if (k < 11) for (int rr = part; rr < 256; rr += 16) v += sh[rr][k];
+   __syncthreads();
+   sh[part][k] = v;
+   __syncthreads();
+   if (tid < 11) {
+      double tot = 0.0;
+      for (int p = 0; p < 16; p++) tot += sh[p][tid];
+      sh[16][tid] = tot;
+   }
+   __syncthreads();
+   if (tid == 0) add_row(tb, sh[16]);
+}
diff --git a/htk_amd/csrc/gmm_bf16.hip b/htk_amd/csrc/gmm_bf16.hip
--- a/htk_amd/csrc/gmm_bf16.hip
+++ b/htk_amd/csrc/gmm_bf16.hip
@@ -487,7 +487,8 @@
 {
    if (a.nTasks <= 0) return HTKAMD_OK;
    { const int rc = htkamd_model_table_current(m, HTKAMD_SCORE_BF16, stream); if (rc) return rc; }
-   if (a.qCounters == a.taskCounter + 8) HIPCHECK(hipMemsetAsync(a.taskCounter, 0, 16 * sizeof(int), stream));
+   if (a.countersZero) ;
+   else if (a.qCounters == a.taskCounter + 8) HIPCHECK(hipMemsetAsync(a.taskCounter, 0, 16 * sizeof(int), stream));
    else {
       HIPCHECK(hipMemsetAsync(a.taskCounter, 0, sizeof(int), stream));
       if (a.qCounters) HIPCHECK(hipMemsetAsync(a.qCounters, 0, 8 * sizeof(int), stream));
diff --git a/htk_amd/csrc/kernels.h b/htk_amd/csrc/kernels.h
--- a/htk_amd/csrc/kernels.h
+++ b/htk_amd/csrc/kernels.h
@@ -32,6 +32,7 @@
    double minLogExp = 0.0;
    const double *laddTab = nullptr;
    int *taskCounter = nullptr;
+   bool countersZero = false;
    const float *mfmaTab = nullptr;
    const int *stateTileOff = nullptr;
    const void *bf16Tab = nullptr;
@@ -182,9 +183,15 @@
    double *sink;
 };
 
+struct TailArgs {
+   int nSeg, segRow0[4], segRows[4], segBlk0[5];
+   int nHouse, nList;
+   int *zero[2]; int nZero[2];
+   const int *resSrc; int *resDst; int resBytes;
+};
 int htkamd_launch_beta(const FbArgs &a, int blockDim, size_t lds, hipStream_t s);
 int htkamd_launch_alpha(const FbArgs &a, int blockDim, size_t lds, hipStream_t s);
-int htkamd_launch_mixstats(const FbArgs &a, hipStream_t s, bool dense, bool listed, bool deferState = false);
+int htkamd_launch_mixstats(const FbArgs &a, hipStream_t s, bool dense, bool listed, bool deferState = false, const TailArgs *tail = nullptr);
 bool htkamd_mixstate_applies(const FbArgs &a);
 int htkamd_launch_mixstate_range(const FbArgs &a, int st0, int st1, hipStream_t s);
 int htkamd_launch_combine_streams(const FbArgs &a, hipStream_t s);
@@ -199,7 +206,7 @@
 int htkamd_launch_beta_lr(const FbArgs &a, int W, bool fast, hipStream_t s);
 bool htkamd_beta_lr_is_lean(const FbArgs &a, bool fast);
 int htkamd_launch_alpha_lr(const FbArgs &a, int W, bool fast, hipStream_t s);
-int htkamd_launch_stats_lr(const FbArgs &a, int W, bool fast, hipStream_t s);
+int htkamd_launch_stats_lr(const FbArgs &a, int W, bool fast, hipStream_t s, bool reduce = true);
 int htkamd_stats_lr_chunks(int TMax);
 size_t htkamd_stats_lr_row_doubles(void);
 int htkamd_stats_lr_region_cap(void);
diff --git a/htk_amd/csrc/update.hip b/htk_amd/csrc/update.hip
--- a/htk_amd/csrc/update.hip
+++ b/htk_amd/csrc/update.hip
@@ -538,13 +538,20 @@
       }
 }
 
-__global__ void k_upd_export(const int *stats, int *dst, const int *blkStats, int nBlk)
-{
+__global__ void k_upd_export(const int *stats, int *dst, const int *blkStats, int nBlk, const float *transP, int nTp, float *pin)
+{
+   for (int i = blockIdx.x * 64 + threadIdx.x; i < nTp; i += gridDim.x * 64) pin[i] = transP[i];
+   if (blockIdx.x != 0) { __threadfence_system(); return; }
    int c0 = 0, c1 = 0, c2 = 0;
    for (int i = threadIdx.x; i < nBlk; i += 64) { c0 += blkStats[3 * i]; c1 += blkStats[3 * i + 1]; c2 += blkStats[3 * i + 2]; }
 #pragma unroll
    for (int o = 32; o > 0; o >>= 1) { c0 += __shfl_xor(c0, o); c1 += __shfl_xor(c1, o); c2 += __shfl_xor(c2, o); }
-   if (threadIdx.x < 16) dst[threadIdx.x] = stats[threadIdx.x] + (threadIdx.x == 0 ? c0 : threadIdx.x == 1 ? c1 : threadIdx.x == 5 ? c2 : 0);
+   if (threadIdx.x < 16) {
+      const int v = stats[threadIdx.x] + (threadIdx.x == 0 ? c0 : threadIdx.x == 1 ? c1 : threadIdx.x == 5 ? c2 : 0);
+      dst[threadIdx.x] = v;
+      ((int *)(pin + nTp))[threadIdx.x] = v;
+   }
+   __threadfence_system();
 }
 
 int htkamd_model_refresh_mfma_device(htkamd_model *m, void *stream)
@@ -659,8 +666,13 @@
    const size_t nTp = (size_t)m->h_transOff[m->nT];
    if (!m->h_updPin) HIPCHECK(hipHostMalloc(&m->h_updPin, sizeof(float) * (nTp + 16), hipHostMallocDefault));
    if (!m->evUpd) { hipEvent_t e; HIPCHECK(hipEventCreateWithFlags(&e, hipEventDisableTiming)); m->evUpd = (void *)e; }
-   hipLaunchKernelGGL(k_upd_export, dim3(1), dim3(64), 0, s, a.stats, (int *)(m->d_transP + nTp), a.blkStats, fusedG ? (int)((m->G + UPD_GPB - 1) / UPD_GPB) : 0);
-   HIPCHECK(hipMemcpyAsync(m->h_updPin, m->d_transP, sizeof(float) * (nTp + 16), hipMemcpyDeviceToHost, s));
+   void *pin = nullptr;
+   HIPCHECK(hipHostGetDevicePointer(&pin, m->h_updPin, 0));
+   const size_t nbExp = (nTp + 255) / 256;
+   if (nTp >= ((size_t)1 << 31)) { htkamd_set_error("model_update_device: %zu transition entries (the export kernel indexes with 32 bits)", nTp); return HTKAMD_EMODEL; }
+   hipLaunchKernelGGL(k_upd_export, dim3((unsigned)(nbExp < 1 ? 1 : nbExp > 64 ? 64 : nbExp)), dim3(64), 0, s, a.stats, (int *)(m->d_transP + nTp), a.blkStats,
+                      fusedG ? (int)((m->G + UPD_GPB - 1) / UPD_GPB) : 0, (const float *)m->d_transP, (int)nTp, (float *)pin);
+   HIPCHECK(hipGetLastError());
    HIPCHECK(hipEventRecord((hipEvent_t)m->evUpd, s));
    free(scanPosHost);
    m->updPending = 1;
```
